# anthonyhu/tumblr-emotions

Measured on AMD Instinct MI355X. Metric: training samples/sec (224x224 img + 32-tok text, batch 256), higher is better.
Workload: dtype f32; 1 GPU; joint train step (fwd+bwd+all-reduce+Adam): Inception-v1 224x224x3 + 300-d embedding + LSTM-512, T=32, V=10000, 15 classes, batch 256 per GPU, reference freeze (<=Mixed_5b conv weights frozen, all BN betas trainable), dropout 0.8, BN train mode; global_batch=256, per_gpu_batch=256, parallelism=dp1, launch=eager

## Files before the change

include/ds_kernels.h:

```cpp
#ifndef DS_KERNELS_H
#define DS_KERNELS_H

#include <stddef.h>
#include <stdint.h>

#ifdef __cplusplus
extern "C" {
#endif

#define DS_OK 0
#define DS_ERR_ARG (-1)
#define DS_ERR_LAUNCH (-2)
#define DS_ERR_WORKSPACE (-3)

#define DS_DTYPE_F32 0
#define DS_DTYPE_BF16 1

#define DS_EPI_BIAS 1
#define DS_EPI_RELU 2
#define DS_EPI_ACCUM 4
#define DS_EPI_STATS 8
#define DS_EPI_MASK 16
#define DS_EPI_BNSUMS 32
#define DS_EPI_BN_RELU 64
// ... 312 lines not shown
                           int32_t N, int32_t H, int32_t W, int32_t C, int32_t k, int32_t stride, int32_t pad_t,
                           int32_t pad_l, int32_t OH, int32_t OW, int32_t y_dtype, float *amax, void *stream);
int ds_bn_pool_bwd_partials(int32_t N, int32_t OH, int32_t OW, int32_t C);
int ds_bn_pool_bwd_reduce(const float *z, const float *dpool, const uint8_t *argmax, int32_t N, int32_t H, int32_t W,
                          int32_t C, int32_t pad_t, int32_t pad_l, int32_t OH, int32_t OW, const float *mean,
                          const float *rstd, const float *shift, float *partials, void *stream);
int ds_bn_pool_bwd_apply(const float *z, const float *dpool, const uint8_t *argmax, int32_t N, int32_t H, int32_t W,
                         int32_t C, int32_t pad_t, int32_t pad_l, int32_t OH, int32_t OW, const float *mean,
                         const float *rstd, const float *shift, const float *coef, float *dz, void *stream);
int ds_bn_pool_bwd_apply_cols(const float *z, int32_t ldz, float *dz, int32_t lddz, const float *dpool, const uint8_t *argmax,
                              int32_t Cp, int32_t c0, int32_t N, int32_t H, int32_t W, int32_t pad_t, int32_t pad_l, int32_t OH,
                              int32_t OW, int32_t ncols, const float *mean, const float *rstd, const float *shift,
                              const float *coef_g, const float *coef_gx, int32_t k, void *stream);
int ds_bn_pool_infer_bwd_apply(const float *z, const float *dpool, const uint8_t *argmax, int32_t N, int32_t H, int32_t W,
                               int32_t C, int32_t pad_t, int32_t pad_l, int32_t OH, int32_t OW, const float *rstd,
                               const float *shift, float *dz, void *stream);
int ds_bn_pool_infer_bwd_apply_sums(const float *z, const float *dpool, const uint8_t *argmax, int32_t N, int32_t H, int32_t W,
                                    int32_t C, int32_t pad_t, int32_t pad_l, int32_t OH, int32_t OW, const float *rstd,
                                    const float *shift, float *dz, float *partials, void *stream);
int ds_maxpool_bwd(const float *dy, const uint8_t *argmax, float *dx, int32_t accumulate, int32_t N,
                   int32_t H, int32_t W, int32_t C, int32_t k, int32_t stride, int32_t pad_t, int32_t pad_l,
                   int32_t OH, int32_t OW, void *stream);

int ds_maxpool3_bwd_sums_partials(int32_t N, int32_t W, int32_t C);
int ds_maxpool3_bwd_sums(const float *dy, const uint8_t *argmax, float *dx, int32_t accumulate, const void *y,
                         int32_t y_dtype, int32_t N, int32_t H, int32_t W, int32_t C, float *partials, void *stream);

int ds_maxpool3_bwd_dy16(const void *dy16, const uint8_t *argmax, float *dx, int32_t accumulate, const void *y, int32_t y_dtype,
                         int32_t N, int32_t H, int32_t W, int32_t C, float *partials, void *stream);

int ds_avgpool_dropout_fwd(const float *x, int32_t N, int32_t HW, int32_t C, float keep, uint64_t seed,
                           const uint64_t *seed_dev, const float *mask_in, float *mask_out, float *out,
                           void *stream);
int ds_avgpool_dropout_bwd(const float *dout, const float *mask, int32_t N, int32_t HW, int32_t C,
                           float keep, float *dx, void *stream);

int ds_gather_rows(const float *table, const int64_t *ids, float *out, int32_t B, int32_t T, int32_t D,
                   int64_t table_rows, int32_t time_major, void *stream);

int ds_token_dot(const float *dx, const float *x, const int64_t *seq_len, float *out, int32_t B, int32_t T, int32_t D,
                 void *stream);

int ds_embedding_grad(const float *dx, const int64_t *ids, float *dtable, int32_t B, int32_t T, int32_t D,
                      int64_t table_rows, int32_t time_major, void *stream);

int ds_lstm_cell_fwd(float *gates, const float *rec_slabs, int32_t nslabs, int64_t slab_stride,
                     const float *c_prev, const float *h_prev, const int64_t *seq_len, int32_t t, int32_t B,
                     int32_t H, float forget_bias, float *c_out, float *h_out, void *stream);
int ds_lstm_cell_bwd(const float *acts, const float *c_t, const float *c_prev, const float *dh,
                     const float *dh_slabs, int32_t nslabs, int64_t slab_stride, const float *dc,
                     const int64_t *seq_len, int32_t t, int32_t B, int32_t H, float *dgates, float *dc_prev,
                     float *dh_carry, void *stream);

int ds_seq_sort_desc(const int64_t *seq_len, int32_t B, int32_t T, int32_t *perm, int64_t *len_sorted, void *stream);
int ds_permute_rows(const void *src, int64_t lds, void *dst, int64_t ldd, const int32_t *perm, int32_t rows, int32_t cols,
                    int32_t elem_bytes, int32_t gather, void *stream);
#define DS_LSTM_SKIP_MASKED 256
int ds_lstm_seq_supported(int32_t B, int32_t H);
size_t ds_lstm_seq_workspace(int32_t B, int32_t H);
int ds_lstm_seq_fwd(float *gates, const float *wh, int32_t ldw, float *h, float *c, const int64_t *seq_len, int32_t T,
                    int32_t B, int32_t H, float forget_bias, int32_t rows, void *ws, size_t ws_bytes, void *stream);
int ds_lstm_seq_bwd(const float *acts, const float *wh, int32_t ldw, const float *c, const float *dh_last,
                    int32_t ld_dh, const int64_t *seq_len, int32_t T, int32_t B, int32_t H, float *dgates, int32_t rows,
                    void *ws, size_t ws_bytes, void *stream);
int ds_lstm_seq_status(void *ws, int32_t B);
#ifdef DS_TUNING
int ds_debug_lstm_seq_set_profile(void *buf);
int ds_debug_lstm_seq_set_profile_bwd(void *buf);
#endif

int ds_softmax_ce(const float *logits, const int64_t *labels, int32_t B, int32_t C, float grad_scale,
                  const float *grad_scale_dev, float *loss, float *dlogits, void *stream);

int ds_adam_tf(float *theta, const float *g, float *m, float *v, int64_t n, int64_t n_wd, float wd,
               float grad_scale, float lr_t, const float *lr_t_dev, float beta1, float beta2, float eps,
               void *stream);

int ds_grad_accumulate(float *acc, float *g, int64_t n, int32_t mode, void *stream);

int ds_sumsq(const float *x, int64_t n, float *scratch, float *out, void *stream);
int ds_colsum(const float *x, int64_t M, int32_t C, int32_t ld, float *scratch, float *out, void *stream);
int ds_slab_epilogue(const float *slabs, int32_t splits, int64_t slab_stride, int32_t lds, int64_t M, int32_t N, float *out,
                     int32_t ldo, const float *bias, const float *mask, int32_t ldmask, int32_t flags, void *stream);
int ds_copy2d(const float *src, int32_t lds, float *dst, int32_t ldd, int64_t rows, int32_t cols,
              void *stream);
int ds_pad_channels(const float *src, int32_t cs, float *dst, int32_t cd, int64_t pixels, void *stream);
int ds_fill(float *dst, int64_t n, float value, void *stream);

typedef struct ds_preprocess_desc {
    int64_t offset;
    int32_t height, width;
    float scale_y, scale_x;
} ds_preprocess_desc;
int ds_preprocess_eval(const uint8_t *bytes, int64_t nbytes, const ds_preprocess_desc *desc, int32_t batch, const float *lut,
                       float *out, int32_t out_h, int32_t out_w, void *stream);

#define DS_PREPROCESS_FLIP 1u
#define DS_PREPROCESS_SATURATION_FIRST 2u
typedef struct ds_preprocess_train_desc {
    int64_t offset;
    int32_t height, width;
    float scale_y, scale_x;
    float delta;
    float factor;
    uint32_t flags;
    uint32_t reserved;
} ds_preprocess_train_desc;
int ds_preprocess_train(const uint8_t *bytes, int64_t nbytes, const ds_preprocess_train_desc *desc, int32_t batch,
                        const float *lut, float *out, int32_t out_h, int32_t out_w, void *stream);

#define DS_JPEG_UNSUPPORTED 1
#define DS_JPEG_MORE 2
#define DS_JPEG_444 0
#define DS_JPEG_422 1
#define DS_JPEG_420 2
#define DS_JPEG_GREY 3
typedef struct ds_jpeg_info {
    int32_t width, height;
    int32_t components;
    int32_t sampling;
    int32_t restart_interval;
    int32_t supported;
    int64_t coef_count;
    int64_t coef_bytes;
    uint8_t quant[3][64];
} ds_jpeg_info;
int ds_jpeg_probe(const uint8_t *bytes, int64_t n, ds_jpeg_info *info);
int ds_jpeg_entropy_decode(const uint8_t *bytes, int64_t n, const ds_jpeg_info *info, int16_t *coef, int64_t capacity);

typedef struct ds_jpeg_desc {
    int64_t coef_offset;
    int64_t out_offset;
    int32_t width, height;
    int32_t sampling;
    int32_t y0, x0, crop_h, crop_w;
    int32_t reserved;
    uint8_t quant[3][64];
} ds_jpeg_desc;
int ds_jpeg_reconstruct_host(const int16_t *coef, int64_t ncoef, const ds_jpeg_desc *desc, int32_t batch,
                             uint8_t *out_bytes, int64_t nbytes);
int ds_jpeg_reconstruct(const int16_t *coef, int64_t ncoef, const ds_jpeg_desc *desc, int32_t batch, uint8_t *out_bytes,
                        int64_t nbytes, void *scratch, int64_t scratch_bytes, void *stream);

typedef struct ds_example_fields {
    int64_t image_offset, image_length;
    int64_t seq_len, label, post_id, day;
    int32_t text_len;
    int32_t reserved;
} ds_example_fields;
int ds_example_parse(const uint8_t *rec, int64_t n, int64_t *text, int32_t text_capacity, ds_example_fields *fields);
int ds_jpeg_record_decode(const uint8_t *rec, int64_t n, int64_t *text, int32_t text_capacity, ds_example_fields *fields,
                          ds_jpeg_info *info, int16_t *coef, int64_t capacity, int32_t *jpeg_status);

typedef struct ds_jpeg_huff {
    uint8_t counts[16];
    uint8_t values[256];
} ds_jpeg_huff;
typedef struct ds_jpeg_scan_info {
    int64_t scan_begin;
    int64_t cut_count;
    ds_jpeg_huff dc[3], ac[3];
} ds_jpeg_scan_info;
int ds_jpeg_scan(const uint8_t *bytes, int64_t n, ds_jpeg_info *info, ds_jpeg_scan_info *scan, int64_t *cuts, int64_t capacity);
int ds_jpeg_record_scan(const uint8_t *rec, int64_t n, int64_t *text, int32_t text_capacity, ds_example_fields *fields,
                        ds_jpeg_info *info, ds_jpeg_scan_info *scan, int64_t *cuts, int64_t capacity, int32_t *jpeg_status);
int ds_jpeg_restart_transcode(const uint8_t *bytes, int64_t n, int32_t interval_mcus, uint8_t *out, int64_t capacity,
// ... 51 lines not shown
```

tumblr_emotions_amd/_lib.py:

```python
import ctypes as C
import os

_HERE = os.path.dirname(os.path.abspath(__file__))
LIB_PATH = os.environ.get("DS_LIB") or os.path.join(_HERE, "libds_kernels.so")

def tuning_env(name, default=None):
    return os.environ.get(name, default) if os.environ.get("DS_LIB") else default


DS_EPI_BIAS, DS_EPI_RELU, DS_EPI_ACCUM, DS_EPI_STATS, DS_EPI_MASK, DS_EPI_BNSUMS = 1, 2, 4, 8, 16, 32
DS_EPI_BN_RELU = 64
DS_DTYPE_F32, DS_DTYPE_BF16 = 0, 1
DS_FP8_E4M3, DS_FP8_E5M2 = 0, 1
DS_CONV_FWD, DS_CONV_DGRAD = 0, 1
DS_LSTM_SKIP_MASKED = 256
DS_ARITH_F32, DS_ARITH_BF16, DS_ARITH_FP8, DS_ARITH_F32X3 = 0, 1, 2, 3
DS_FAM_IGEMM, DS_FAM_WINO2, DS_FAM_WINO4, DS_FAM_STEM, DS_FAM_BF16D, DS_FAM_FP8D, DS_FAM_F32X3, DS_FAM_WINO4H, DS_FAM_STEM_POOL = range(9)
DS_FAM_STEM_DGRAD = 9
DS_PLAN_NO_WINO, DS_PLAN_NO_WINO4, DS_PLAN_NO_STEM_DIRECT, DS_PLAN_NO_BF16_DIRECT, DS_PLAN_ACT16, DS_PLAN_PACKED_RGB = 1, 2, 4, 8, 16, 32
DS_PLAN_FP8_EVERYWHERE, DS_PLAN_FP8_WIDE_RULE, DS_PLAN_NO_WINO4H, DS_PLAN_STEM_POOL = 64, 128, 256, 512
DS_PLAN_NO_SPLITK = 1024
DS_PREPROCESS_FLIP, DS_PREPROCESS_SATURATION_FIRST = 1, 2
DS_JPEG_UNSUPPORTED, DS_JPEG_MORE = 1, 2
DS_JPEG_444, DS_JPEG_422, DS_JPEG_420, DS_JPEG_GREY = 0, 1, 2, 3
DS_JPEG_E_CODE, DS_JPEG_E_RUN, DS_JPEG_E_RANGE, DS_JPEG_E_COLUMN, DS_JPEG_E_SEGMENT, DS_JPEG_E_TABLE = 1, 2, 4, 8, 16, 32


class ConvDesc(C.Structure):
    _fields_ = [
        ("N", C.c_int32), ("H", C.c_int32), ("W", C.c_int32), ("Cin", C.c_int32), ("ldx", C.c_int32),
        ("KH", C.c_int32), ("KW", C.c_int32), ("stride", C.c_int32), ("pad_t", C.c_int32), ("pad_l", C.c_int32),
        ("OH", C.c_int32), ("OW", C.c_int32), ("Cout", C.c_int32), ("ldz", C.c_int32),
        ("w_tap_stride", C.c_int64), ("w_n_stride", C.c_int32), ("w_k_stride", C.c_int32),
        ("flip", C.c_int32), ("fold_cin", C.c_int32), ("flags", C.c_int32), ("ldmask", C.c_int32),
        ("splits", C.c_int32), ("z_split_stride", C.c_int64),
        ("tile_nt", C.c_int32), ("grid_x", C.c_int32), ("dtype", C.c_int32), ("x_dtype", C.c_int32),
        ("partials", C.c_int32),
        ("norm_rstd", C.c_void_p), ("norm_shift", C.c_void_p), ("mask_rstd", C.c_void_p), ("mask_shift", C.c_void_p),
        ("bnb", C.c_void_p), ("mask_dtype", C.c_int32), ("z_dtype", C.c_int32), ("pool_argmax", C.c_void_p), ("fin", C.c_void_p),
    ]


class BnBwdOnLoad(C.Structure):
    _fields_ = [("mean", C.c_void_p), ("rstd", C.c_void_p), ("shift", C.c_void_p), ("coef", C.c_void_p),
                ("nseg", C.c_int32), ("c_end", C.c_int32 * 3), ("ld", C.c_int32 * 3), ("dy", C.c_void_p * 3)]


class BnFinalizeInLaunch(C.Structure):
    _fields_ = [("beta", C.c_void_p), ("mean", C.c_void_p), ("rstd", C.c_void_p), ("shift", C.c_void_p),
                ("moving_mean", C.c_void_p), ("moving_var", C.c_void_p), ("ticket", C.c_void_p), ("count", C.c_int64),
                ("eps", C.c_float), ("decay", C.c_float)]


class LayerPlanStruct(C.Structure):
    _fields_ = [("d", ConvDesc), ("family", C.c_int32), ("role", C.c_int32), ("arith", C.c_int32), ("partials", C.c_int32),
                ("w_cin", C.c_int32), ("w_cout", C.c_int32), ("k", C.c_int32), ("a_format", C.c_int32), ("x16_ok", C.c_int32),
                ("w_bytes", C.c_int64), ("wscale_floats", C.c_int64), ("alg_flops", C.c_double), ("splitk", C.c_int32),
                ("reserved0", C.c_int32), ("ws_bytes", C.c_int64)]


class ConvIO(C.Structure):
    _fields_ = [("bias", C.c_void_p), ("mask", C.c_void_p), ("stats", C.c_void_p), ("pivot", C.c_void_p),
                ("x_amax", C.c_void_p), ("wscale", C.c_void_p), ("fin", C.c_void_p), ("ws", C.c_void_p), ("ws_bytes", C.c_size_t),
                ("scale", C.c_void_p), ("shift", C.c_void_p)]


class Segments(C.Structure):
    _fields_ = [("nseg", C.c_int32), ("c_begin", C.c_int32 * 4), ("c_end", C.c_int32 * 4),
                ("ld", C.c_int32 * 4), ("ptr", C.c_void_p * 4), ("dtype", C.c_int32 * 4),
                ("amax", C.c_void_p * 4), ("ptr2", C.c_void_p * 4)]


class BnFinalizeJob(C.Structure):
    _fields_ = [("stats", C.c_void_p), ("P", C.c_int32), ("C", C.c_int32), ("count", C.c_int64), ("beta", C.c_void_p),
                ("pivot", C.c_void_p), ("mean", C.c_void_p), ("rstd", C.c_void_p), ("shift", C.c_void_p),
                ("moving_mean", C.c_void_p), ("moving_var", C.c_void_p)]


class BnInferJob(C.Structure):
    _fields_ = [("beta", C.c_void_p), ("moving_mean", C.c_void_p), ("moving_var", C.c_void_p), ("C", C.c_int32),
                ("rstd", C.c_void_p), ("shift", C.c_void_p)]


class BnSumJob(C.Structure):
    _fields_ = [("partials", C.c_void_p), ("P", C.c_int32), ("C", C.c_int32), ("dbeta", C.c_void_p)]


class SumSegments(C.Structure):
    _fields_ = [("nseg", C.c_int32), ("c_begin", C.c_int32 * 4), ("c_end", C.c_int32 * 4), ("P", C.c_int32 * 4),
                ("kind", C.c_int32 * 4), ("s", C.c_void_p * 4), ("q", C.c_void_p * 4), ("P2", C.c_int32 * 4),
                ("s2", C.c_void_p * 4), ("q2", C.c_void_p * 4)]


class PreprocessDesc(C.Structure):
    _fields_ = [("offset", C.c_int64), ("height", C.c_int32), ("width", C.c_int32), ("scale_y", C.c_float), ("scale_x", C.c_float)]


class PreprocessTrainDesc(C.Structure):
    _fields_ = [("offset", C.c_int64), ("height", C.c_int32), ("width", C.c_int32), ("scale_y", C.c_float), ("scale_x", C.c_float),
                ("delta", C.c_float), ("factor", C.c_float), ("flags", C.c_uint32), ("reserved", C.c_uint32)]


class JpegInfo(C.Structure):
    _fields_ = [("width", C.c_int32), ("height", C.c_int32), ("components", C.c_int32), ("sampling", C.c_int32),
                ("restart_interval", C.c_int32), ("supported", C.c_int32), ("coef_count", C.c_int64), ("coef_bytes", C.c_int64),
                ("quant", C.c_uint8 * 192)]


class JpegDesc(C.Structure):
    _fields_ = [("coef_offset", C.c_int64), ("out_offset", C.c_int64), ("width", C.c_int32), ("height", C.c_int32),
                ("sampling", C.c_int32), ("y0", C.c_int32), ("x0", C.c_int32), ("crop_h", C.c_int32), ("crop_w", C.c_int32),
                ("reserved", C.c_int32), ("quant", C.c_uint8 * 192)]


class JpegHuff(C.Structure):
    _fields_ = [("counts", C.c_uint8 * 16), ("values", C.c_uint8 * 256)]


class JpegScanInfo(C.Structure):
    _fields_ = [("scan_begin", C.c_int64), ("cut_count", C.c_int64), ("dc", JpegHuff * 3), ("ac", JpegHuff * 3)]


class GatherDesc(C.Structure):
    _fields_ = [("src_offset", C.c_int64), ("out_offset", C.c_int64), ("src", C.c_int32), ("pitch", C.c_int32),
                ("y0", C.c_int32), ("x0", C.c_int32), ("height", C.c_int32), ("width", C.c_int32)]


class ExampleFields(C.Structure):
    _fields_ = [("image_offset", C.c_int64), ("image_length", C.c_int64), ("seq_len", C.c_int64), ("label", C.c_int64),
                ("post_id", C.c_int64), ("day", C.c_int64), ("text_len", C.c_int32), ("reserved", C.c_int32)]


_P = C.c_void_p
_i32, _i64, _f32, _u64 = C.c_int32, C.c_int64, C.c_float, C.c_uint64
_CD = C.POINTER(ConvDesc)
_SG = C.POINTER(Segments)
_SS = C.POINTER(SumSegments)
_LP = C.POINTER(LayerPlanStruct)
_IO = C.POINTER(ConvIO)

SIGNATURES = {
    "ds_version": (C.c_int, []),
    "ds_last_error": (C.c_char_p, []),
    "ds_conv_igemm_partials": (C.c_int, [_CD]),
    "ds_conv_igemm_bnsums_supported": (C.c_int, [_CD]),
    "ds_conv_igemm_norm_supported": (C.c_int, [_CD]),
    "ds_conv_igemm_bnb_supported": (C.c_int, [_CD]),
    "ds_conv_igemm_pool3_supported": (C.c_int, [_CD]),
    "ds_conv_igemm_finalize_tickets": (C.c_int, [_CD]),
    "ds_conv_igemm": (C.c_int, [_CD, _P, _P, _P, _P, _P, _P, _P, _P]),
    "ds_weights_bf16_bytes": (C.c_size_t, [_i32, _i32, _i32, _i32]),
    "ds_weights_to_bf16": (C.c_int, [_P, _P, _i32, _i32, _i32, _i32, _P]),
    "ds_conv_bf16_supported": (C.c_int, [_CD]),
    "ds_conv_bf16_partials": (C.c_int, [_CD]),
    "ds_conv_bf16": (C.c_int, [_CD, _P, _P, _P, _P, _P, _P, _P]),
    "ds_weights_f32x3_bytes": (C.c_size_t, [_i32, _i32, _i32, _i32]),
    "ds_weights_to_f32x3": (C.c_int, [_P, _P, _i32, _i32, _i32, _i32, _P]),
    "ds_conv_f32x3_supported": (C.c_int, [_CD]),
    "ds_conv_f32x3_partials": (C.c_int, [_CD]),
    "ds_conv_f32x3": (C.c_int, [_CD, _P, _P, _P, _P, _P, _P, _P]),
    "ds_absmax": (C.c_int, [_P, _i64, _i32, _P, _P]),
    "ds_weights_fp8_bytes": (C.c_size_t, [_i32, _i32, _i32, _i32]),
    "ds_weights_to_fp8": (C.c_int, [_P, _P, _P, _i32, _i32, _i32, _i32, _P]),
    "ds_conv_fp8_supported": (C.c_int, [_CD]),
    "ds_conv_fp8_partials": (C.c_int, [_CD]),
    "ds_conv_fp8": (C.c_int, [_CD, _P, _P, _i32, _P, _P, _P, _P, _P, _P, _P]),
    "ds_conv_stem_partials": (C.c_int, [_i32, _i32, _i32]),
    "ds_conv_stem_bf16_partials": (C.c_int, [_i32, _i32, _i32]),
    "ds_conv_stem": (C.c_int, [_P, _P, _P, _P, _P, _i32, _i32, _i32, _i32, _i32, _i32, _P]),
    "ds_conv_stem_bf16": (C.c_int, [_P, _P, _P, _P, _P, _i32, _i32, _i32, _i32, _i32, _i32, _P]),
    "ds_conv_stem_pool_supported": (C.c_int, [_i32, _i32]),
    "ds_conv_stem_pool_partials": (C.c_int, [_i32, _i32, _i32]),
    "ds_conv_stem_pool": (C.c_int, [_P, _P, _P, _P, _P, _i32, _i32, _i32, _i32, _i32, _i32, _P]),
    "ds_conv_stem_pool_bf16": (C.c_int, [_P, _P, _P, _P, _P, _i32, _i32, _i32, _i32, _i32, _i32, _P]),
    "ds_conv_stem_dgrad_supported": (C.c_int, [_i32, _i32]),
    "ds_conv_stem_dgrad": (C.c_int, [_P, _P, _P, _i32, _i32, _i32, _i32, _i32, _P]),
    "ds_wino_transform_weights": (C.c_int, [_P, _P, _i32, _i32, _i32, _P]),
    "ds_conv_wino_partials": (C.c_int, [_i32, _i32, _i32]),
    "ds_conv_wino": (C.c_int, [_P, _P, _P, _P, _P, _P, _i32, _i32, _i32, _i32, _i32, _i32, _i32, _i32, _P]),
    "ds_conv_wino4_supported": (C.c_int, [_i32, _i32, _i32, _i32]),
    "ds_conv_wino4_prefer": (C.c_int, [_i32, _i32, _i32, _i32, _i32]),
    "ds_wino4_transform_weights": (C.c_int, [_P, _P, _i32, _i32, _i32, _P]),
    "ds_conv_wino4_partials": (C.c_int, [_i32, _i32, _i32]),
    "ds_conv_wino4_splitk_choose": (C.c_int, [_i32, _i32, _i32, _i32, _i32]),
    "ds_conv_wino4_splitk_partials": (C.c_int, [_i32, _i32, _i32]),
    "ds_conv_wino4_splitk_workspace": (C.c_size_t, [_i32, _i32, _i32, _i32, _i32]),
    "ds_conv_wino4_splitk": (C.c_int, [_P, _P, _P, _P, _P, _P, _i32, _i32, _i32, _i32, _i32, _i32, _i32, _i32, _i32, _i32, _P, C.c_size_t, _P]),
    "ds_conv_wino4": (C.c_int, [_P, _P, _P, _P, _P, _P, _i32, _i32, _i32, _i32, _i32, _i32, _i32, _i32, _P]),
    "ds_conv_wino4_bf16x2": (C.c_int, [_P, _P, _P, _P, _P, _P, _i32, _i32, _i32, _i32, _i32, _i32, _i32, _i32, _i32, _P]),
    "ds_conv_wino4_bf16x2_x16": (C.c_int, [_P, _P, _P, _P, _P, _P, _i32, _i32, _i32, _i32, _i32, _i32, _i32, _i32, _i32, _P]),
    "ds_wino4_transform_weights_bf16x2": (C.c_int, [_P, _P, _i32, _i32, _i32, _P]),
    "ds_conv_plan": (C.c_int, [_LP, _i32, _i32, C.c_uint32] + [_i32] * 10),
    "ds_conv_plan_set_flags": (C.c_int, [_LP, _i32]),
    "ds_conv_plan_enable_bnsums": (C.c_int, [_LP, _i32]),
    "ds_conv_plan_norm_supported": (C.c_int, [_LP]),
    "ds_conv_plan_bnb_supported": (C.c_int, [_LP]),
    "ds_conv_plan_enable_pool3": (C.c_int, [_LP, C.c_void_p]),
    "ds_conv_plan_enable_bn_relu": (C.c_int, [_LP]),
    "ds_conv_plan_finalize_tickets": (C.c_int, [_LP]),
    "ds_conv_prepare_weights": (C.c_int, [_LP, _P, _P, _P, _P]),
    "ds_conv_run": (C.c_int, [_LP, _P, _P, _P, _IO, _P]),
    "ds_conv_wgrad_workspace": (C.c_size_t, [_CD]),
    "ds_conv_wgrad": (C.c_int, [_CD, _P, _P, _i32, _P, _P, C.c_size_t, _P]),
    "ds_bn_finalize": (C.c_int, [_P, _i32, _i64, _i32, _P, _P, _f32, _f32, _P, _P, _P, _P, _P, _P]),
    "ds_bn_finalize_centered": (C.c_int, [_P, _i32, _i64, _i32, _P, _P, _f32, _f32, _P, _P, _P, _P, _P, _P, _P, _P]),
    "ds_bn_apply_relu": (C.c_int, [_P, _i64, _i32, _P, _P, _SG, _P]),
    "ds_bn_apply_relu_z16": (C.c_int, [_P, _i64, _i32, _P, _P, _SG, _P]),
    "ds_bn_bwd_apply_z16": (C.c_int, [_P, _i32, _SG, _i64, _i32, _P, _P, _P, _P, _P, _i32, _P, _P]),
    "ds_bn_infer_prepare": (C.c_int, [_P, _P, _P, _f32, _i32, _P, _P, _P]),
    "ds_bn_infer_prepare_multi": (C.c_int, [_P, _i32, _f32, _P]),
    "ds_bn_bwd_partials": (C.c_int, [_i64, _i32]),
    "ds_bn_bwd_reduce": (C.c_int, [_P, _i32, _i32, _SG, _i64, _i32, _P, _P, _P, _P, _P]),
    "ds_bn_bwd_finalize_segs": (C.c_int, [_SS, _i64, _i32, _P, _P, _P, _P]),
    "ds_bn_bwd_finalize": (C.c_int, [_P, _i32, _i64, _i32, _P, _P, _P]),
    "ds_bn_bwd_finalize_multi": (C.c_int, [_SS, _i64, _i32, _P, _P, _P, _P]),
    "ds_bn_finalize_multi": (C.c_int, [_P, _i32, _f32, _f32, _P]),
    "ds_bn_finalize_apply_relu": (C.c_int, [_P, _i32, _i64, _i32, _P, _P, _f32, _f32, _P, _P, _P, _P, _P, _P, _i64, _SG, _P, _P]),
    "ds_bn_bwd_finalize_apply": (C.c_int, [_SS, _P, _P, _P, _P, _P, _P, _i32, _SG, _i64, _i32, _P, _P, _P, _P, _i32, _i32, _P, _P, _P]),
    "ds_bn_bwd_apply": (C.c_int, [_P, _i32, _SG, _i64, _i32, _P, _P, _P, _P, _P, _P, _P]),
    "ds_bn_bwd_apply_cols": (C.c_int, [_P, _i32, _SG, _i64, _i32, _P, _P, _P, _P, _P, _P, _P]),
    "ds_bn_infer_bwd_apply": (C.c_int, [_P, _i32, _SG, _i64, _i32, _P, _P, _P, _P]),
    "ds_bn_infer_bwd_partials": (C.c_int, [_i64, _i32]),
    "ds_bn_infer_bwd_apply_sums": (C.c_int, [_P, _i32, _SG, _i64, _i32, _P, _P, _P, _P, _P]),
    "ds_bn_dbeta_reduce_multi": (C.c_int, [_P, _i32, _P]),
    "ds_bn_bwd_apply_bf16": (C.c_int, [_P, _i32, _SG, _i64, _i32, _P, _P, _P, _P, _P, _i32, _P, _P]),
    "ds_maxpool_fwd": (C.c_int, [_P, _P, _P] + [_i32] * 11 + [_P]),
    "ds_maxpool_bn_relu_fwd": (C.c_int, [_P, _P, _P, _P, _P] + [_i32] * 11 + [_P, _P]),
    "ds_bn_pool_bwd_partials": (C.c_int, [_i32, _i32, _i32, _i32]),
    "ds_bn_pool_bwd_reduce": (C.c_int, [_P, _P, _P] + [_i32] * 8 + [_P, _P, _P, _P, _P]),
    "ds_bn_pool_bwd_apply": (C.c_int, [_P, _P, _P] + [_i32] * 8 + [_P, _P, _P, _P, _P, _P]),
    "ds_bn_pool_bwd_apply_cols": (C.c_int, [_P, _i32, _P, _i32, _P, _P] + [_i32] * 10 + [_P, _P, _P, _P, _P, _i32, _P]),
    "ds_bn_pool_infer_bwd_apply": (C.c_int, [_P, _P, _P] + [_i32] * 8 + [_P, _P, _P, _P]),
    "ds_bn_pool_infer_bwd_apply_sums": (C.c_int, [_P, _P, _P] + [_i32] * 8 + [_P, _P, _P, _P, _P]),
    "ds_maxpool_bwd": (C.c_int, [_P, _P, _P] + [_i32] * 11 + [_P]),
    "ds_maxpool3_bwd_sums_partials": (C.c_int, [_i32, _i32, _i32]),
    "ds_maxpool3_bwd_sums": (C.c_int, [_P, _P, _P, _i32, _P, _i32, _i32, _i32, _i32, _i32, _P, _P]),
    "ds_maxpool3_bwd_dy16": (C.c_int, [_P, _P, _P, _i32, _P, _i32, _i32, _i32, _i32, _i32, _P, _P]),
    "ds_avgpool_dropout_fwd": (C.c_int, [_P, _i32, _i32, _i32, _f32, _u64, _P, _P, _P, _P, _P]),
    "ds_avgpool_dropout_bwd": (C.c_int, [_P, _P, _i32, _i32, _i32, _f32, _P, _P]),
    "ds_gather_rows": (C.c_int, [_P, _P, _P, _i32, _i32, _i32, _i64, _i32, _P]),
    "ds_token_dot": (C.c_int, [_P, _P, _P, _P, _i32, _i32, _i32, _P]),
    "ds_embedding_grad": (C.c_int, [_P, _P, _P, _i32, _i32, _i32, _i64, _i32, _P]),
    "ds_lstm_cell_fwd": (C.c_int, [_P, _P, _i32, _i64, _P, _P, _P, _i32, _i32, _i32, _f32, _P, _P, _P]),
    "ds_lstm_cell_bwd": (C.c_int, [_P, _P, _P, _P, _P, _i32, _i64, _P, _P, _i32, _i32, _i32, _P, _P, _P, _P]),
    "ds_seq_sort_desc": (C.c_int, [_P, _i32, _i32, _P, _P, _P]),
    "ds_permute_rows": (C.c_int, [_P, _i64, _P, _i64, _P, _i32, _i32, _i32, _i32, _P]),
    "ds_lstm_seq_supported": (C.c_int, [_i32, _i32]),
    "ds_lstm_seq_workspace": (C.c_size_t, [_i32, _i32]),
    "ds_lstm_seq_fwd": (C.c_int, [_P, _P, _i32, _P, _P, _P, _i32, _i32, _i32, _f32, _i32, _P, C.c_size_t, _P]),
    "ds_lstm_seq_bwd": (C.c_int, [_P, _P, _i32, _P, _P, _i32, _P, _i32, _i32, _i32, _P, _i32, _P, C.c_size_t, _P]),
    "ds_lstm_seq_status": (C.c_int, [_P, _i32]),
    "ds_softmax_ce": (C.c_int, [_P, _P, _i32, _i32, _f32, _P, _P, _P, _P]),
    "ds_adam_tf": (C.c_int, [_P, _P, _P, _P, _i64, _i64, _f32, _f32, _f32, _P, _f32, _f32, _f32, _P]),
    "ds_grad_accumulate": (C.c_int, [_P, _P, _i64, _i32, _P]),
    "ds_sumsq": (C.c_int, [_P, _i64, _P, _P, _P]),
    "ds_colsum": (C.c_int, [_P, _i64, _i32, _i32, _P, _P, _P]),
    "ds_slab_epilogue": (C.c_int, [_P, _i32, _i64, _i32, _i64, _i32, _P, _i32, _P, _P, _i32, _i32, _P]),
    "ds_copy2d": (C.c_int, [_P, _i32, _P, _i32, _i64, _i32, _P]),
    "ds_pad_channels": (C.c_int, [_P, _i32, _P, _i32, _i64, _P]),
    "ds_fill": (C.c_int, [_P, _i64, _f32, _P]),
    "ds_preprocess_eval": (C.c_int, [_P, _i64, _P, _i32, _P, _P, _i32, _i32, _P]),
    "ds_preprocess_train": (C.c_int, [_P, _i64, _P, _i32, _P, _P, _i32, _i32, _P]),
    "ds_jpeg_probe": (C.c_int, [_P, _i64, C.POINTER(JpegInfo)]),
    "ds_jpeg_entropy_decode": (C.c_int, [_P, _i64, C.POINTER(JpegInfo), _P, _i64]),
    "ds_jpeg_reconstruct_host": (C.c_int, [_P, _i64, _P, _i32, _P, _i64]),
    "ds_jpeg_reconstruct": (C.c_int, [_P, _i64, _P, _i32, _P, _i64, _P, _i64, _P]),
    "ds_example_parse": (C.c_int, [_P, _i64, _P, _i32, C.POINTER(ExampleFields)]),
    "ds_jpeg_record_decode": (C.c_int, [_P, _i64, _P, _i32, C.POINTER(ExampleFields), C.POINTER(JpegInfo), _P, _i64,
                                        C.POINTER(_i32)]),
    "ds_jpeg_scan": (C.c_int, [_P, _i64, C.POINTER(JpegInfo), C.POINTER(JpegScanInfo), _P, _i64]),
    "ds_jpeg_record_scan": (C.c_int, [_P, _i64, _P, _i32, C.POINTER(ExampleFields), C.POINTER(JpegInfo), C.POINTER(JpegScanInfo),
                                      _P, _i64, C.POINTER(_i32)]),
    "ds_jpeg_restart_transcode": (C.c_int, [_P, _i64, _i32, _P, _i64, C.POINTER(_i64)]),
    "ds_jpeg_entropy_decode_segments_host": (C.c_int, [_P, _i64, _P, _i32, _P, _i64, _P, _i64, _P]),
    "ds_jpeg_entropy_decode_device": (C.c_int, [_P, _i64, _P, _i32, _P, _i64, _P, _i64, _P, _P]),
    "ds_ragged_gather": (C.c_int, [_P, _i64, _P, _i64, _P, _i32, _P, _i64, _P]),
    "ds_ragged_gather_host": (C.c_int, [_P, _i64, _P, _i64, _P, _i32, _P, _i64]),
    "ds_eval_metrics_workspace": (C.c_int, [_i32, _i32]),
    "ds_eval_metrics_update": (C.c_int, [_P, _i32, _P, _i32, _i32, _P, _P, _P, _P]),
}

_lib = None


DEBUG_SIGNATURES = {
    "ds_debug_conv_set_tile": (C.c_int, [C.c_int, C.c_int]),
    "ds_debug_conv_set_path": (C.c_int, [C.c_int]),
    "ds_debug_conv_set_wide": (C.c_int, [C.c_int]),
    "ds_debug_conv_wino_allow_ablation": (C.c_int, [C.c_int]),
    "ds_debug_conv_wino4_set_nb": (C.c_int, [C.c_int]),
    "ds_debug_conv_bf16_set_max_nb": (C.c_int, [C.c_int]),
    "ds_debug_lstm_seq_set_profile": (C.c_int, [_P]),
    "ds_debug_lstm_seq_set_profile_bwd": (C.c_int, [_P]),
}
TUNING_LIB_PATH = os.path.join(_HERE, "libds_kernels_tuning.so")
_tuning = None


def _bind(lib, table):
    for name, (res, args) in table.items():
        fn = getattr(lib, name)
        fn.restype = res
        fn.argtypes = args


def load_tuning():
    global _tuning
    if _tuning is None:
        if not os.path.exists(TUNING_LIB_PATH):
            raise RuntimeError("tumblr_emotions_amd: %s not found -- `make -C tumblr_emotions_amd/csrc` builds it" % TUNING_LIB_PATH)
        lib = C.CDLL(TUNING_LIB_PATH)
        _bind(lib, SIGNATURES)
        _bind(lib, DEBUG_SIGNATURES)
        _tuning = lib
    return _tuning


class tuning_library:

    def __enter__(self):
        global _lib
        self._saved = load()
        _lib = load_tuning()
        return _lib

    def __exit__(self, *exc):
        global _lib
        _lib = self._saved
        return False


def load():
    global _lib
    if _lib is not None:
        return _lib
    if not os.path.exists(LIB_PATH):
        raise RuntimeError(
            "tumblr_emotions_amd: %s not found -- build it with `python -c 'import __graft_entry__ as g; "
            "g.build()'` or `make -C tumblr_emotions_amd/csrc`.  There is no CPU fallback." % LIB_PATH)
    if os.environ.get("DS_LIB"):
# ... 14 lines not shown
```

tumblr_emotions_amd/csrc/conv_igemm.hip:

```cpp
#include <stdlib.h>
#include <type_traits>
#include "ds_common.h"

typedef float f32x16 __attribute__((ext_vector_type(16)));
typedef float f32x4 __attribute__((ext_vector_type(4)));
typedef float f32x2 __attribute__((ext_vector_type(2)));
typedef unsigned int u32x4 __attribute__((ext_vector_type(4)));
typedef __attribute__((address_space(3))) void *lds_ptr;

namespace {

constexpr int BK = 16;
constexpr int LDK = 20;
constexpr unsigned kOOB = 0x80000000u;

struct ConvParams {
    ds_conv_desc d;
    const float *x;
    const float *w;
    float *z;
    const float *bias;
    const float *mask;
    float *stats;
    const float *pivot;
    int M;
    int taps;
    int row_tiles;
    unsigned x_bytes, w_bytes;
    int prio_mode;
    int col_tiles;
    int col_total;
    ds_bn_bwd_on_load bnb;
    int pool_rpb, pool_bpi;
    ds_bn_finalize_in_launch fin;
    double fin_inv_count;
    const float *scale, *shift;
};

__device__ __forceinline__ __amdgpu_buffer_rsrc_t make_srd(const void *p, unsigned bytes) {
    return __builtin_amdgcn_make_buffer_rsrc(const_cast<void *>(p), 0, (int)bytes, 0x00020000);
}

struct TileId {
    int row, col, stride;
};
__device__ __forceinline__ TileId tile_id(const ConvParams &p) {
    TileId t;
    if (p.col_tiles > 0) {
        const int id = blockIdx.x;
        const int lin = (id & 7) * (int)(gridDim.x >> 3) + (id >> 3);
        t.row = lin / p.col_tiles;
        t.col = lin - t.row * p.col_tiles;
        t.stride = p.row_tiles;
    } else {
        t.row = blockIdx.x;
        t.col = blockIdx.y;
        t.stride = gridDim.x;
    }
    return t;
}

template <bool VEC>
__device__ __forceinline__ f32x4 load4(__amdgpu_buffer_rsrc_t r, unsigned off, bool ok, int valid) {
    if (VEC) {
        return __builtin_bit_cast(f32x4, __builtin_amdgcn_raw_buffer_load_b128(r, ok ? off : kOOB, 0, 0));
    } else {
        f32x4 v;
#pragma unroll
        for (int j = 0; j < 4; ++j)
            v[j] = __builtin_bit_cast(float, __builtin_amdgcn_raw_buffer_load_b32(r, (ok && j < valid) ? off + 4 * j : kOOB, 0, 0));
        return v;
    }
}

template <int MT, int NT, bool BNMAJOR, bool FOLD, bool VEC, bool BNR = false>
__global__ __launch_bounds__(256, (MT == 1 && NT == 1) ? 4 : (MT == 1 && NT == 2) ? 3 : 1) void conv_igemm_kernel(
    const ConvParams p) {
    constexpr int WM = 4;
    constexpr int BM = WM * MT * 32, BN = NT * 32;
    constexpr int AR = BM / 64;
    constexpr int BR = (BN * 4 + 255) / 256;
    constexpr int LDB = BNMAJOR ? (BN + 4) : LDK;
    constexpr int BSZ = BNMAJOR ? BK * LDB : BN * LDK;
    __shared__ __attribute__((aligned(16))) float smem[2 * BM * LDK + 2 * BSZ];
    float *As = smem;
    float *Bs = smem + 2 * BM * LDK;

    const ds_conv_desc &d = p.d;
    const int tid = threadIdx.x, lane = tid & 63;
    const int wm = __builtin_amdgcn_readfirstlane(tid >> 6);
    const int li = lane & 31, lk = lane >> 5;
    const TileId tid0 = tile_id(p);
    const int n0 = tid0.col * BN;
    const int ohw = d.OH * d.OW;
    const int chunks = (d.Cin + BK - 1) / BK;
    const int KT_all = p.taps * chunks;
    const int kts = (KT_all + (int)gridDim.z - 1) / (int)gridDim.z;
    const int kt0 = (int)blockIdx.z * kts;
    const int KT = (kt0 + kts < KT_all ? kt0 + kts : KT_all) - kt0;
    float *const zout = p.z + (int64_t)blockIdx.z * p.d.z_split_stride;
    const int flags = d.flags;
    const __amdgpu_buffer_rsrc_t srd_x = make_srd(p.x, p.x_bytes);
    const __amdgpu_buffer_rsrc_t srd_w = make_srd(p.w, p.w_bytes);

    switch (p.prio_mode ? ((blockIdx.x + blockIdx.y * gridDim.x + blockIdx.z * gridDim.x * gridDim.y) >> 8) & 3 : 0) {
        case 1: __builtin_amdgcn_s_setprio(1); break;
        case 2: __builtin_amdgcn_s_setprio(2); break;
        case 3: __builtin_amdgcn_s_setprio(3); break;
        default: break;
    }

    float csum[NT], csq[NT];
#pragma unroll
    for (int j = 0; j < NT; ++j) csum[j] = csq[j] = 0.f;

    const int arow = tid >> 2, ak4 = (tid & 3) * 4;

    int b_n[BR], b_k[BR];
    unsigned b_off[BR];
    bool b_ok[BR];
#pragma unroll
    for (int i = 0; i < BR; ++i) {
        const int idx = tid + 256 * i;
        if (BNMAJOR) {
            b_n[i] = n0 + (idx % (BN / 4)) * 4;
            b_k[i] = idx / (BN / 4);
            b_off[i] = (unsigned)b_k[i] * (unsigned)d.w_k_stride + (unsigned)b_n[i];
        } else {
            b_n[i] = n0 + (idx >> 2);
            b_k[i] = (idx & 3) * 4;
            b_off[i] = (unsigned)b_n[i] * (unsigned)d.w_n_stride + (unsigned)b_k[i];
        }
        b_ok[i] = idx < BN * 4 && b_n[i] < d.Cout;
    }

    int ih0[AR], iw0[AR];
    unsigned xb[AR];
    int tap, c0, dh, dw;
    f32x4 ra[AR], rb[BR];
    f32x16 acc[MT][NT];

    auto setup_tile = [&](int tile) {
        const int m0 = tile * BM;
#pragma unroll
        for (int i = 0; i < AR; ++i) {
            const int m = m0 + arow + 64 * i;
            const bool rv = m < p.M;
            const int mm = rv ? m : 0;
            const int n = mm / ohw;
            const int r = mm - n * ohw;
            const int oh = r / d.OW;
            const int ow = r - oh * d.OW;
            ih0[i] = rv ? oh * d.stride - d.pad_t : -(1 << 20);
            iw0[i] = ow * d.stride - d.pad_l;
            xb[i] = (unsigned)n * (unsigned)(d.H * d.W) * (unsigned)d.ldx;
        }
        const int chunk = kt0 / p.taps;
        tap = kt0 - chunk * p.taps;
        c0 = chunk * BK;
        dh = tap / d.KW;
        dw = tap - dh * d.KW;
    };

    {

        auto load_tile = [&]() {
            const int k = c0 + ak4;
#pragma unroll
            for (int i = 0; i < AR; ++i) {
                const int ih = ih0[i] + dh;
                const int iw = iw0[i] + dw;
                const int iwc = FOLD ? iw + k / d.fold_cin : iw;
                const bool ok = (unsigned)ih < (unsigned)d.H && (unsigned)iwc < (unsigned)d.W && k < d.Cin;
                const unsigned off = xb[i] + (unsigned)(ih * d.W + iw) * (unsigned)d.ldx + (unsigned)k;
                ra[i] = load4<VEC>(srd_x, off * 4u, ok, d.Cin - k);
            }
            const int tap_eff = d.flip ? p.taps - 1 - tap : tap;
            const unsigned wt = (unsigned)tap_eff * (unsigned)d.w_tap_stride +
                                (unsigned)c0 * (BNMAJOR ? (unsigned)d.w_k_stride : 1u);
#pragma unroll
            for (int i = 0; i < BR; ++i) {
                const bool ok = b_ok[i] && c0 + b_k[i] < d.Cin;
                rb[i] = load4<VEC>(srd_w, (wt + b_off[i]) * 4u, ok, BNMAJOR ? d.Cout - b_n[i] : d.Cin - c0 - b_k[i]);
            }
            ++tap;
            if (++dw == d.KW) {
                dw = 0;
                if (++dh == d.KH) { dh = 0; tap = 0; c0 += BK; }
// ... 67 lines not shown
        for (int a = 0; a < MT; ++a)
#pragma unroll
            for (int b = 0; b < NT; ++b)
#pragma unroll
                for (int r = 0; r < 16; ++r) acc[a][b][r] = 0.f;
        for (int kt = 0; kt < KT; ++kt) {
            const bool last = kt + 1 == KT;
            if (last && has_next) setup_tile(tile + tid0.stride);
            const bool fetch = !last || has_next;
            if (fetch) load_tile();
            compute(par);
            if (fetch) store_tile(par ^ 1);
            __syncthreads();
            par ^= 1;
        }

#pragma unroll
        for (int b = 0; b < NT; ++b) {
            const int col = n0 + b * 32 + li;
            const bool colok = col < d.Cout;
            const float bv = ((flags & DS_EPI_BIAS) && colok) ? p.bias[col] : 0.f;
            const float pv = (p.pivot && colok) ? p.pivot[col] : 0.f;
            float s = 0.f, q = 0.f;
            if constexpr (BNR) {
                const float sc = colok ? p.scale[col] : 0.f, sh = colok ? p.shift[col] : 0.f;
#pragma unroll
                for (int a = 0; a < MT; ++a) {
#pragma unroll
                    for (int r = 0; r < 16; ++r) {
                        const int row = m0 + wm * MT * 32 + a * 32 + (r & 3) + 8 * (r >> 2) + 4 * lk;
                        if (row < p.M && colok) zout[(int64_t)row * d.ldz + col] = fmaxf(fmaf(acc[a][b][r], sc, sh), 0.f);
                    }
                }
                continue;
            }
#pragma unroll
            for (int a = 0; a < MT; ++a) {
#pragma unroll
                for (int r = 0; r < 16; ++r) {
                    const int row = m0 + wm * MT * 32 + a * 32 + (r & 3) + 8 * (r >> 2) + 4 * lk;
                    if (row < p.M && colok) {
                        float v = acc[a][b][r] + bv;
                        const int64_t off = (int64_t)row * d.ldz + col;
                        if (flags & DS_EPI_ACCUM) v += zout[off];
                        if (flags & DS_EPI_MASK) v = p.mask[(int64_t)row * d.ldmask + col] > 0.f ? v : 0.f;
                        if (flags & DS_EPI_RELU) v = fmaxf(v, 0.f);
                        zout[off] = v;
                        const float u = v - pv;
                        s += u;
                        q += u * u;
                    }
                }
            }
            csum[b] += s;
            csq[b] += q;
        }
    }
    }

    if (flags & DS_EPI_STATS) {
        float *red = smem;
        __syncthreads();
#pragma unroll
        for (int b = 0; b < NT; ++b) {
            const float s = csum[b] + __shfl_xor(csum[b], 32);
            const float q = csq[b] + __shfl_xor(csq[b], 32);
            if (lk == 0) {
                const int c = b * 32 + li;
                red[(wm * BN + c) * 2 + 0] = s;
                red[(wm * BN + c) * 2 + 1] = q;
            }
        }
        __syncthreads();
        if (tid < BN && n0 + tid < d.Cout && tid0.row < p.row_tiles) {
            float s = 0.f, q = 0.f;
#pragma unroll
            for (int w = 0; w < WM; ++w) {
                s += red[(w * BN + tid) * 2 + 0];
                q += red[(w * BN + tid) * 2 + 1];
            }
            p.stats[(int64_t)(n0 + tid) * tid0.stride + tid0.row] = s;
            p.stats[((int64_t)d.Cout + n0 + tid) * tid0.stride + tid0.row] = q;
        }
    }
}

template <int MT, int NT, bool BNMAJOR>
struct Frag {
    f32x4 alo[MT], ahi[MT];
    f32x4 blo[BNMAJOR ? 1 : NT], bhi[BNMAJOR ? 1 : NT];
    float bs[BNMAJOR ? NT : 1][8];
};

template <int MT, int NT, bool BNMAJOR, bool FOLD>
__global__ __launch_bounds__(256) void conv_direct_kernel(const ConvParams p) {
    const ds_conv_desc &d = p.d;
    const int tid = threadIdx.x, lane = tid & 63;
    const int wave = __builtin_amdgcn_readfirstlane(tid >> 6);
    const int li = lane & 31, lk = lane >> 5;
    constexpr int BM = 32 * MT, BN = 32 * NT;
    const int n0 = blockIdx.y * BN;
    const int ohw = d.OH * d.OW;
    const int chunks = (d.Cin + BK - 1) / BK;
    const int KT_all = p.taps * chunks;
    const int kts = (KT_all + (int)gridDim.z - 1) / (int)gridDim.z;
    const int kt0 = (int)blockIdx.z * kts;
    const int KT = (kt0 + kts < KT_all ? kt0 + kts : KT_all) - kt0;
    float *const zout = p.z + (int64_t)blockIdx.z * p.d.z_split_stride;
    const int flags = d.flags;
    const __amdgpu_buffer_rsrc_t srd_x = make_srd(p.x, p.x_bytes);
    const __amdgpu_buffer_rsrc_t srd_w = make_srd(p.w, p.w_bytes);
    const int wave_id = blockIdx.x * 4 + wave, waves = gridDim.x * 4;

    unsigned b_off[NT];
    bool b_ok[NT];
#pragma unroll
    for (int b = 0; b < NT; ++b) {
        const int n = n0 + b * 32 + li;
        b_ok[b] = n < d.Cout;
        b_off[b] = BNMAJOR ? (unsigned)n + (unsigned)(lk * 8) * (unsigned)d.w_k_stride
                           : (unsigned)n * (unsigned)d.w_n_stride + (unsigned)(lk * 8);
    }

    int ih0[MT], iw0[MT];
    unsigned xb[MT];
    int tap, c0, dh, dw;
    auto setup_tile = [&](int tile) {
#pragma unroll
        for (int a = 0; a < MT; ++a) {
            const int m = tile * BM + a * 32 + li;
            const bool rv = m < p.M;
            const int mm = rv ? m : 0;
            const int n = mm / ohw;
            const int r = mm - n * ohw;
            const int oh = r / d.OW;
            const int ow = r - oh * d.OW;
            ih0[a] = rv ? oh * d.stride - d.pad_t : -(1 << 20);
            iw0[a] = ow * d.stride - d.pad_l;
            xb[a] = (unsigned)n * (unsigned)(d.H * d.W) * (unsigned)d.ldx;
        }
        const int chunk = kt0 / p.taps;
        tap = kt0 - chunk * p.taps;
        c0 = chunk * BK;
        dh = tap / d.KW;
        dw = tap - dh * d.KW;
    };

    typedef Frag<MT, NT, BNMAJOR> F;
    auto load = [&](F &f) {
        const int k = c0 + lk * 8;
#pragma unroll
        for (int a = 0; a < MT; ++a) {
            const int ih = ih0[a] + dh, iw = iw0[a] + dw;
            const bool pix = (unsigned)ih < (unsigned)d.H;
            const bool ok0 = pix && (unsigned)(FOLD ? iw + k / d.fold_cin : iw) < (unsigned)d.W && k < d.Cin;
            const bool ok1 = pix && (unsigned)(FOLD ? iw + (k + 4) / d.fold_cin : iw) < (unsigned)d.W && k + 4 < d.Cin;
            const unsigned off = (xb[a] + (unsigned)(ih * d.W + iw) * (unsigned)d.ldx + (unsigned)k) * 4u;
            f.alo[a] = __builtin_bit_cast(f32x4, __builtin_amdgcn_raw_buffer_load_b128(srd_x, ok0 ? off : kOOB, 0, 0));
            f.ahi[a] = __builtin_bit_cast(f32x4, __builtin_amdgcn_raw_buffer_load_b128(srd_x, ok1 ? off + 16u : kOOB, 0, 0));
        }
        const int tap_eff = d.flip ? p.taps - 1 - tap : tap;
        const unsigned wt = (unsigned)tap_eff * (unsigned)d.w_tap_stride + (unsigned)c0 * (BNMAJOR ? (unsigned)d.w_k_stride : 1u);
        if (BNMAJOR) {
#pragma unroll
            for (int b = 0; b < NT; ++b)
#pragma unroll
// ... 1714 lines not shown
extern "C" int ds_debug_conv_set_path(int path) {
    DS_REQUIRE(path >= 0 && path <= 3, "ds_debug_conv_set_path: 0 = automatic, 1 = register-staged LDS kernel, 2 = register-direct kernel, 3 = LDS-DMA kernel");
    force_path = path;
    return DS_OK;
}
#endif

extern "C" int ds_conv_igemm_partials(const ds_conv_desc *d) {
    Variant v;
    v.bnmajor = d->w_n_stride == 1 && d->w_k_stride != 1;
    v.fold = d->fold_cin > 0;
    v.vec = dims_vec(d);
    const TileCfg c = pick_cfg(d, v.vec);
    int gx, gy, rt;
    grid_for(d, c, v, &gx, &gy, &rt);
    return c.direct ? gx * 4 : gx;
}

extern "C" int ds_conv_igemm_bnsums_supported(const ds_conv_desc *d) {
    if (!d) return 0;
    ds_conv_desc t = *d;
    t.flags = (t.flags & DS_EPI_ACCUM) | DS_EPI_BNSUMS;
    return wide_nb(&t, dims_vec(&t)) > 0 ? 1 : 0;
}

extern "C" int ds_conv_igemm_norm_supported(const ds_conv_desc *d) {
    if (!d || d->Cin > 1024) return 0;
    return wide_nb(d, dims_vec(d)) > 0 ? 1 : 0;
}

extern "C" int ds_conv_igemm_pool3_supported(const ds_conv_desc *d) {
    if (!d) return 0;
    return pool3_nb(d, dims_vec(d)) > 0 ? 1 : 0;
}

extern "C" int ds_conv_igemm_finalize_tickets(const ds_conv_desc *d) {
    if (!d || !(d->flags & DS_EPI_STATS)) return 0;
    ds_conv_desc t = *d;
    t.partials = 0;
    t.fin = nullptr;
    const Variant v = {t.w_n_stride == 1 && t.w_k_stride != 1, t.fold_cin > 0, dims_vec(&t)};
    const TileCfg c = pick_cfg(&t, v.vec);
    if (!c.wide) return 0;
    int gx, gy, rt;
    grid_for(&t, c, v, &gx, &gy, &rt);
    return rt <= 256 ? gy : 0;
}

namespace ds {
int conv_igemm_bn_relu_supported(const ds_conv_desc *d) {
    if (!d || (d->flags & ~DS_EPI_BN_RELU)) return 0;
    ds_conv_desc t = *d;
    t.flags = DS_EPI_BN_RELU;
    const Variant v = {t.w_n_stride == 1 && t.w_k_stride != 1, t.fold_cin > 0, dims_vec(&t)};
    return bnr_supported(&t, pick_cfg(&t, v.vec), v) ? 1 : 0;
}
}

extern "C" int ds_conv_igemm_bnb_supported(const ds_conv_desc *d) {
    if (!d || d->Cin > 1024 || (d->w_n_stride == 1 && d->w_k_stride != 1) || d->norm_rstd) return 0;
    return wide_nb(d, dims_vec(d), true) > 0 ? 1 : 0;
}

namespace {
int igemm_launch(const ds_conv_desc *d, const float *x, const float *w, float *z, const float *bias, const float *mask,
                 float *stats, const float *pivot, const float *scale, const float *shift, void *stream);
}

extern "C" int ds_conv_igemm(const ds_conv_desc *d, const float *x, const float *w, float *z, const float *bias,
                             const float *mask, float *stats, const float *pivot, void *stream) {
    DS_REQUIRE(!d || !(d->flags & DS_EPI_BN_RELU), "ds_conv_igemm: DS_EPI_BN_RELU takes its scale / shift through ds_conv_run (ds_conv_io)");
    return igemm_launch(d, x, w, z, bias, mask, stats, pivot, nullptr, nullptr, stream);
}

namespace ds {
int conv_igemm_bn_relu(const ds_conv_desc *d, const float *x, const float *w, float *z, const float *scale, const float *shift,
                       void *stream) {
    DS_REQUIRE(d && (d->flags & DS_EPI_BN_RELU) && scale && shift, "ds_conv_run: DS_EPI_BN_RELU without scale / shift");
    return igemm_launch(d, x, w, z, nullptr, nullptr, nullptr, nullptr, scale, shift, stream);
}
}

namespace {
int igemm_launch(const ds_conv_desc *d, const float *x, const float *w, float *z, const float *bias, const float *mask,
                 float *stats, const float *pivot, const float *scale, const float *shift, void *stream) {
    DS_REQUIRE(d && x && w && z, "ds_conv_igemm: null argument");
    DS_REQUIRE(d->Cin > 0 && d->Cout > 0 && d->N > 0 && d->OH > 0 && d->OW > 0, "ds_conv_igemm: bad dims");
    DS_REQUIRE(d->w_n_stride == 1 || d->w_k_stride == 1, "ds_conv_igemm: one weight stride must be 1");
    DS_REQUIRE(!(d->flags & DS_EPI_BIAS) || bias, "ds_conv_igemm: DS_EPI_BIAS without bias");
    DS_REQUIRE(!(d->flags & DS_EPI_MASK) || mask, "ds_conv_igemm: DS_EPI_MASK without mask");
    DS_REQUIRE(!(d->flags & DS_EPI_STATS) || stats, "ds_conv_igemm: DS_EPI_STATS without stats buffer");
    DS_REQUIRE(!(d->flags & DS_EPI_BNSUMS) || (stats && mask && !(d->flags & (DS_EPI_STATS | DS_EPI_MASK)) && d->ldmask >= d->Cout),
               "ds_conv_igemm: DS_EPI_BNSUMS needs the partials buffer (stats), y (mask, ldmask) and excludes STATS / MASK");
    DS_REQUIRE(conv_M(d) < (1ll << 31), "ds_conv_igemm: M too large");
    DS_REQUIRE(d->dtype == DS_DTYPE_F32 || d->dtype == DS_DTYPE_BF16, "ds_conv_igemm: dtype must be DS_DTYPE_F32 or DS_DTYPE_BF16");
    const Variant v = variant_of(d, x, w);
    DS_REQUIRE(!(d->flags & DS_EPI_STATS) || v.vec == dims_vec(d),
               "ds_conv_igemm: DS_EPI_STATS needs 16-byte aligned operand pointers");

    ConvParams p;
    p.d = *d;
    p.x = x; p.w = w; p.z = z; p.bias = bias; p.mask = mask; p.stats = stats;
    p.pivot = (d->flags & DS_EPI_STATS) ? pivot : nullptr;
    p.M = (int)conv_M(d);
    p.taps = d->KH * d->KW;
    static int prio_mode = -1;
    if (prio_mode < 0) {
        const char *e = ds::tune_env("DS_CONV_PRIO");
        prio_mode = e ? atoi(e) : 0;
    }
    p.prio_mode = prio_mode;
    const int64_t x_elems = ((int64_t)d->N * d->H * d->W - 1) * d->ldx + (v.fold ? d->fold_cin : d->Cin);
    const int64_t w_elems = (int64_t)(p.taps - 1) * d->w_tap_stride + (int64_t)(d->Cout - 1) * d->w_n_stride +
                            (int64_t)(d->Cin - 1) * d->w_k_stride + 1;
    DS_REQUIRE(x_elems * 4 < (1ll << 31) && w_elems * 4 < (1ll << 31),
               "ds_conv_igemm: operand larger than 2 GiB (split the batch)");
    p.x_bytes = (unsigned)(x_elems * 4);
    p.w_bytes = (unsigned)(w_elems * 4);
    DS_REQUIRE(!v.fold || (v.bnmajor && v.vec && d->KW == 1 && d->fold_cin % 4 == 0 && d->ldx == d->fold_cin),
               "ds_conv_igemm: fold_cin needs KW=1, n-contiguous 16-byte-aligned weights, ldx==fold_cin");

    DS_REQUIRE(d->dtype != DS_DTYPE_BF16 || (v.vec && d->splits <= 1),
               "ds_conv_igemm: DS_DTYPE_BF16 needs 16-byte aligned operands with channel counts / strides divisible by 4, no split-K");
    const int splits = d->splits > 1 ? d->splits : 1;
    DS_REQUIRE(splits == 1 || (d->flags == 0 && d->z_split_stride >= (int64_t)(conv_M(d) - 1) * d->ldz + d->Cout),
               "ds_conv_igemm: split-K needs flags == 0 and non-overlapping output slabs");
    if (splits == 1) p.d.z_split_stride = 0;
    const TileCfg c = pick_cfg(d, v.vec);
    const bool bnr = (d->flags & DS_EPI_BN_RELU) != 0;
    DS_REQUIRE(!bnr || (d->flags == DS_EPI_BN_RELU && scale && shift && bnr_supported(d, c, v)),
               "ds_conv_igemm: DS_EPI_BN_RELU excludes every other epilogue flag, needs scale / shift and a forward fp32 launch "
               "with 16-byte aligned operands (ds_conv_plan_enable_bn_relu)");
    p.scale = scale; p.shift = shift;
    int gx, gy, rt;
    bool one;
    grid_for(d, c, v, &gx, &gy, &rt, &one);
    DS_REQUIRE((!d->norm_rstd && !d->norm_shift) || (c.wide && d->norm_rstd && d->norm_shift && d->Cin <= 1024),
               "ds_conv_igemm: norm_rstd / norm_shift are implemented by the wide 1x1 kernel only (ds_conv_igemm_norm_supported)");
    DS_REQUIRE((!d->mask_rstd && !d->mask_shift) || ((d->flags & DS_EPI_BNSUMS) && d->mask_rstd && d->mask_shift),
               "ds_conv_igemm: mask_rstd / mask_shift go with DS_EPI_BNSUMS");
    DS_REQUIRE(!(d->flags & DS_EPI_BNSUMS) || c.wide,
               "ds_conv_igemm: DS_EPI_BNSUMS is implemented by the wide 1x1 kernel only (ds_conv_igemm_bnsums_supported)");
    DS_REQUIRE(!(d->flags & (DS_EPI_STATS | DS_EPI_BNSUMS)) || d->partials <= 0 || d->partials == (c.direct ? gx * 4 : gx),
               "ds_conv_igemm: the launch would write %d statistics partials but the plan was made for %d "
               "(a ds_debug_conv_set_* switch changed after planning?)", c.direct ? gx * 4 : gx, d->partials);
    p.row_tiles = rt;
    static int xcd_remap = -1;
    if (xcd_remap < 0) {
        const char *e = ds::tune_env("DS_CONV_XCD_REMAP");
        xcd_remap = e ? atoi(e) : 1;
    }
    dim3 grid(gx, gy, splits);
    p.col_tiles = 0;
    if (one && (c.wide || (xcd_remap && gy > 1)) && !c.direct) {
        p.col_tiles = gy;
        grid = dim3((rt * gy + 7) / 8 * 8, 1, splits);
    }
    if (d->bnb) {
        const ds_bn_bwd_on_load &b = *d->bnb;
        DS_REQUIRE(c.wide && !v.bnmajor && d->Cin <= 1024 && !d->norm_rstd,
                   "ds_conv_igemm: ds_conv_desc.bnb is implemented by the wide 1x1 kernel for k-contiguous weights only "
                   "(ds_conv_igemm_bnb_supported)");
        DS_REQUIRE(b.mean && b.rstd && b.shift && b.coef && b.nseg >= 1 && b.nseg <= 3 && b.c_end[b.nseg - 1] == d->Cin,
                   "ds_conv_igemm: bnb needs mean / rstd / shift / coef and 1..3 channel ranges that end at Cin");
        for (int i = 0; i < b.nseg; ++i) {
            const int cb = i ? b.c_end[i - 1] : 0;
            DS_REQUIRE(b.dy[i] && (((uintptr_t)b.dy[i]) & 15) == 0 && b.ld[i] % 4 == 0 && b.c_end[i] > cb && cb % 16 == 0 &&
                           b.ld[i] >= b.c_end[i] - cb && ((int64_t)(p.M - 1) * b.ld[i] + (b.c_end[i] - cb)) * 4 < (1ll << 31),
                       "ds_conv_igemm: bnb channel range %d (16-byte aligned dy, ld %% 4 == 0, boundaries %% 16 == 0)", i);
        }
        p.bnb = b;
    }
    p.fin = ds_bn_finalize_in_launch{};
    p.fin_inv_count = 0.0;
    if (d->fin) {
        DS_REQUIRE(c.wide && (d->flags & DS_EPI_STATS) && rt <= 256 && d->fin->ticket && d->fin->beta && d->fin->mean &&
                       d->fin->rstd && d->fin->shift && d->fin->count > 0,
                   "ds_conv_igemm: ds_conv_desc.fin needs a DS_EPI_STATS launch of the wide 1x1 kernel with at most 256 partials "
                   "(ds_conv_igemm_finalize_tickets) and beta / mean / rstd / shift / ticket / count");
        p.fin = *d->fin;
        p.fin_inv_count = 1.0 / (double)d->fin->count;
    }
    p.pool_rpb = p.pool_bpi = 0;
    if (d->pool_argmax) {
        DS_REQUIRE(c.wide && v.bnmajor && pool3_nb(d, v.vec) == c.wide && !d->bnb,
                   "ds_conv_igemm: ds_conv_desc.pool_argmax is implemented by the wide 1x1 kernel's forward instantiation only "
                   "(ds_conv_igemm_pool3_supported)");
        pool3_blocks(d, &p.pool_rpb, &p.pool_bpi);
    }
    if (c.wide) launch_wide(c.wide, v.bnmajor, d->bnb != nullptr, grid, (hipStream_t)stream, p);
    else hipLaunchKernelGGL(bnr ? bnr_kernel(c) : kernel_for(c, v), grid, dim3(256), 0, (hipStream_t)stream, p);
    return ds::check_launch("ds_conv_igemm");
}
}

namespace {
int g_bf16d_max_nb = 8;
int bf16d_nb(int Cout, bool x16_1x1) {
    const int top = x16_1x1 && g_bf16d_max_nb > 4 ? 4 : g_bf16d_max_nb;
    int best = top, best_cost = 1 << 30;
    for (int nb = top; nb >= 1; --nb) {
        const int tiles = (Cout + 32 * nb - 1) / (32 * nb);
        const int cost = tiles * (4 + nb);
        if (cost < best_cost) { best_cost = cost; best = nb; }
    }
    return best;
}
bool bf16d_ok(const ds_conv_desc *d) {
    return (d->KH == d->KW) && (d->KH == 1 || d->KH == 3) && d->fold_cin == 0 && d->Cin % 8 == 0 && d->ldx % 4 == 0 &&
           !(d->flags & ~(DS_EPI_STATS | DS_EPI_ACCUM | DS_EPI_BNSUMS)) &&
           !((d->flags & DS_EPI_BNSUMS) && (d->flags & DS_EPI_STATS)) && d->splits <= 1 &&
           ((conv_M(d) - 1) * d->ldz + d->Cout) * 4 < (1ll << 31) &&
           (!(d->flags & DS_EPI_BNSUMS) || ((conv_M(d) - 1) * d->ldmask + d->Cout) * 4 < (1ll << 31));
}
}

extern "C" size_t ds_weights_bf16_bytes(int32_t Cin, int32_t Cout, int32_t taps, int32_t dgrad) {
    const int K = dgrad ? Cout : Cin, Ncol = dgrad ? Cin : Cout;
    return (size_t)((K + 15) / 16) * taps * ((Ncol + 31) / 32 * 32) * 16 * 2;
}

extern "C" int ds_weights_to_bf16(const float *w, void *wb, int32_t Cin, int32_t Cout, int32_t taps, int32_t dgrad,
                                  void *stream) {
    DS_REQUIRE(w && wb && Cin > 0 && Cout > 0 && taps > 0, "ds_weights_to_bf16: bad argument");
    const int64_t total = (int64_t)ds_weights_bf16_bytes(Cin, Cout, taps, dgrad) / 2;
    hipLaunchKernelGGL(weights_to_bf16_kernel, dim3(ds::stream_grid(total, 256)), dim3(256), 0, (hipStream_t)stream, w,
                       (__bf16 *)wb, Cin, Cout, taps, dgrad);
    return ds::check_launch("ds_weights_to_bf16");
}

extern "C" int ds_conv_bf16_supported(const ds_conv_desc *d) { return d && bf16d_ok(d) ? 1 : 0; }

#ifdef DS_TUNING
extern "C" int ds_debug_conv_bf16_set_max_nb(int nb) {
    DS_REQUIRE(nb >= 1 && nb <= 8, "ds_debug_conv_bf16_set_max_nb: 1 .. 8 column blocks per wave");
    g_bf16d_max_nb = nb;
    return 0;
}
#endif

extern "C" int ds_conv_bf16_partials(const ds_conv_desc *d) { return (int)((conv_M(d) + 127) / 128); }

extern "C" int ds_conv_bf16(const ds_conv_desc *d, const void *x, const void *wb, float *z, const void *mask, float *stats,
                            const float *pivot, void *stream) {
    DS_REQUIRE(d && x && wb && z, "ds_conv_bf16: null argument");
    DS_REQUIRE(!(d->flags & DS_EPI_BNSUMS) || (mask && stats && d->ldmask >= d->Cout &&
                                               (d->mask_dtype == DS_DTYPE_F32 || d->mask_dtype == DS_DTYPE_BF16)),
               "ds_conv_bf16: DS_EPI_BNSUMS needs mask (row stride ldmask, mask_dtype) and a partials buffer");
    DS_REQUIRE(!d->mask_rstd && !d->norm_rstd && !d->bnb, "ds_conv_bf16: the on-load transforms belong to the fp32 kernels");
    DS_REQUIRE(d->x_dtype == DS_DTYPE_F32 || (d->x_dtype == DS_DTYPE_BF16 && d->ldx % 8 == 0),
               "ds_conv_bf16: x_dtype must be DS_DTYPE_F32 or DS_DTYPE_BF16 (then ldx %% 8 == 0)");
    const bool xb = d->x_dtype == DS_DTYPE_BF16;
    DS_REQUIRE(bf16d_ok(d), "ds_conv_bf16: needs a 1x1 or 3x3 conv, Cin %% 8 == 0, ldx %% 4 == 0, flags within DS_EPI_STATS, or "
                            "DS_EPI_ACCUM | DS_EPI_BNSUMS for a dgrad");
    DS_REQUIRE(((((uintptr_t)x | (uintptr_t)wb) & 15) == 0) && conv_M(d) < (1ll << 31), "ds_conv_bf16: operands must be 16-byte aligned");
    DS_REQUIRE(!(d->flags & DS_EPI_STATS) || stats, "ds_conv_bf16: DS_EPI_STATS without stats buffer");
    DS_REQUIRE(d->z_dtype == DS_DTYPE_F32 || (d->z_dtype == DS_DTYPE_BF16 && !(d->flags & (DS_EPI_ACCUM | DS_EPI_BNSUMS))),
               "ds_conv_bf16: the output in bf16 storage excludes the accumulate / BatchNorm-sums epilogues");
    ConvParams p = {};
    p.d = *d;
    p.x = (const float *)x; p.w = (const float *)wb; p.z = z; p.stats = stats; p.mask = (const float *)mask;
    p.pivot = (d->flags & DS_EPI_STATS) ? pivot : nullptr;
    p.M = (int)conv_M(d);
    p.taps = d->KH * d->KW;
    const int64_t x_elems = ((int64_t)d->N * d->H * d->W - 1) * d->ldx + d->Cin;
    const int64_t wb_bytes = (int64_t)((d->Cin + 15) / 16) * p.taps * ((d->Cout + 31) / 32 * 32) * 32;
    DS_REQUIRE(x_elems * 4 < (1ll << 31) && wb_bytes < (1ll << 31), "ds_conv_bf16: operand larger than 2 GiB");
    p.x_bytes = (unsigned)(x_elems * (xb ? 2 : 4));
    p.w_bytes = (unsigned)wb_bytes;
    p.col_total = (d->Cout + 31) / 32 * 32;
    const int nb = bf16d_nb(d->Cout, xb && d->KH == 1);
    p.row_tiles = (int)((conv_M(d) + 127) / 128);
    p.col_tiles = (d->Cout + 32 * nb - 1) / (32 * nb);
    const dim3 grid((unsigned)(((int64_t)p.row_tiles * p.col_tiles + 7) / 8 * 8));
    hipStream_t st = (hipStream_t)stream;
#define DS_B16(NBV)                                                                                        \
// ... 87 lines not shown
```

tumblr_emotions_amd/csrc/text_misc.hip:

```cpp
#include <stdlib.h>
#include "ds_common.h"

namespace {

template <int VEC, bool NT = true, bool OUTORDER = false>
__global__ __launch_bounds__(256) void gather_rows_kernel(const float *table, const int64_t *ids, float *out, int B,
                                                          int T, int D, int64_t rows, int time_major, int rpw) {
    typedef float vec_t __attribute__((ext_vector_type(VEC)));
    const int lane = threadIdx.x & 63;
    const int64_t wave = ((int64_t)blockIdx.x * 256 + threadIdx.x) >> 6;
    const int64_t total = (int64_t)B * T;
    int64_t r = wave * rpw;
    const int64_t r1 = r + rpw < total ? r + rpw : total;
    if (r >= r1) return;
    const int DV = D / VEC;
    int b, t;
    if (OUTORDER) { t = (int)(r / B); b = (int)(r - (int64_t)t * B); }
    else { b = (int)(r / T); t = (int)(r - (int64_t)b * T); }
    constexpr int U = 4;
    if (VEC == 4 && DV <= 128) {
        const float *srcA[U], *srcB[U];
        float *dstA[U], *dstB[U];
        bool okA[U], okB[U];
        vec_t a0[U], a1[U], b0[U], b1[U];
// ... 93 lines not shown
            const int b = p / T, t = p - b * T;
            const float *src = dx + (time_major ? (int64_t)t * B + b : (int64_t)p) * D;
#pragma unroll
            for (int q = 0; q < NQ; ++q) {
                const int c = lane + 64 * q;
                if (c < D) acc[q] += src[c];
            }
        }
    }
#pragma unroll
    for (int q = 0; q < NQ; ++q) {
        const int c = lane + 64 * q;
        if (c < D) dtable[v * D + c] = acc[q];
    }
}

__device__ __forceinline__ float sigmoidf_(float x) { return 1.f / (1.f + __expf(-x)); }

__global__ __launch_bounds__(256) void lstm_cell_fwd_kernel(float *gates, const float *rec, int nslabs,
                                                            int64_t slab_stride, const float *c_prev,
                                                            const float *h_prev, const int64_t *seq_len, int t, int B,
                                                            int H, float forget_bias, float *c_out, float *h_out) {
    const int64_t total = (int64_t)B * H;
    for (int64_t i = (int64_t)blockIdx.x * 256 + threadIdx.x; i < total; i += (int64_t)gridDim.x * 256) {
        const int b = (int)(i / H), h = (int)(i - (int64_t)b * H);
        float *g = gates + (int64_t)b * 4 * H + h;
        float pi = g[0], pj = g[H], pf = g[2 * H], po = g[3 * H];
        for (int s = 0; s < nslabs; ++s) {
            const float *r = rec + s * slab_stride + (int64_t)b * 4 * H + h;
            pi += r[0]; pj += r[H]; pf += r[2 * H]; po += r[3 * H];
        }
        const float si = sigmoidf_(pi);
        const float tj = tanhf(pj);
        const float sf = sigmoidf_(pf + forget_bias);
        const float so = sigmoidf_(po);
        const float cp = c_prev[i], hp = h_prev[i];
        const float cn = cp * sf + si * tj;
        const float hn = tanhf(cn) * so;
        const bool live = (int64_t)t < seq_len[b];
        g[0] = si;
        g[H] = tj;
        g[2 * H] = sf;
        g[3 * H] = so;
        c_out[i] = live ? cn : cp;
        h_out[i] = live ? hn : hp;
    }
}

__global__ __launch_bounds__(256) void lstm_cell_bwd_kernel(const float *acts, const float *c_t, const float *c_prev,
                                                            const float *dh, const float *dh_slabs, int nslabs,
                                                            int64_t slab_stride, const float *dc,
                                                            const int64_t *seq_len, int t, int B, int H,
                                                            float *dgates, float *dc_prev, float *dh_carry) {
    const int64_t total = (int64_t)B * H;
    for (int64_t i = (int64_t)blockIdx.x * 256 + threadIdx.x; i < total; i += (int64_t)gridDim.x * 256) {
        const int b = (int)(i / H), h = (int)(i - (int64_t)b * H);
        const float *a = acts + (int64_t)b * 4 * H + h;
        float *dg = dgates + (int64_t)b * 4 * H + h;
        const bool live = (int64_t)t < seq_len[b];
        float dhv = dh[i];
        for (int s = 0; s < nslabs; ++s) dhv += dh_slabs[s * slab_stride + i];
        const float dcv = dc[i];
        if (live) {
            const float si = a[0], tj = a[H], sf = a[2 * H], so = a[3 * H];
            const float tc = tanhf(c_t[i]);
            const float dct = dcv + dhv * so * (1.f - tc * tc);
            dg[0] = dct * tj * si * (1.f - si);
            dg[H] = dct * si * (1.f - tj * tj);
            dg[2 * H] = dct * c_prev[i] * sf * (1.f - sf);
            dg[3 * H] = dhv * tc * so * (1.f - so);
            dc_prev[i] = dct * sf;
            dh_carry[i] = 0.f;
        } else {
            dg[0] = 0.f;
            dg[H] = 0.f;
            dg[2 * H] = 0.f;
            dg[3 * H] = 0.f;
            dc_prev[i] = dcv;
            dh_carry[i] = dhv;
        }
    }
}

__global__ __launch_bounds__(256) void softmax_ce_kernel(const float *logits, const int64_t *labels, int B, int C,
                                                         float grad_scale, const float *grad_scale_dev,
                                                         float *loss, float *dlogits) {
    __shared__ float red[256];
    if (grad_scale_dev) grad_scale *= grad_scale_dev[0];
    float acc = 0.f;
    for (int b = threadIdx.x; b < B; b += 256) {
        const float *z = logits + (int64_t)b * C;
        float m = -INFINITY;
        for (int c = 0; c < C; ++c) m = fmaxf(m, z[c]);
        float s = 0.f;
        for (int c = 0; c < C; ++c) s += expf(z[c] - m);
        const int64_t yl = labels[b];
        const bool yok = yl >= 0 && yl < C;
        const int y = yok ? (int)yl : -1;
        acc += yok ? (m + logf(s)) - z[y] : NAN;
        if (dlogits) {
            const float k = grad_scale / (float)B, inv = 1.f / s;
            for (int c = 0; c < C; ++c)
                dlogits[(int64_t)b * C + c] = (expf(z[c] - m) * inv - (c == y ? 1.f : 0.f)) * k;
        }
    }
    red[threadIdx.x] = acc;
    __syncthreads();
    for (int o = 128; o > 0; o >>= 1) {
        if (threadIdx.x < o) red[threadIdx.x] += red[threadIdx.x + o];
        __syncthreads();
    }
    if (threadIdx.x == 0 && loss) loss[0] = red[0] / (float)B;
}

__global__ __launch_bounds__(256) void adam_tf_kernel(float *theta, const float *g, float *m, float *v, int64_t n,
                                                      int64_t n_wd, float wd, float grad_scale, float lr_t,
                                                      const float *lr_t_dev, float b1, float b2, float eps) {
    if (lr_t_dev) lr_t = lr_t_dev[0];
    for (int64_t i = (int64_t)blockIdx.x * 256 + threadIdx.x; i < n; i += (int64_t)gridDim.x * 256) {
        const float w = theta[i];
        float gi = g[i] * grad_scale;
        if (i < n_wd) gi += wd * w;
        const float mi = b1 * m[i] + (1.f - b1) * gi;
        const float vi = b2 * v[i] + (1.f - b2) * gi * gi;
        m[i] = mi;
        v[i] = vi;
        theta[i] = w - lr_t * mi / (sqrtf(vi) + eps);
    }
}

constexpr int kAccumVecPerBlock = 256 * 4;

template <int MODE>
__global__ __launch_bounds__(256) void grad_accumulate_kernel(float4 *acc, float4 *g, int64_t n4) {
    for (int64_t i = (int64_t)blockIdx.x * 256 + threadIdx.x; i < n4; i += (int64_t)gridDim.x * 256) {
        const float4 b = g[i];
        if (MODE == 0) {
            acc[i] = b;
        } else {
            const float4 a = acc[i];
            const float4 s = make_float4(a.x + b.x, a.y + b.y, a.z + b.z, a.w + b.w);
            if (MODE == 1) acc[i] = s;
            else g[i] = s;
        }
    }
}

constexpr int kSumsqBlocks = 256;

__global__ __launch_bounds__(256) void sumsq_stage1(const float *x, int64_t n, float *partials) {
    __shared__ float red[256];
    float acc = 0.f;
    for (int64_t i = (int64_t)blockIdx.x * 256 + threadIdx.x; i < n; i += (int64_t)gridDim.x * 256) acc += x[i] * x[i];
    red[threadIdx.x] = acc;
    __syncthreads();
    for (int o = 128; o > 0; o >>= 1) {
        if (threadIdx.x < o) red[threadIdx.x] += red[threadIdx.x + o];
        __syncthreads();
    }
    if (threadIdx.x == 0) partials[blockIdx.x] = red[0];
}

__global__ __launch_bounds__(256) void sum_stage2(const float *partials, int n, float *out) {
    __shared__ double red[256];
    double acc = 0.0;
    for (int i = threadIdx.x; i < n; i += 256) acc += (double)partials[i];
    red[threadIdx.x] = acc;
    __syncthreads();
    for (int o = 128; o > 0; o >>= 1) {
        if (threadIdx.x < o) red[threadIdx.x] += red[threadIdx.x + o];
        __syncthreads();
    }
    if (threadIdx.x == 0) out[0] = (float)red[0];
}

__global__ __launch_bounds__(256) void colsum_stage1(const float *x, int64_t M, int C, int ld, int rows_per_split,
                                                     float *partials) {
    __shared__ float red[4][64];
    const int cl = threadIdx.x & 63, rl = threadIdx.x >> 6;
    const int c = blockIdx.x * 64 + cl;
    const int64_t r0 = (int64_t)blockIdx.y * rows_per_split;
    int64_t r1 = r0 + rows_per_split;
    if (r1 > M) r1 = M;
    float acc = 0.f;
    if (c < C)
        for (int64_t r = r0 + rl; r < r1; r += 4) acc += x[r * ld + c];
    red[rl][cl] = acc;
    __syncthreads();
    if (rl == 0 && c < C) partials[(int64_t)blockIdx.y * C + c] = red[0][cl] + red[1][cl] + red[2][cl] + red[3][cl];
}

__global__ __launch_bounds__(256) void colsum_small_kernel(const float *x, int64_t M, int C, int ld, int rows_per_split,
                                                           int RS, float *out) {
    __shared__ float red[4][64];
    const int cl = threadIdx.x & 63, rl = threadIdx.x >> 6;
// ... 217 lines not shown
        perm[rank] = i;
        len_sorted[rank] = li;
    }
}

template <typename E>
__global__ __launch_bounds__(256) void permute_rows_kernel(const E *src, int64_t lds, E *dst, int64_t ldd, const int *perm,
                                                           int rows, int cols, int gather) {
    const int64_t total = (int64_t)rows * cols;
    for (int64_t i = (int64_t)blockIdx.x * 256 + threadIdx.x; i < total; i += (int64_t)gridDim.x * 256) {
        const int r = (int)(i / cols), c = (int)(i - (int64_t)r * cols);
        const int pr = perm[r];
        if (gather) dst[(int64_t)r * ldd + c] = src[(int64_t)pr * lds + c];
        else dst[(int64_t)pr * ldd + c] = src[(int64_t)r * lds + c];
    }
}

extern "C" int ds_seq_sort_desc(const int64_t *seq_len, int32_t B, int32_t T, int32_t *perm, int64_t *len_sorted, void *stream) {
    DS_REQUIRE(seq_len && perm && len_sorted && B > 0 && B <= 4096 && T > 0, "ds_seq_sort_desc: bad argument (1 <= B <= 4096)");
    hipLaunchKernelGGL(seq_sort_desc_kernel, dim3(1), dim3(256), (size_t)B * sizeof(int), (hipStream_t)stream, seq_len, B, T, perm,
                       len_sorted);
    return ds::check_launch("ds_seq_sort_desc");
}

extern "C" int ds_permute_rows(const void *src, int64_t lds, void *dst, int64_t ldd, const int32_t *perm, int32_t rows, int32_t cols,
                               int32_t elem_bytes, int32_t gather, void *stream) {
    DS_REQUIRE(src && dst && perm && rows > 0 && cols > 0 && lds >= cols && ldd >= cols && (elem_bytes == 4 || elem_bytes == 8),
               "ds_permute_rows: bad argument (elem_bytes 4 or 8)");
    const int grid = ds::stream_grid((int64_t)rows * cols, 256);
    if (elem_bytes == 4)
        hipLaunchKernelGGL(permute_rows_kernel<float>, dim3(grid), dim3(256), 0, (hipStream_t)stream, (const float *)src, lds,
                           (float *)dst, ldd, perm, rows, cols, gather);
    else
        hipLaunchKernelGGL(permute_rows_kernel<int64_t>, dim3(grid), dim3(256), 0, (hipStream_t)stream, (const int64_t *)src, lds,
                           (int64_t *)dst, ldd, perm, rows, cols, gather);
    return ds::check_launch("ds_permute_rows");
}

extern "C" int ds_colsum(const float *x, int64_t M, int32_t C, int32_t ld, float *scratch, float *out, void *stream) {
    DS_REQUIRE(x && scratch && out && M > 0 && C > 0 && ld >= C, "ds_colsum: bad argument");
    int RS = (int)((M + 63) / 64);
    if (RS > 64) RS = 64;
    const int rps = (int)((M + RS - 1) / RS);
    if (RS <= 8) {
        hipLaunchKernelGGL(colsum_small_kernel, dim3((C + 63) / 64), dim3(256), 0, (hipStream_t)stream, x, M, C, ld, rps, RS, out);
        return ds::check_launch("ds_colsum");
    }
    hipLaunchKernelGGL(colsum_stage1, dim3((C + 63) / 64, RS), dim3(256), 0, (hipStream_t)stream, x, M, C, ld, rps,
                       scratch);
    hipLaunchKernelGGL(colsum_stage2, dim3((C + 255) / 256), dim3(256), 0, (hipStream_t)stream, scratch, RS, C, out);
    return ds::check_launch("ds_colsum");
}

__global__ __launch_bounds__(256) void slab_epilogue_kernel(const float *slabs, int splits, int64_t slab_stride, int lds,
                                                            int64_t M, int N, float *out, int ldo, const float *bias,
                                                            const float *mask, int ldmask, int flags) {
    const int64_t total = M * N;
    for (int64_t i = (int64_t)blockIdx.x * 256 + threadIdx.x; i < total; i += (int64_t)gridDim.x * 256) {
        const int64_t m = i / N;
        const int n = (int)(i - m * N);
        float v = 0.f;
        for (int k = 0; k < splits; ++k) v += slabs[(int64_t)k * slab_stride + m * lds + n];
        if (flags & DS_EPI_BIAS) v += bias[n];
        const int64_t o = m * ldo + n;
        if (flags & DS_EPI_ACCUM) v += out[o];
        if (flags & DS_EPI_MASK) v = mask[m * ldmask + n] > 0.f ? v : 0.f;
        if (flags & DS_EPI_RELU) v = fmaxf(v, 0.f);
        out[o] = v;
    }
}

extern "C" int ds_slab_epilogue(const float *slabs, int32_t splits, int64_t slab_stride, int32_t lds, int64_t M, int32_t N,
                                float *out, int32_t ldo, const float *bias, const float *mask, int32_t ldmask, int32_t flags,
                                void *stream) {
    DS_REQUIRE(slabs && out && splits >= 1 && M > 0 && N > 0 && lds >= N && ldo >= N, "ds_slab_epilogue: bad argument");
    DS_REQUIRE((flags & ~(DS_EPI_BIAS | DS_EPI_ACCUM | DS_EPI_MASK | DS_EPI_RELU)) == 0 && (!(flags & DS_EPI_BIAS) || bias) &&
                   (!(flags & DS_EPI_MASK) || (mask && ldmask >= N)),
               "ds_slab_epilogue: flags are BIAS / ACCUM / MASK / RELU (with their operands)");
    hipLaunchKernelGGL(slab_epilogue_kernel, dim3(ds::stream_grid(M * N, 256)), dim3(256), 0, (hipStream_t)stream, slabs, splits,
                       slab_stride, lds, M, N, out, ldo, bias, mask, ldmask, flags);
    return ds::check_launch("ds_slab_epilogue");
}

extern "C" int ds_copy2d(const float *src, int32_t lds, float *dst, int32_t ldd, int64_t rows, int32_t cols,
                         void *stream) {
    DS_REQUIRE(src && dst && rows > 0 && cols > 0, "ds_copy2d: bad argument");
    hipLaunchKernelGGL(copy2d_kernel, dim3(ds::stream_grid(rows * cols, 256)), dim3(256), 0, (hipStream_t)stream, src,
                       lds, dst, ldd, rows, cols);
    return ds::check_launch("ds_copy2d");
}

extern "C" int ds_pad_channels(const float *src, int32_t cs, float *dst, int32_t cd, int64_t pixels, void *stream) {
    DS_REQUIRE(src && dst && cs > 0 && cd >= cs && pixels > 0, "ds_pad_channels: bad argument");
    hipLaunchKernelGGL(pad_channels_kernel, dim3(ds::stream_grid(pixels * cd, 256)), dim3(256), 0, (hipStream_t)stream,
                       src, cs, dst, cd, pixels);
    return ds::check_launch("ds_pad_channels");
}

extern "C" int ds_fill(float *dst, int64_t n, float value, void *stream) {
    DS_REQUIRE(dst && n > 0, "ds_fill: bad argument");
    hipLaunchKernelGGL(fill_kernel, dim3(ds::stream_grid(n, 256)), dim3(256), 0, (hipStream_t)stream, dst, n, value);
    return ds::check_launch("ds_fill");
}
```

tumblr_emotions_amd/engine_image.py:

```python
import contextlib
import ctypes as C
import os
from collections import namedtuple

import torch

from . import _lib, ops
from .ops import WgradPlan, gemm_plan, make_segments, same_pad, DS_EPI_BIAS, DS_EPI_STATS

BN_EPS = 0.001
BN_DECAY = 0.9997
WEIGHT_DECAY = 0.00004

TOPOLOGY = [
    ("conv", "Conv2d_1a_7x7", 7, 2, 64),
    ("maxpool", "MaxPool_2a_3x3", 3, 2),
    ("conv", "Conv2d_2b_1x1", 1, 1, 64),
    ("conv", "Conv2d_2c_3x3", 3, 1, 192),
    ("maxpool", "MaxPool_3a_3x3", 3, 2),
    ("mixed", "Mixed_3b", 64, (96, 128), (16, 32), 32),
    ("mixed", "Mixed_3c", 128, (128, 192), (32, 96), 64),
    ("maxpool", "MaxPool_4a_3x3", 3, 2),
    ("mixed", "Mixed_4b", 192, (96, 208), (16, 48), 64),
    ("mixed", "Mixed_4c", 160, (112, 224), (24, 64), 64),
# ... 1001 lines not shown
        from_pool = self.pooled_bwd and batched and not eng.fuse_fin_apply
        if self.pooled_bwd and not from_pool:
            nx = self.next
            ops.maxpool_bwd(nx.dout, nx.argmax, self.dout, False, self.B, self.H, self.W, self.C, nx.k, nx.stride, "SAME")
        if batched:
            self._bn_backward_closing(from_pool)
        if infer and self.zcat:
            M, Ct = self.B * self.H * self.W, self.C
            if self._infer_close is None:
                self._infer_close = (make_segments([(0, Ct - b0, self.dout.data_ptr() + 4 * b0, Ct)]), self.out.view(M, Ct)[:, b0:])
            dy, z = self._infer_close
            if self.c1.gbeta is not None:
                if self._fz_close is None:
                    P = ops.bn_infer_bwd_partials(M, Ct - b0)
                    self._fz_close = torch.empty((Ct - b0) * P, device=eng.device)
                    off = 0
                    for l in (self.c1, self.c2, self.c3):
                        l.fz_job = (self._fz_close.data_ptr() + 4 * off * P, P)
                        off += l.cout
                ops.bn_infer_bwd_apply_sums(z, dy, M, Ct - b0, self.rs_cat[0, b0:], self.rs_cat[1, b0:], z, self._fz_close, ldz=Ct)
            else:
                ops.bn_infer_bwd_apply(z, dy, M, Ct - b0, self.rs_cat[0, b0:], self.rs_cat[1, b0:], z, ldz=Ct)

        def closing(layer, x_ptr, ldx, dx_ptr, ndx):
            if infer:
                layer.backward_pointwise(x_ptr, ldx, dx_ptr, ndx, apply=not self.zcat)
            elif batched:
                layer._run_dgrad(dx_ptr)
            else:
                layer.backward(x_ptr, ldx, dx_ptr, ndx)

        def branch3():
            closing(self.c3, None if self.fuse_b3 else ops._p(self.pooled), p.C, ops._p(self.dpooled), need_dx)
            if pool_first:
                ops.maxpool_bwd(self.dpooled, self.argmax, p.dout, False, self.B, p.H, p.W, p.C, 3, 1, "SAME")
            elif need_dx and self.split_dout and infer:
                ops.maxpool_bwd(self.dpooled, self.argmax, p.dout2, False, self.B, p.H, p.W, p.C, 3, 1, "SAME")
            elif need_dx and self.split_dout:
                ops.maxpool3_bwd_sums(self.dpooled, self.argmax, p.dout2, False, p.out, self.B, p.H, p.W, p.C, self.pool_sums)

        self._fork_join(None, lambda: closing(self.c1, ops._p(self.r1), b1a, ops._p(self.dr1), True),
                        lambda: closing(self.c2, ops._p(self.r2), b2a, ops._p(self.dr2), True), branch3)
        if infer:
            self.fused.backward_pointwise(x, p.C, ops._p(p.dout) if need_dx else None, need_dx)
            if need_dx and not pool_first and not self.split_dout:
                ops.maxpool_bwd(self.dpooled, self.argmax, p.dout, True, self.B, p.H, p.W, p.C, 3, 1, "SAME")
            return
        self.fused.backward(x, p.C, ops._p(p.dout) if need_dx else None, need_dx, pool=self.next if from_pool else None)
        if need_dx and self.split_dout:
            ops.bn_bwd_reduce(p.out, self._dgrad_sum_segs, self.B * p.H * p.W, p.C, eng.zeros, eng.ones, eng.zeros, self.dgrad_sums,
                              ldz=p.C)
        if need_dx and not pool_first and not self.split_dout:
            if self.pool_sums is not None:
                ops.maxpool3_bwd_sums(self.dpooled, self.argmax, p.dout, True, p.out, self.B, p.H, p.W, p.C, self.pool_sums)
            else:
                ops.maxpool_bwd(self.dpooled, self.argmax, p.dout, True, self.B, p.H, p.W, p.C, 3, 1, "SAME")


class InceptionV1Engine:

    def __init__(self, store, num_classes, image_size=224, dropout_keep_prob=0.8, trainable_bn_beta=True,
                 device="cuda", train_all=False, dtype="f32"):
        self.store, self.num_classes, self.keep = store, num_classes, dropout_keep_prob
        assert dtype in ("f32", "bf16", "fp8")
        self.dtype = dtype
        self.conv_dtype = ops.DS_DTYPE_F32 if dtype == "f32" else ops.DS_DTYPE_BF16
        self.trainable_bn_beta = trainable_bn_beta
        self.train_all = train_all
        self.device = torch.device(device)
        self.update_moving = True
        self.training = True
        self.reducer = None
        self.sync_bn = False
        self.sync_world = 1
        self.sync_group = None
        self.seed_dev = None
        self.side_mode = None
        self.one_side_stream = 1
        self.pool_first = True
        self.act16 = dtype in ("bf16", "fp8") and not train_all
        self.wgrad_side = True
        self.side_w = None
        self.wgrad_stream = None
        self.bwd_sums = True
        self.stem_direct = True
        self.stem_pool = _lib.tuning_env("DS_STEM_POOL", "1") != "0"
        self.branch_streams = True
        self.side = None
        self.fp8_everywhere = _lib.tuning_env("DS_FP8_EVERYWHERE", "0") == "1"
        self.fp8_wide_rule = _lib.tuning_env("DS_FP8_RULE", "0") == "1"
        self.bf16_direct = True
        self.wino16 = _lib.tuning_env("DS_WINO16", "1") != "0"
        self.winograd = True
        self.mul3 = _lib.tuning_env("DS_MUL3", "0") == "1"
        self.bnb_on_load = int(_lib.tuning_env("DS_BNB", "1"))
        self.zcat = _lib.tuning_env("DS_ZCAT", "1") != "0"
        self.pool_apply = _lib.tuning_env("DS_POOL_APPLY", "1") != "0"
        self.fuse_finalize = _lib.tuning_env("DS_FUSE_FIN", "0") == "1"
        self.fuse_fin_apply = _lib.tuning_env("DS_FIN_APPLY", "0") == "1"
        e = _lib.tuning_env("DS_BATCH_BN")
        self.batch_bn = int(e) if e else None
        self.pool_sums = _lib.tuning_env("DS_POOL_SUMS", "1") != "0"
        self.split_dout = _lib.tuning_env("DS_SPLIT_DOUT", "0") == "1"
        self.z16 = _lib.tuning_env("DS_Z16", "1") != "0"
        self.dpooled16 = _lib.tuning_env("DS_DPOOLED16", "0") == "1"
        self.stem_sums_from_dgrad = _lib.tuning_env("DS_STEM_SUMS", "1") != "0"
        self.dz16 = int(_lib.tuning_env("DS_DZ16", "2"))
        self.fuse_branch3 = _lib.tuning_env("DS_FUSE_B3", "1") != "0"
        self.winograd4 = _lib.tuning_env("DS_WINO4", "1") != "0"
        self.splitk = _lib.tuning_env("DS_SPLITK", "1") != "0"
        e = _lib.tuning_env("DS_TEXT_GATE")
        self.text_gate = int(e) if e else None
        self.text_gate_event = None
        self.weights_version = 0
        self.fused_infer = False
        self.fused_request = False
        self._fused_key = None
        self._fused_targets = {}
        self._fused_jobs = None
        self.input_grad = False
        self.infer_bwd = False
        self.frozen_step = False
        self._frozen_prep = None
        self._frozen_jobs = {}
        self._input_grad_training = True
        self._pivots = None
        self._restore_pivots = None
        self._stats_n = self._bwdp_n = self._ws_bytes = 0
        self.B = None
        self.alloc_gen = 0
        self.input = InputStage(self, image_size)
        self.stages = []
        prev = self.input
        for item in TOPOLOGY:
            kind, name = item[0], item[1]
            tr = train_all or name in TRAINABLE_ENDPOINTS
            bucket = 1 if tr else 2
            if kind == "conv":
                st = ConvStage(self, name, prev, item[2], item[3], item[4], tr, bucket)
            elif kind == "maxpool":
                st = PoolStage(self, name, prev, item[2], item[3])
            else:
                st = MixedStage(self, name, prev, item[2], item[3], item[4], item[5], tr, bucket)
            self.stages.append(st)
            prev = st
        self.last = prev
        for a, b in zip(self.stages[:-1], self.stages[1:]):
            a.next = b
        self.fuse_bn_pool = True
        assert self.last.H == 7 and self.last.W == 7, "AvgPool_0a_7x7 + SpatialSqueeze need a 7x7 map (224x224 input)"
        self.feat = self.last.C
        lg = "InceptionV1/Logits/Conv2d_0c_1x1"
        store.declare(lg + "/weights", (1, 1, self.feat, num_classes), True, l2=True, bucket=1)
        store.declare(lg + "/biases", (num_classes,), True, bucket=1)
        self.lg = lg
        self.layers = [l for s in self.stages for l in s.layers]

    @property
    def batch_stats(self):
        return bool(self.training and not self.frozen_step)

    @property
    def arith(self):
        if self.dtype == "f32":
            return ops.DS_ARITH_F32X3 if self.mul3 else ops.DS_ARITH_F32
        return ops.DS_ARITH_BF16 if self.dtype == "bf16" else ops.DS_ARITH_FP8
# ... 166 lines not shown

    def _frozen_prepare(self):
        if self._frozen_prep is None or self._frozen_prep[0] != self.alloc_gen:
            jobs = [(l.beta, l.mm, l.mv, l.cout, l.rstd, l.shift) for l in self.layers]
            self._frozen_prep = (self.alloc_gen, ops.BnInferJobs(jobs))
        self._frozen_prep[1].run(BN_EPS)

    def _frozen_dbeta(self, top):
        if not self.trainable_bn_beta:
            return
        key = (self.alloc_gen, top)
        jobs = self._frozen_jobs.get(key)
        if jobs is None:
            layers = [l for s in self.stages if (s.name in TRAINABLE_ENDPOINTS) == top for l in s.layers]
            assert all(l.fz_job is not None for l in layers)
            jobs = self._frozen_jobs[key] = ops.BnSumJobs([(l.fz_job[0], l.fz_job[1], l.cout, l.gbeta) for l in layers])
        jobs.run()

    def fused_report(self):
        return [(l.key, self._fused_targets[id(l)]) for l in self.layers
                if isinstance(self._fused_targets.get(id(l)), str)]

    def forward(self, images, dropout_mask=None, seed=0, input_grad=False, fused=None):
        B = images.shape[0]
        if fused is None:
            fused = self.fused_request
        if fused and (self.training or input_grad or self.dtype != "f32" or self.mul3):
            raise ValueError("the fused forward is the fp32 moving-statistics pass (is_training=False)")
        self.fused_infer = bool(fused)
        self._set_input_grad(input_grad)
        self.alloc(B)
        if self._restore_pivots is not None:
            pB, pivots = self._restore_pivots
            self._restore_pivots = None
            if pB == B:
                for l, m in zip(self.layers, pivots):
                    l.mean.copy_(m)
        if input_grad:
            self._input_grad_training = bool(self.training)
        if input_grad and self.training:
            saved = self._pivots if self._pivots is not None and self._pivots[0] == B else None
            for i, l in enumerate(self.layers):
                l.mean.copy_(saved[1][i] if saved is not None else l.mm)
        for a, b in zip(self.stages[:-1], self.stages[1:]):
            if isinstance(a, ConvStage):
                a.fused_into_pool = self.fuse_bn_pool and isinstance(b, PoolStage) and b.k == 3
                a.pool = b if a.fused_into_pool else None
        if images.dtype != torch.float32 or images.dim() != 4 or images.shape[-1] != 3:
            raise ValueError("images must be float32 NHWC [B, H, W, 3], got %s %s" % (images.dtype, tuple(images.shape)))
        if not images.is_contiguous():
            images = images.contiguous()
        self.images = images
        if self.amax_pool is not None:
            ops.fill(self.amax_pool, self._amax_next, 0.0)
        stem = self.stages[0].layer
        if not stem.stem_direct or (stem.trainable and self.training):
            ops.pad_channels(images, 3, self.input.out, 4, B * self.input.H * self.input.W)
        if self.frozen_step:
            if not self.training or input_grad or fused:
                raise ValueError("a frozen-BatchNorm step is a plain training pass")
            if self.dtype != "f32" or self.train_all or self.sync_bn:
                raise NotImplementedError("frozen-BatchNorm training is the fp32 configuration without train_all / sync_bn")
            self._frozen_prepare()
        if self.fused_infer:
            self._fused_prepare()
        else:
            self._fused_key = None
        gate = self.text_gate
        for i, s in enumerate(self.stages):
            s.forward()
            if gate is not None and i == gate:
                self.text_gate_event = torch.cuda.Event()
                self.text_gate_event.record(torch.cuda.current_stream())
        last = self.last
        ops.avgpool_dropout_fwd(last.out, B, last.H * last.W, self.feat, self.keep if self.training else 1.0, seed,
                                dropout_mask, self.mask, self.pooled, seed_dev=self.seed_dev)
        self.fc.run(ops._p(self.pooled), self.w_fc, ops._p(self.logits), bias=self.b_fc)
        return self.logits

    def backward(self, dlogits):
        B, nc, F = self.B, self.num_classes, self.feat
        last = self.last
        dl = ops._p(dlogits)
        self.fc_wgrad.run(ops._p(self.pooled), dl, self.gw_fc, ops._p(self.ws), self.ws_bytes)
        ops.colsum(dlogits, B, nc, nc, self.colsum_scratch, self.gb_fc)
        self.fc_dgrad.run(dl, self.w_fc, ops._p(self.dpooled))
        ops.avgpool_dropout_bwd(self.dpooled, self.mask, B, last.H * last.W, F, self.keep, last.dout)
        n = len(self.stages)
        stop = 0
        if not self.trainable_bn_beta:
            stop = min(i for i, s in enumerate(self.stages) if any(l.trainable for l in s.layers))
        self.wgrad_stream = self.side_w if (self.wgrad_side and self.side_w is not None) else None
        self.wgrad_pending = False
        if self.frozen_step:
            self._backward_frozen(n, stop)
            return
        self._backward_walk(n, stop)

    def _backward_frozen(self, n, stop):
        with self._pointwise_backward():
            self._backward_walk(n, stop)

    @contextlib.contextmanager
    def _pointwise_backward(self, on=True):
        plans = [l.dgrad for l in self.layers if l.dgrad is not None] if on else []
        saved_plans = [(pl.d.flags, pl.d.bnb, pl.d.mask_rstd, pl.d.mask_shift) for pl in plans]
        try:
            for pl in plans:
                pl.d.flags &= ~ops.DS_EPI_BNSUMS
                pl.d.bnb = pl.d.mask_rstd = pl.d.mask_shift = None
            self.infer_bwd = bool(on)
            yield
        finally:
            self.infer_bwd = False
            for pl, (fl, bnb, mr, ms) in zip(plans, saved_plans):
                pl.d.flags, pl.d.bnb, pl.d.mask_rstd, pl.d.mask_shift = fl, bnb, mr, ms

    def _backward_walk(self, n, stop):
        frozen = self.frozen_step
        for i in range(n - 1, stop - 1, -1):
            self.stages[i].backward(need_dx=(i > stop))
            top = self.stages[i].name in TRAINABLE_ENDPOINTS
            if frozen and top:
                self._frozen_dbeta(True)
                if self.wgrad_pending:
                    self.wgrad_stream.wait_stream(torch.cuda.current_stream())
            if self.reducer is not None and not self.train_all and top:
                if self.wgrad_pending:
                    with torch.cuda.stream(self.wgrad_stream):
                        self.reducer.stage_done(self.stages[i].name)
                else:
                    self.reducer.stage_done(self.stages[i].name)
        if frozen and stop == 0:
            self._frozen_dbeta(False)
        if self.wgrad_pending:
            torch.cuda.current_stream().wait_stream(self.wgrad_stream)
        if self.reducer is not None and self.train_all:
            self.reducer.stage_done(TRAINABLE_ENDPOINTS[0])

    def input_backward(self, dlogits, dimages, eval_mode=False):
        if not self.input_grad:
            raise RuntimeError("input_backward needs a forward pass with input_grad=True")
        if bool(eval_mode) == self._input_grad_training:
            raise RuntimeError("input_backward(eval_mode=%s) after a forward pass with training=%s" % (bool(eval_mode), self._input_grad_training))
        if eval_mode and self.dtype != "f32":
            raise NotImplementedError("the moving-statistics backward is implemented for the fp32 configuration only")
        B, F = self.B, self.feat
        if tuple(dimages.shape) != (B, self.input.H, self.input.W, 3) or dimages.dtype != torch.float32 or not dimages.is_contiguous():
            raise ValueError("dimages must be a contiguous float32 [%d, %d, %d, 3] tensor" % (B, self.input.H, self.input.W))
        last = self.last
        self.fc_dgrad.run(ops._p(dlogits), self.w_fc, ops._p(self.dpooled))
        ops.avgpool_dropout_bwd(self.dpooled, self.mask, B, last.H * last.W, F, 1.0 if eval_mode else self.keep, last.dout)
        stem = self.stages[0].layer
        if stem.dgrad is None:
            stem.make_dgrad(3)
        saved = [(l.trainable, l.gbeta) for l in self.layers]
        self.input.dout = dimages
        try:
            for l in self.layers:
                l.trainable, l.gbeta = False, None
            with self._pointwise_backward(bool(eval_mode)):
                self.wgrad_stream, self.wgrad_pending = None, False
                for s in reversed(self.stages):
                    s.backward(need_dx=True)
        finally:
            for l, (tr, gb) in zip(self.layers, saved):
                l.trainable, l.gbeta = tr, gb
            self.input.dout = None
        return dimages
```

tumblr_emotions_amd/engine_text.py:

```python
import ctypes as C

import torch

from . import _lib, ops
from .ops import WgradPlan, gemm_plan, head_gemm_plan, DS_EPI_ACCUM, DS_EPI_BIAS, DS_EPI_MASK, DS_EPI_RELU

FORGET_BIAS = 1.0


def _vp(addr):
    return C.c_void_p(addr)


def _gemm_wgrad(M, K, N, lda, lddz):
    return WgradPlan(M, 1, 1, K, lda, 1, 1, 1, N, lddz, pad_t=0, pad_l=0, OH=1, OW=1)


class TextTowerEngine:
    KERNEL = "Text/rnn/basic_lstm_cell/kernel"
    BIAS = "Text/rnn/basic_lstm_cell/bias"
    EMB = "Text/W_embedding"

    def __init__(self, store, vocab_rows, embed_dim, rnn_size, post_size, device="cuda", trainable_embedding=False):
        self.store, self.V, self.D, self.H, self.T = store, vocab_rows, embed_dim, rnn_size, post_size
        self.device = torch.device(device)
        self.trainable_embedding = trainable_embedding
        store.declare(self.EMB, (vocab_rows, embed_dim), trainable_embedding, bucket=1)
        store.declare(self.KERNEL, (embed_dim + rnn_size, 4 * rnn_size), True, bucket=1)
        store.declare(self.BIAS, (4 * rnn_size,), True, bucket=1)
        self.B = None
        self.reducer = None
        self.persistent = True
        self.seq_rows = 1
        self.sort_by_length = _lib.tuning_env("DS_LSTM_SORT", "1") != "0" 

    def alloc(self, B):
        if self.B == B:
            return
        dev, T, D, H = self.device, self.T, self.D, self.H
        self.B = B
        self.alloc_gen = getattr(self, "alloc_gen", 0) + 1
        self.use_seq = self.persistent and ops.lstm_seq_supported(B, H)
        self.sorted = bool(self.use_seq and self.sort_by_length)
        if self.sorted:
            self.perm = torch.empty(B, dtype=torch.int32, device=dev)
            self.len_sorted = torch.empty(B, dtype=torch.int64, device=dev)
            self.texts_sorted = torch.empty(B, T, dtype=torch.int64, device=dev)
            self.h_last = torch.empty(B, H, device=dev)
            self.dh_sorted = torch.empty(B, H, device=dev)
        self.seq_ws = torch.zeros(max(ops.lstm_seq_workspace(B, H) // 4, 4), dtype=torch.int32, device=dev)
        self.x = torch.empty(T * B, D, device=dev)
        self.gates = torch.empty(T, B, 4 * H, device=dev)
        self.dgates = torch.empty(T, B, 4 * H, device=dev)
        self.h = torch.zeros(T + 1, B, H, device=dev)
        self.c = torch.zeros(T + 1, B, H, device=dev)
        self.dh = [torch.empty(B, H, device=dev), torch.empty(B, H, device=dev)]
        self.dc = torch.empty(B, H, device=dev)
        st = self.store
        self.table = st.view(self.EMB)
        kptr = st.ptr(self.KERNEL)
        self.wx, self.wh = _vp(kptr), _vp(kptr + 4 * D * 4 * H)
        self.bias = _vp(st.ptr(self.BIAS))
        gk = st.grad_ptr(self.KERNEL)
        self.gwx, self.gwh = _vp(gk), _vp(gk + 4 * D * 4 * H)
        self.gbias = st.grad_view(self.BIAS)
        self.xproj = gemm_plan(T * B, D, 4 * H, D, 4 * H, 4 * H, flags=DS_EPI_BIAS)
        def nsplit(m, n, k):
            blocks = -(-m // 128) * -(-n // 32)
            return int(max(1, min(512 // max(blocks, 1), (k // 16) // 4)))
        self.sf, self.sb = nsplit(B, 4 * H, H), nsplit(B, H, 4 * H)
        self.rec_slabs = torch.empty(self.sf, B, 4 * H, device=dev)
        self.dh_slabs = torch.empty(self.sb, B, H, device=dev)
        self.rec = gemm_plan(B, H, 4 * H, H, 4 * H, 4 * H, splits=self.sf, z_split_stride=B * 4 * H)
        self.rec_dgrad = gemm_plan(B, 4 * H, H, 4 * H, H, 4 * H, transposed_w=True, splits=self.sb,
                                   z_split_stride=B * H)
        self.wgrad_x = _gemm_wgrad(T * B, D, 4 * H, D, 4 * H)
        self.wgrad_h = _gemm_wgrad(T * B, H, 4 * H, H, 4 * H)
        self.ws_bytes = max(self.wgrad_x.ws_bytes, self.wgrad_h.ws_bytes)
        self.ws = torch.empty(max(self.ws_bytes // 4, 4), device=dev)
        self.colsum_scratch = torch.empty(64 * 4 * H, device=dev)
        self.dx = None
        if self.trainable_embedding:
# ... 32 lines not shown
            if self.sorted:
                ops.permute_rows(self.h[T], self.h_last, self.perm, B, H, gather=False)
                return self.h_last
            return self.h[T]
        slab = B * 4 * H
        for t in range(T):
            ns = 0
            if t > 0:
                self.rec.run(ops._p(self.h[t]), self.wh, ops._p(self.rec_slabs))
                ns = self.sf
            ops.lstm_cell_fwd(self.gates[t], self.c[t], self.h[t], seq_lens, t, B, H, FORGET_BIAS, self.c[t + 1],
                              self.h[t + 1], self.rec_slabs, ns, slab)
        return self.h[T]

    def check_status(self):
        if self.B is not None and self.use_seq:
            ops.lstm_seq_status(self.seq_ws, self.B)

    def backward(self, dh_last):
        self._bptt(dh_last)
        self._weight_grads()

    def input_backward(self, dh_last):
        B, T, D, H = self.B, self.T, self.D, self.H
        self._bptt(dh_last)
        self._ensure_dx()
        self.x_dgrad.run(ops._p(self.dgates), self.wx, ops._p(self.dx))
        ops.token_dot(self.dx, self.x, self.seq_lens, self.tok, B, T, D)
        live = torch.arange(T, device=self.device).view(1, T) < self.seq_lens.view(B, 1)
        dwords = torch.where(live.unsqueeze(-1), self.dx.view(T, B, D).permute(1, 0, 2), self.dx.new_zeros(()))
        scores = self.tok
        if self.sorted:
            order = torch.empty_like(self.perm, dtype=torch.int64)
            order[self.perm.long()] = torch.arange(B, device=self.device)
            dwords, scores = dwords[order], scores[order]
        return dwords.contiguous(), scores.clone()

    def _bptt(self, dh_last):
        B, T, H = self.B, self.T, self.H
        if self.use_seq:
            rows = self.seq_rows
            if self.sorted:
                ops.permute_rows(dh_last, self.dh_sorted, self.perm, B, H, gather=True)
                dh_last, rows = self.dh_sorted, rows | _lib.DS_LSTM_SKIP_MASKED
            ops.lstm_seq_bwd(self.gates, self.wh, 4 * H, self.c, dh_last, dh_last.stride(0), self.seq_lens, T, B, H,
                             self.dgates, self.seq_ws, rows=rows)
            return
        dh, dh2 = self.dh
        ops.copy2d(dh_last, dh_last.stride(0), dh, H, B, H)
        ops.fill(self.dc, B * H, 0.0)
        ns = 0
        for t in range(T - 1, -1, -1):
            ops.lstm_cell_bwd(self.gates[t], self.c[t + 1], self.c[t], dh, self.dc, self.seq_lens, t, B, H,
                              self.dgates[t], self.dc, dh2, self.dh_slabs, ns, B * H)
            if t > 0:
                self.rec_dgrad.run(ops._p(self.dgates[t]), self.wh, ops._p(self.dh_slabs))
                ns = self.sb
            dh, dh2 = dh2, dh

    def _weight_grads(self):
        B, T, H = self.B, self.T, self.H
        dg = ops._p(self.dgates)
        self.wgrad_x.run(ops._p(self.x), dg, self.gwx, ops._p(self.ws), self.ws_bytes)
        self.wgrad_h.run(ops._p(self.h), dg, self.gwh, ops._p(self.ws), self.ws_bytes)
        ops.colsum(self.dgates, T * B, 4 * H, 4 * H, self.colsum_scratch, self.gbias)
        if self.trainable_embedding:
            self.x_dgrad.run(dg, self.wx, ops._p(self.dx))
            ops.embedding_grad(self.dx, self.texts, self.gtable, B, T, self.D, time_major=True)
        if self.reducer is not None:
            self.reducer.stage_done("text")


class JointHeadEngine:

    def __init__(self, store, im_size, tx_size, fc_size, nb_emotions, device="cuda"):
        self.store, self.im, self.tx, self.fc, self.nc = store, im_size, tx_size, fc_size, nb_emotions
        self.device = torch.device(device)
        store.declare("W_fc", (im_size + tx_size, fc_size), True, bucket=1)
        store.declare("b_fc", (fc_size,), True, bucket=1)
        store.declare("W_softmax", (fc_size, nb_emotions), True, bucket=1)
        store.declare("b_softmax", (nb_emotions,), True, bucket=1)
        self.B = None
        self.reducer = None

    def alloc(self, B):
        if self.B == B:
            return
        dev, im, tx, fc, nc = self.device, self.im, self.tx, self.fc, self.nc
        self.B = B
        self.alloc_gen = getattr(self, "alloc_gen", 0) + 1
        self.dense = torch.empty(B, fc, device=dev)
        self.ddense = torch.empty(B, fc, device=dev)
        self.logits = torch.empty(B, nc, device=dev)
        self.d_im = torch.empty(B, im, device=dev)
        self.d_tx = torch.empty(B, tx, device=dev)
        st = self.store
        w = st.ptr("W_fc")
        self.w_im, self.w_tx = _vp(w), _vp(w + 4 * im * fc)
        gw = st.grad_ptr("W_fc")
        self.gw_im, self.gw_tx = _vp(gw), _vp(gw + 4 * im * fc)
        self.b_fc, self.gb_fc = _vp(st.ptr("b_fc")), st.grad_view("b_fc")
        self.w_sm, self.gw_sm = _vp(st.ptr("W_softmax")), _vp(st.grad_ptr("W_softmax"))
        self.b_sm, self.gb_sm = _vp(st.ptr("b_softmax")), st.grad_view("b_softmax")
        self.fc_im = None
        self.ws_bytes = 0
        self.colsum_scratch = torch.empty(64 * max(fc, nc), device=dev)

    def _plans(self, ld_im, ld_tx):
        B, im, tx, fc, nc = self.B, self.im, self.tx, self.fc, self.nc
        self.fc_im = head_gemm_plan(B, im, fc, ld_im, fc, fc, device=self.device)
        self.fc_tx = head_gemm_plan(B, tx, fc, ld_tx, fc, fc, flags=DS_EPI_ACCUM | DS_EPI_BIAS | DS_EPI_RELU, device=self.device)
        self.sm = head_gemm_plan(B, fc, nc, fc, nc, nc, flags=DS_EPI_BIAS, device=self.device)
        self.sm_dgrad = head_gemm_plan(B, nc, fc, nc, fc, nc, transposed_w=True, flags=DS_EPI_MASK, ldmask=fc, device=self.device)
        self.sm_wgrad = _gemm_wgrad(B, fc, nc, fc, nc)
        self.im_dgrad = head_gemm_plan(B, fc, im, fc, im, fc, transposed_w=True, device=self.device)
        self.tx_dgrad = head_gemm_plan(B, fc, tx, fc, tx, fc, transposed_w=True, device=self.device)
        self.im_wgrad = _gemm_wgrad(B, im, fc, ld_im, fc)
        self.tx_wgrad = _gemm_wgrad(B, tx, fc, ld_tx, fc)
        self.ws_bytes = max(p.ws_bytes for p in (self.sm_wgrad, self.im_wgrad, self.tx_wgrad))
        self.ws = torch.empty(max(self.ws_bytes // 4, 4), device=self.device)
        self._lds = (ld_im, ld_tx)

    def forward(self, im_feat, tx_feat):
        B = im_feat.shape[0]
        self.alloc(B)
        lds = (im_feat.stride(0), tx_feat.stride(0))
        if self.fc_im is None or self._lds != lds:
            self._plans(*lds)
        self.im_feat, self.tx_feat = im_feat, tx_feat
        self.fc_im.run(ops._p(im_feat), self.w_im, ops._p(self.dense))
        self.fc_tx.run(ops._p(tx_feat), self.w_tx, ops._p(self.dense), bias=self.b_fc)
        self.sm.run(ops._p(self.dense), self.w_sm, ops._p(self.logits), bias=self.b_sm)
        return self.logits

    def backward(self, dlogits):
        B, fc, nc = self.B, self.fc, self.nc
        dl, ws = ops._p(dlogits), ops._p(self.ws)
        self.sm_wgrad.run(ops._p(self.dense), dl, self.gw_sm, ws, self.ws_bytes)
        ops.colsum(dlogits, B, nc, nc, self.colsum_scratch, self.gb_sm)
        self.sm_dgrad.run(dl, self.w_sm, ops._p(self.ddense), mask=ops._p(self.dense))
        dd = ops._p(self.ddense)
        self.im_wgrad.run(ops._p(self.im_feat), dd, self.gw_im, ws, self.ws_bytes)
        self.tx_wgrad.run(ops._p(self.tx_feat), dd, self.gw_tx, ws, self.ws_bytes)
        ops.colsum(self.ddense, B, fc, fc, self.colsum_scratch, self.gb_fc)
        self.im_dgrad.run(dd, self.w_im, ops._p(self.d_im))
        self.tx_dgrad.run(dd, self.w_tx, ops._p(self.d_tx))
        if self.reducer is not None:
            self.reducer.stage_done("head")
        return self.d_im, self.d_tx

    def input_backward(self, dlogits, with_text=False):
        self.sm_dgrad.run(ops._p(dlogits), self.w_sm, ops._p(self.ddense), mask=ops._p(self.dense))
        self.im_dgrad.run(ops._p(self.ddense), self.w_im, ops._p(self.d_im))
        if with_text:
            self.tx_dgrad.run(ops._p(self.ddense), self.w_tx, ops._p(self.d_tx))
            return self.d_im, self.d_tx
        return self.d_im


class TextHeadEngine:

    def __init__(self, store, rnn_size, nb_emotions, device="cuda"):
        self.store, self.H, self.nc = store, rnn_size, nb_emotions
        self.device = torch.device(device)
        store.declare("W_softmax", (rnn_size, nb_emotions), True, bucket=1)
        store.declare("b_softmax", (nb_emotions,), True, bucket=1)
        self.B = None
        self.reducer = None

    def alloc(self, B):
        if self.B == B:
            return
        dev, H, nc = self.device, self.H, self.nc
        self.B = B
        self.alloc_gen = getattr(self, "alloc_gen", 0) + 1
        self.logits = torch.empty(B, nc, device=dev)
        self.d_tx = torch.empty(B, H, device=dev)
        st = self.store
        self.w_sm, self.gw_sm = _vp(st.ptr("W_softmax")), _vp(st.grad_ptr("W_softmax"))
        self.b_sm, self.gb_sm = _vp(st.ptr("b_softmax")), st.grad_view("b_softmax")
        self.sm = head_gemm_plan(B, H, nc, H, nc, nc, flags=DS_EPI_BIAS, device=self.device)
        self.sm_dgrad = head_gemm_plan(B, nc, H, nc, H, nc, transposed_w=True, device=self.device)
        self.sm_wgrad = _gemm_wgrad(B, H, nc, H, nc)
        self.ws_bytes = self.sm_wgrad.ws_bytes
        self.ws = torch.empty(max(self.ws_bytes // 4, 4), device=dev)
        self.colsum_scratch = torch.empty(64 * max(nc, 4), device=dev)

    def forward(self, tx_feat):
        self.alloc(tx_feat.shape[0])
        assert tx_feat.stride(0) == self.H
        self.tx_feat = tx_feat
        self.sm.run(ops._p(tx_feat), self.w_sm, ops._p(self.logits), bias=self.b_sm)
        return self.logits

    def backward(self, dlogits):
        dl = ops._p(dlogits)
        self.sm_wgrad.run(ops._p(self.tx_feat), dl, self.gw_sm, ops._p(self.ws), self.ws_bytes)
        ops.colsum(dlogits, self.B, self.nc, self.nc, self.colsum_scratch, self.gb_sm)
        self.sm_dgrad.run(dl, self.w_sm, ops._p(self.d_tx))
        if self.reducer is not None:
            self.reducer.stage_done("head")
        return self.d_tx

    def input_backward(self, dlogits):
        self.sm_dgrad.run(ops._p(dlogits), self.w_sm, ops._p(self.d_tx))
        return self.d_tx
```

tumblr_emotions_amd/net.py:

```python
import math

import numpy as np
import torch

from . import ops
from .engine_image import InceptionV1Engine, WEIGHT_DECAY
from .engine_text import JointHeadEngine, TextHeadEngine, TextTowerEngine
from .functions import (InceptionV1Function, JointHeadFunction, SoftmaxCrossEntropyFunction, TextHeadFunction,
                        TextTowerFunction)
from .dp import GradientReducer
from .params import ParamStore

ADAM_B1, ADAM_B2, ADAM_EPS = 0.9, 0.999, 1e-8


class SentimentNet:
    def __init__(self, mode="joint", nb_emotions=15, im_features_size=256, rnn_size=512, fc_size=512,
                 vocab_size=10000, embedding_dim=300, post_size=32, image_size=224, dropout_keep_prob=0.8,
                 trainable_bn_beta=True, device="cuda", process_group=None, overlap_comm=True,
                 concurrent_towers=True, train_all=False, trainable_embedding=False, dtype="f32",
                 force_dp_buckets=False, sync_bn=False, frozen_bn=False):
        assert mode in ("joint", "image", "text")
        self.dtype = dtype
        self.frozen_bn = bool(frozen_bn)
        if self.frozen_bn:
            if mode == "text":
                raise ValueError("frozen_bn: mode 'text' has no BatchNorm")
            if sync_bn:
                raise ValueError("frozen_bn with sync_bn: fixed statistics leave nothing to synchronise")
            if dtype != "f32":
                raise NotImplementedError("frozen_bn is implemented for the fp32 configuration, not %r" % dtype)
            if train_all:
                raise NotImplementedError("frozen_bn with train_all is not implemented")
        if not torch.cuda.is_available():
            raise RuntimeError("tumblr_emotions_amd needs an MI355X (HIP) device: the training path has no CPU fallback")
        self.mode, self.nb_emotions, self.device = mode, nb_emotions, torch.device(device)
        self.store = ParamStore(device)
        self.image = self.text = self.head = None
        if mode in ("joint", "image"):
            nc = im_features_size if mode == "joint" else nb_emotions
            self.image = InceptionV1Engine(self.store, nc, image_size, dropout_keep_prob, trainable_bn_beta, device,
                                           train_all=train_all, dtype=dtype)
        if mode in ("joint", "text"):
            self.text = TextTowerEngine(self.store, vocab_size + 1, embedding_dim, rnn_size, post_size, device,
                                        trainable_embedding=trainable_embedding)
        if mode == "joint":
            self.head = JointHeadEngine(self.store, im_features_size, rnn_size, fc_size, nb_emotions, device)
        elif mode == "text":
            self.head = TextHeadEngine(self.store, rnn_size, nb_emotions, device)
        self.store.finalize()
        st = self.store
        self.leaves = {e.name: st.view(e.name).detach().requires_grad_() for e in st.entries.values() if e.trainable}
        if self.image is not None:
            self.image_param_names = [n for n in self.leaves if n.startswith("InceptionV1/")]
            self.image.param_names = self.image_param_names
            self.image_params = [self.leaves[n] for n in self.image_param_names]
        self.step = 0
        self.frozen_l2_sumsq = 0.0
        self.loss_buf = torch.zeros(1, device=self.device)
        self.l2_buf = torch.zeros(1, device=self.device)
        self.l2_scratch = torch.zeros(256, device=self.device)
        self.lr_t_dev = torch.zeros(1, device=self.device)
        self.seed_dev = torch.zeros(1, dtype=torch.int64, device=self.device)
        self.dlogits = None
        self.pg = process_group
        from . import streams
        streams.reserve(self.device)
        self.text_stream = streams.get("text", self.device) if (mode == "joint" and concurrent_towers) else None
        if self.text_stream is not None:
            self.text.seq_rows = 8
        self.reducer = GradientReducer(st.grad, st.n_bucket1, process_group, overlap_comm,
                                       force_buckets=force_dp_buckets)
        self.world = self.reducer.world
        self.reducer.expect(*[n for n, e in (("Mixed_5c", self.image), ("text", self.text), ("head", self.head))
                              if e is not None])
        for e in (self.image, self.text, self.head):
            if e is not None:
                e.reducer = self.reducer
        self.sync_bn = bool(sync_bn and self.world > 1 and self.image is not None)
        self.sync_bn_requested = bool(sync_bn)
        if self.sync_bn:
            if dtype != "f32":
                raise ValueError("sync_bn is implemented for the fp32 configuration")
            self.image.sync_bn, self.image.sync_world, self.image.sync_group = True, self.world, process_group
        self.logits = None
        self._graph = None
        self._graph_key = None

    def initialize(self, seed=1):
        rng = np.random.RandomState(seed)
        sd = {}

        def trunc(shape, std):
            a = rng.standard_normal(size=shape)
            bad = np.abs(a) > 2
            while bad.any():
                a[bad] = rng.standard_normal(size=int(bad.sum()))
                bad = np.abs(a) > 2
            return (a * std).astype(np.float32)

        def glorot(shape):
            fi, fo = (shape[0], shape[0]) if len(shape) == 1 else (int(np.prod(shape[:-1])), shape[-1])
            lim = math.sqrt(6.0 / (fi + fo))
            return rng.uniform(-lim, lim, size=shape).astype(np.float32)

        for e in self.store.entries.values():
            n, shp = e.name, e.shape
            if n.endswith("/weights") and "/Logits/" in n:
                v = trunc(shp, math.sqrt(1.3 * 2.0 / (shp[0] * shp[1] * shp[2])))
            elif n.endswith("/weights"):
                v = trunc(shp, 0.01)
                if shp[2] == 4 and shp[0] == 7:
                    v[:, :, 3, :] = 0
            elif n.endswith("moving_variance"):
                v = np.ones(shp, np.float32)
            elif n.endswith("beta") or n.endswith("moving_mean") or n.endswith("/biases") or n.endswith("cell/bias"):
                v = np.zeros(shp, np.float32)
            elif n == "Text/W_embedding":
                v = rng.normal(0, 0.4, size=shp).astype(np.float32)
                v[-1] = 0
            else:
                v = glorot(shp)
            self.store.view(n).copy_(torch.from_numpy(v))
        self.after_load()

    def load_state_dict(self, sd, strict=True):
        sd = dict(sd)
        k = "InceptionV1/Conv2d_1a_7x7/weights"
        if k in sd and np.asarray(sd[k]).shape[2] == 3:
            w = np.zeros((7, 7, 4, 64), np.float32)
# ... 187 lines not shown
        for b in range(B):
            sub = {}
            if has_im:
                x, x0 = x_all[b:b + 1], x0_all[b:b + 1]
                sub["images"] = (x0 + alpha.view(steps, 1, 1, 1) * (x - x0)).contiguous()
            if has_tx:
                sub["texts"] = batch["texts"][b:b + 1].expand(steps, -1).contiguous()
                sub["seq_lens"] = batch["seq_lens"][b:b + 1].expand(steps).contiguous()
            _, dimg, dwords, _ = self.eval_gradients(sub, target[b:b + 1].expand(steps, -1).contiguous(),
                                                    text_scale=alpha if has_tx else None)
            if has_im:
                im_attr[b] = (x_all[b] - x0_all[b]) * dimg.mean(0)
            if has_tx:
                words = self.text.table[batch["texts"][b]]
                tok_attr[b] = (words * dwords.mean(0)).sum(-1)
        idx = torch.arange(2 * B, device=self.device)
        f = torch.empty(2 * B, device=self.device)
        for i in range(0, 2 * B, steps):
            take = idx[i:i + steps]
            pad = torch.cat([take, take[-1:].expand(steps - take.shape[0])])
            post, at_x = pad % B, pad >= B
            ends = {}
            if has_im:
                ends["images"] = torch.where(at_x.view(-1, 1, 1, 1), x_all[post], x0_all[post]).contiguous()
            if has_tx:
                ends["texts"], ends["seq_lens"] = batch["texts"][post].contiguous(), batch["seq_lens"][post].contiguous()
            lg, _, _, _ = self.eval_gradients(ends, target[post].contiguous(), text_scale=at_x.float() if has_tx else None)
            f[take] = (lg * target[post]).sum(1)[:take.shape[0]]
        delta = f[B:] - f[:B]
        return im_attr, tok_attr, delta

    def cross_entropy(self, logits, labels):
        if self.dlogits is None or self.dlogits.shape != logits.shape:
            self.dlogits = torch.empty(logits.shape, device=self.device)
        return SoftmaxCrossEntropyFunction.apply(logits, labels, self.loss_buf, self.dlogits)

    def total_loss_value(self):
        reg = 0.0
        if self.store.n_l2 > 0 or self.frozen_l2_sumsq:
            reg = 0.5 * WEIGHT_DECAY * (self.frozen_l2_sumsq + float(self.l2_buf.item()))
        if getattr(self, "_clone_count", 1) > 1:
            ce = 0.0
            for x in self.clone_loss.cpu().tolist():
                ce += x
            ce /= self._clone_count
        else:
            ce = float(self.loss_buf.item())
        loss = ce + reg
        self.check_status()
        return loss

    def check_status(self):
        if self.text is not None:
            torch.cuda.synchronize(self.device)
            self.text.check_status()

    def _rank_seed(self, seed):
        return int(seed) * 4096 + self.reducer.rank

    def train_step(self, batch, lr, dropout_mask=None, seed=None, num_clones=1, after_clone=None):
        if type(num_clones) is not int or num_clones != 1:
            return self._train_step_clones(batch, lr, dropout_mask, seed, num_clones, after_clone)
        self._clone_count = 1
        st = self.store
        self.step += 1
        t = self.step
        if self.image is not None:
            self.image.invalidate_fused()
        lr_t = lr * math.sqrt(1.0 - ADAM_B2 ** t) / (1.0 - ADAM_B1 ** t)
        seed = self._rank_seed(self.step) if seed is None else seed
        if self._graph is not None:
            if self._graph_key == self._batch_key(batch, dropout_mask):
                self.seed_dev.fill_(seed)
                self.lr_t_dev.fill_(lr_t)
                self._graph.replay()
                return self.loss_buf.view(())
            if self._graph_key[-2:] != self._batch_key(batch, dropout_mask)[-2:]:
                self.release_graph()
        for p in self.leaves.values():
            p.grad = None
        if self.frozen_bn:
            self.image.frozen_step = True
        try:
            logits = self.forward(batch, dropout_mask, seed)
            ce = self.cross_entropy(logits, batch["labels"])
            if st.n_l2 > 0:
                ops.sumsq(st.theta, st.n_l2, self.l2_scratch, self.l2_buf)
            self.reducer.begin_step()
            ce.backward()
        finally:
            if self.frozen_bn:
                self.image.frozen_step = False
        grad_scale = self.reducer.finish()
        ops.adam_tf(st.theta, st.grad, st.m, st.v, st.n_trainable_padded, st.n_l2, WEIGHT_DECAY, grad_scale, lr_t,
                    ADAM_B1, ADAM_B2, ADAM_EPS)
        return ce

    def check_clones(self, num_clones, batch_rows=None, seed=None):
        K = num_clones
        if isinstance(K, bool) or not isinstance(K, (int, np.integer)) or K < 1:
            raise ValueError("num_clones must be a positive int, not %r" % (K,))
        K = int(K)
        if K == 1:
            return K
        if self.sync_bn_requested:
            raise ValueError("num_clones = %d with sync_bn: clones have their own BatchNorm statistics by definition" % K)
        if self.dtype != "f32":
            raise NotImplementedError("num_clones = %d with dtype %r: clones are implemented for the fp32 configuration"
                                      % (K, self.dtype))
        if self._graph is not None:
            raise NotImplementedError("num_clones = %d with a captured step: release_graph() first, a step of several "
                                      "clones is not captured" % K)
        if seed is not None:
            raise ValueError("num_clones = %d with an explicit seed: every clone draws its own dropout stream" % K)
        if K * self.world > 4096:
            raise ValueError("num_clones * world = %d exceeds the 4096 dropout streams of a step" % (K * self.world))
        if batch_rows is not None and batch_rows % K != 0:
            raise ValueError("num_clones = %d does not divide the batch of %d rows" % (K, batch_rows))
        return K

    @staticmethod
    def _clone_rows(t, lo, hi):
        v = t[lo:hi]
        return v if v.data_ptr() % 16 == 0 and v.is_contiguous() else v.clone(memory_format=torch.contiguous_format)

    def _train_step_clones(self, batch, lr, dropout_mask, seed, num_clones, after_clone):
        B = int(batch["labels"].shape[0])
        K = self.check_clones(num_clones, B, seed)
        if K == 1:
            return self.train_step(batch, lr, dropout_mask=dropout_mask, seed=seed)
        st = self.store
        b = B // K
        nc = self.nb_emotions
        if getattr(self, "grad_acc", None) is None:
            self.grad_acc = torch.zeros_like(st.grad)
        if getattr(self, "clone_loss", None) is None or self.clone_loss.shape[0] != K:
            self.clone_loss = torch.zeros(K, device=self.device)
        if getattr(self, "clone_logits", None) is None or tuple(self.clone_logits.shape) != (B, nc):
            self.clone_logits = torch.empty(B, nc, device=self.device)
        self.step += 1
        t = self.step
        if self.image is not None:
            self.image.invalidate_fused()
        lr_t = lr * math.sqrt(1.0 - ADAM_B2 ** t) / (1.0 - ADAM_B1 ** t)
        if self.frozen_bn:
            self.image.frozen_step = True
        try:
            self.reducer.begin_step(defer=True)
            for c in range(K):
                lo, hi = c * b, (c + 1) * b
                sub = {k: self._clone_rows(v, lo, hi) for k, v in batch.items()}
                mask = None if dropout_mask is None else self._clone_rows(dropout_mask, lo, hi)
                clone_seed = int(self.step) * 4096 + self.reducer.rank * K + c
                for p in self.leaves.values():
                    p.grad = None
                if self.image is not None:
                    self.image.update_moving = c == 0
                logits = self.forward(sub, mask, clone_seed)
                if self.dlogits is None or self.dlogits.shape != logits.shape:
                    self.dlogits = torch.empty(logits.shape, device=self.device)
                ce = SoftmaxCrossEntropyFunction.apply(logits, sub["labels"], self.clone_loss[c:c + 1], self.dlogits)
                if c == 0 and st.n_l2 > 0:
                    ops.sumsq(st.theta, st.n_l2, self.l2_scratch, self.l2_buf)
                ce.backward()
                self.clone_logits[lo:hi].copy_(logits.detach())
                ops.grad_accumulate(self.grad_acc, st.grad, st.n_trainable_padded, 0 if c == 0 else (2 if c == K - 1 else 1))
                if after_clone is not None:
                    after_clone(c)
        finally:
            if self.image is not None:
                self.image.update_moving = True
            if self.frozen_bn:
                self.image.frozen_step = False
        self.reducer.finish()
        self.logits = self.clone_logits
        self._clone_count = K
        ops.adam_tf(st.theta, st.grad, st.m, st.v, st.n_trainable_padded, st.n_l2, WEIGHT_DECAY, 1.0 / (self.world * K), lr_t,
                    ADAM_B1, ADAM_B2, ADAM_EPS)
        return self.clone_loss

    def _batch_key(self, batch, dropout_mask):
        gen = tuple(getattr(e, "alloc_gen", 0) for e in (self.image, self.text, self.head) if e is not None)
        wv = self.image.weights_version if self.image is not None else 0
        return tuple(sorted((k, v.data_ptr(), tuple(v.shape)) for k, v in batch.items())) + (
            None if dropout_mask is None else dropout_mask.data_ptr(), gen, wv)

    def _step_kernels(self, batch, dropout_mask):
        st = self.store
        main = torch.cuda.current_stream()
        side = self.text_stream if (self.image is not None and self.text is not None) else None
        im = tx = None
        if side is not None:
            ready = torch.cuda.Event()
            ready.record(main)
        if self.image is not None:
            im = self.image.forward(batch["images"], dropout_mask, 0)
        if self.text is not None:
            if side is not None:
                side.wait_event(ready)
                with torch.cuda.stream(side):
                    tx = self.text.forward(batch["texts"], batch["seq_lens"])
                main.wait_stream(side)
            else:
                tx = self.text.forward(batch["texts"], batch["seq_lens"])
        if self.mode == "image":
            logits = im
        elif self.mode == "text":
            logits = self.head.forward(tx)
        else:
            logits = self.head.forward(im, tx)
        self.logits = logits
        if self.dlogits is None or self.dlogits.shape != logits.shape:
            raise RuntimeError("capture_step: run one eager train_step with this batch size first")
        B, C_ = logits.shape
        ops.softmax_ce(logits, batch["labels"], B, C_, 1.0, None, self.loss_buf, self.dlogits)
        if st.n_l2 > 0:
            ops.sumsq(st.theta, st.n_l2, self.l2_scratch, self.l2_buf)
        if self.mode == "image":
            self.image.backward(self.dlogits)
        elif self.mode == "text":
            self.text.backward(self.head.backward(self.dlogits))
        else:
            d_im, d_tx = self.head.backward(self.dlogits)
            if side is not None:
                side.wait_stream(main)
                with torch.cuda.stream(side):
                    self.text.backward(d_tx)
                self.image.backward(d_im)
                main.wait_stream(side)
            else:
                self.text.backward(d_tx)
                self.image.backward(d_im)

    def capture_step(self, batch, dropout_mask=None, num_clones=1):
        if type(num_clones) is not int or num_clones != 1:
            if self.check_clones(num_clones) > 1:
                raise NotImplementedError("capture_step with num_clones = %d: a step of several clones is not captured"
                                          % num_clones)
        if self.frozen_bn:
            raise NotImplementedError("capture_step is not implemented for a frozen_bn net")
        if self.reducer.active:
            return False
        st = self.store
        keep = [b.clone() for b in (st.theta, st.m, st.v, st.frozen)]
        if self.image is not None and self.image.B != batch["images"].shape[0]:
            self.image.alloc(batch["images"].shape[0])
        if self.image is not None:
            im = self.image
            im.one_side_stream = im.side_arrangement(im.side_mode, im.B, im.dtype, capturing=True)
        pivots = [] if self.image is None else [l.mean for l in self.image.layers]
        keep_pivots = [m.clone() for m in pivots]
        self.train_step(batch, 0.0, dropout_mask)
        self.step -= 1
        for b, k in zip((st.theta, st.m, st.v, st.frozen), keep):
            b.copy_(k)
        for m, k in zip(pivots, keep_pivots):
            m.copy_(k)
        if self.image is not None:
            self.image.seed_dev = self.seed_dev
        torch.cuda.synchronize()
        g = torch.cuda.CUDAGraph()
        with torch.cuda.graph(g):
            self._step_kernels(batch, dropout_mask)
            ops.adam_tf(st.theta, st.grad, st.m, st.v, st.n_trainable_padded, st.n_l2, WEIGHT_DECAY, 1.0, 0.0,
                        ADAM_B1, ADAM_B2, ADAM_EPS, lr_t_dev=self.lr_t_dev)
        self._graph, self._graph_key = g, self._batch_key(batch, dropout_mask)
        return True

    def release_graph(self):
        self._graph = self._graph_key = None
        if self.image is not None:
            self.image.seed_dev = None
            im = self.image
            if im.B is not None:
                im.one_side_stream = im.side_arrangement(im.side_mode, im.B, im.dtype)
```

tumblr_emotions_amd/ops.py:

```python
import ctypes as C
import os

import torch

from . import _lib
from ._lib import (ConvDesc, Segments, SumSegments, DS_EPI_ACCUM, DS_EPI_BIAS, DS_EPI_BNSUMS, DS_EPI_MASK, DS_EPI_RELU,
                   DS_EPI_STATS, DS_EPI_BN_RELU,
                   DS_DTYPE_BF16, DS_DTYPE_F32, DS_FP8_E4M3, DS_FP8_E5M2, DS_CONV_FWD, DS_CONV_DGRAD, DS_ARITH_F32, DS_ARITH_BF16,
                   DS_ARITH_FP8, DS_ARITH_F32X3, DS_FAM_IGEMM, DS_FAM_WINO2, DS_FAM_WINO4, DS_FAM_STEM, DS_FAM_BF16D, DS_FAM_FP8D,
                   DS_FAM_F32X3, DS_FAM_WINO4H, DS_FAM_STEM_POOL, DS_FAM_STEM_DGRAD, DS_PLAN_STEM_POOL, DS_PLAN_NO_SPLITK, DS_PLAN_NO_WINO4H, DS_PLAN_NO_WINO, DS_PLAN_NO_WINO4, DS_PLAN_NO_STEM_DIRECT, DS_PLAN_NO_BF16_DIRECT, DS_PLAN_ACT16,
                   DS_PLAN_PACKED_RGB, DS_PLAN_FP8_EVERYWHERE, DS_PLAN_FP8_WIDE_RULE)


_raw_stream = getattr(torch._C, "_cuda_getCurrentRawStream", None)


def _stream():
    if _raw_stream is not None:
        return C.c_void_p(_raw_stream(torch.cuda.current_device()))
    return C.c_void_p(torch.cuda.current_stream().cuda_stream)


def _p(t):
    if t is None:
# ... 53 lines not shown

    def enable_bnsums(self, ldy):
        if not _lib.load().ds_conv_igemm_bnsums_supported(C.byref(self.d)):
            return 0
        self.d.partials = 0
        self.d.flags |= DS_EPI_BNSUMS
        self.d.ldmask = ldy
        self.partials = _lib.load().ds_conv_igemm_partials(C.byref(self.d))
        self.d.partials = self.partials
        return self.partials

    def run(self, x, w, z, bias=None, mask=None, stats=None, pivot=None):
        t = CONV_TIMER
        if t is not None:
            t.begin()
        _lib.check(_lib.load().ds_conv_igemm(C.byref(self.d), x, w, z, bias, mask, stats, pivot, _stream()),
                   "ds_conv_igemm")
        if t is not None:
            t.end(self)


class ConvTimer:

    def __init__(self):
        self.records = []
        self._start = None

    def begin(self):
        self._start = torch.cuda.Event(enable_timing=True)
        self._start.record(torch.cuda.current_stream())

    def end(self, plan):
        e = torch.cuda.Event(enable_timing=True)
        e.record(torch.cuda.current_stream())
        d = getattr(plan, "d", None)
        pooled = getattr(plan, "family", None) == DS_FAM_STEM_POOL or bool(getattr(d, "pool_argmax", None))
        self.records.append((self._start, e, plan.alg_flops, pooled))

    def summary(self, pooled=None):
        recs = [r for r in self.records if pooled is None or r[3] == pooled]
        ms = sum(s.elapsed_time(e) for (s, e, _, _) in recs)
        return len(recs), ms, sum(f for (_, _, f, _) in recs)


CONV_TIMER = None


def head_gemm_plan(M, K, N, lda, ldc, w_ld, transposed_w=False, flags=0, ldmask=0, *, device):
    if M <= 512 and K >= 256 and _lib.tuning_env("DS_SPLIT_GEMM", "1") != "0":
        return SplitGemm(M, K, N, lda, ldc, w_ld, transposed_w, flags, ldmask, 8 if K >= 512 else 4, device)
    return gemm_plan(M, K, N, lda, ldc, w_ld, transposed_w=transposed_w, flags=flags, ldmask=ldmask)


def gemm_plan(M, K, N, lda, ldc, w_ld, transposed_w=False, flags=0, ldmask=0, splits=1, z_split_stride=0,
              dtype=DS_DTYPE_F32):
    if transposed_w:
        return ConvPlan(M, 1, 1, K, lda, 1, 1, 1, N, ldc, 0, w_ld, 1, flags=flags, ldmask=ldmask,
                        pad_t=0, pad_l=0, OH=1, OW=1, splits=splits, z_split_stride=z_split_stride, dtype=dtype)
    return ConvPlan(M, 1, 1, K, lda, 1, 1, 1, N, ldc, 0, 1, w_ld, flags=flags, ldmask=ldmask,
                    pad_t=0, pad_l=0, OH=1, OW=1, splits=splits, z_split_stride=z_split_stride, dtype=dtype)


class SplitGemm:

    def __init__(self, M, K, N, lda, ldc, w_ld, transposed_w, flags, ldmask, splits, device):
        self.M, self.N, self.ldc, self.flags, self.ldmask, self.splits = M, N, ldc, flags, ldmask, splits
        self.slabs = torch.empty(splits, M, N, device=device)
        self.plan = gemm_plan(M, K, N, lda, N, w_ld, transposed_w=transposed_w, splits=splits, z_split_stride=M * N)
        self.d, self.alg_flops, self.partials = self.plan.d, self.plan.alg_flops, 0

    def run(self, x, w, z, bias=None, mask=None, stats=None, pivot=None):
        if stats is not None or pivot is not None:
            raise ValueError("SplitGemm has no BatchNorm-statistics epilogue (the heads' GEMMs are not followed by BatchNorm)")
        t = CONV_TIMER
        if t is not None:
            t.begin()
        lib = _lib.load()
        _lib.check(lib.ds_conv_igemm(C.byref(self.plan.d), x, w, _p(self.slabs), None, None, None, None, _stream()),
                   "ds_conv_igemm")
        _lib.check(lib.ds_slab_epilogue(_p(self.slabs), self.splits, self.M * self.N, self.N, self.M, self.N, z, self.ldc,
                                        bias, mask, self.ldmask, self.flags, _stream()), "ds_slab_epilogue")
        if t is not None:
            t.end(self)


class WinoPlan:

    def __init__(self, N, H, W, Cin, ldx, Cout, ldz, flags=0, f4=False):
        self.args = (N, H, W, Cin, ldx, Cout, ldz)
        self.flags = flags
        self.f4 = bool(f4)
        lib = _lib.load()
        self._run, self._name = (lib.ds_conv_wino4, "ds_conv_wino4") if f4 else (lib.ds_conv_wino, "ds_conv_wino")
        self._partials = lib.ds_conv_wino4_partials if f4 else lib.ds_conv_wino_partials
        self.u_elems = (36 if f4 else 16) * Cin * Cout
        self.M = N * H * W
        self.partials = self._partials(N, H, W) if flags & (DS_EPI_STATS | DS_EPI_BNSUMS) else 0
        self.alg_flops = 2.0 * self.M * Cout * 9 * Cin

    def enable_bnsums(self):
        N, H, W = self.args[:3]
        self.flags = (self.flags & ~DS_EPI_STATS) | DS_EPI_BNSUMS
        self.partials = self._partials(N, H, W)
        return self.partials

    def set_ldx(self, ldx):
        self.args = self.args[:4] + (ldx,) + self.args[5:]

    def set_ldz(self, ldz):
        self.args = self.args[:6] + (ldz,)

    def run(self, x, u, z, stats=None, pivot=None, ymask=None):
        t = CONV_TIMER
        if t is not None:
            t.begin()
        N, H, W, Cin, ldx, Cout, ldz = self.args
        _lib.check(self._run(x, u, z, stats, pivot, ymask, N, H, W, Cin, ldx, Cout, ldz, self.flags, _stream()), self._name)
        if t is not None:
            t.end(self)


class LayerPlan:

    def __init__(self, role, arith, options, N, H, W, w_cin, w_cout, k, stride, ldx, ldz, flags=0):
        self.p = _lib.LayerPlanStruct()
        _lib.check(_lib.load().ds_conv_plan(C.byref(self.p), role, arith, options, N, H, W, w_cin, w_cout, k, stride, ldx,
                                            ldz, flags), "ds_conv_plan")
        self.d = self.p.d
        self.family = self.p.family
        self.M = N * self.d.OH * self.d.OW
        self.alg_flops = self.p.alg_flops
        self.u = None
        self.wscale = None
        self.io = _lib.ConvIO()
        self.ws_bytes = int(self.p.ws_bytes)
        self.splitk = int(self.p.splitk)
        self._ws = None
        self._run = _lib.load().ds_conv_run
        self._ref = C.byref(self.p)
        self._io_ref = C.byref(self.io)

    @property
    def partials(self):
        return self.p.partials

    @property
    def x16_ok(self):
        return bool(self.p.x16_ok)

    def alloc_weights(self, device):
        if self.p.w_bytes:
            self.u = torch.empty(self.p.w_bytes, dtype=torch.uint8, device=device)
        if self.p.wscale_floats:
            self.wscale = torch.zeros(self.p.wscale_floats, device=device)
            self.io.wscale = self.wscale.data_ptr()

    def set_workspace(self, t):
        assert t.numel() * t.element_size() >= self.ws_bytes
        self._ws = t
        self.io.ws, self.io.ws_bytes = t.data_ptr(), t.numel() * t.element_size()

    def prepare(self, w_hwio):
        if self.u is not None:
            _lib.check(_lib.load().ds_conv_prepare_weights(self._ref, w_hwio, _p(self.u), _p(self.wscale), _stream()),
                       "ds_conv_prepare_weights")

# ... 1142 lines not shown
```

Baseline: 19780 samples/s.

## Group head split-K GEMMs into single launches and fuse epilogue with softmax-CE

Adds a grouped GEMM kernel that runs up to four small plain split-K GEMMs of the joint head in one launch, plus a grouped slab-combine epilogue and a slab-epilogue fused with softmax cross-entropy. Head weight gradients and the L2 sum-of-squares term are moved onto a side stream and joined before the optimizer. The aim is to cut kernel launch count and serialization in the small head layers, at the cost of extra stream synchronization and more complex bookkeeping.

```diff
diff --git a/include/ds_kernels.h b/include/ds_kernels.h
--- a/include/ds_kernels.h
+++ b/include/ds_kernels.h
@@ -418,6 +418,29 @@
 int ds_colsum(const float *x, int64_t M, int32_t C, int32_t ld, float *scratch, float *out, void *stream);
 int ds_slab_epilogue(const float *slabs, int32_t splits, int64_t slab_stride, int32_t lds, int64_t M, int32_t N, float *out,
                      int32_t ldo, const float *bias, const float *mask, int32_t ldmask, int32_t flags, void *stream);
+
+int ds_gemm_group(const ds_conv_desc *const *descs, const float *const *x, const float *const *w, float *const *z,
+                  int32_t count, void *stream);
+typedef struct ds_slab_combine {
+    const float *slabs;
+    const float *pre_slabs;
+    int64_t slab_stride, pre_slab_stride;
+    int64_t M;
+    int32_t N;
+    int32_t splits, pre_splits;
+    int32_t lds, pre_lds;
+    int32_t flags;
+    float *out;
+    float *out2;
+    int32_t ldo, ldo2, n_split;
+    int32_t ldmask;
+    const float *bias;
+    const float *mask;
+} ds_slab_combine;
+int ds_slab_epilogue_group(const ds_slab_combine *ops, int32_t count, void *stream);
+int ds_slab_epilogue_ce(const float *slabs, int32_t splits, int64_t slab_stride, int32_t lds, int32_t M, int32_t N,
+                        float *logits, const float *bias, const int64_t *labels, float grad_scale,
+                        const float *grad_scale_dev, float *loss, float *dlogits, void *stream);
 int ds_copy2d(const float *src, int32_t lds, float *dst, int32_t ldd, int64_t rows, int32_t cols,
               void *stream);
 int ds_pad_channels(const float *src, int32_t cs, float *dst, int32_t cd, int64_t pixels, void *stream);
diff --git a/tumblr_emotions_amd/_lib.py b/tumblr_emotions_amd/_lib.py
--- a/tumblr_emotions_amd/_lib.py
+++ b/tumblr_emotions_amd/_lib.py
@@ -90,6 +90,13 @@
     _fields_ = [("nseg", C.c_int32), ("c_begin", C.c_int32 * 4), ("c_end", C.c_int32 * 4), ("P", C.c_int32 * 4),
                 ("kind", C.c_int32 * 4), ("s", C.c_void_p * 4), ("q", C.c_void_p * 4), ("P2", C.c_int32 * 4),
                 ("s2", C.c_void_p * 4), ("q2", C.c_void_p * 4)]
+
+
+class SlabCombine(C.Structure):
+    _fields_ = [("slabs", C.c_void_p), ("pre_slabs", C.c_void_p), ("slab_stride", C.c_int64), ("pre_slab_stride", C.c_int64),
+                ("M", C.c_int64), ("N", C.c_int32), ("splits", C.c_int32), ("pre_splits", C.c_int32), ("lds", C.c_int32),
+                ("pre_lds", C.c_int32), ("flags", C.c_int32), ("out", C.c_void_p), ("out2", C.c_void_p), ("ldo", C.c_int32),
+                ("ldo2", C.c_int32), ("n_split", C.c_int32), ("ldmask", C.c_int32), ("bias", C.c_void_p), ("mask", C.c_void_p)]
 
 
 class PreprocessDesc(C.Structure):
@@ -256,6 +263,9 @@
     "ds_sumsq": (C.c_int, [_P, _i64, _P, _P, _P]),
     "ds_colsum": (C.c_int, [_P, _i64, _i32, _i32, _P, _P, _P]),
     "ds_slab_epilogue": (C.c_int, [_P, _i32, _i64, _i32, _i64, _i32, _P, _i32, _P, _P, _i32, _i32, _P]),
+    "ds_gemm_group": (C.c_int, [C.POINTER(_CD), C.POINTER(_P), C.POINTER(_P), C.POINTER(_P), _i32, _P]),
+    "ds_slab_epilogue_group": (C.c_int, [C.POINTER(SlabCombine), _i32, _P]),
+    "ds_slab_epilogue_ce": (C.c_int, [_P, _i32, _i64, _i32, _i32, _i32, _P, _P, _P, _f32, _P, _P, _P, _P]),
     "ds_copy2d": (C.c_int, [_P, _i32, _P, _i32, _i64, _i32, _P]),
     "ds_pad_channels": (C.c_int, [_P, _i32, _P, _i32, _i64, _P]),
     "ds_fill": (C.c_int, [_P, _i64, _f32, _P]),
diff --git a/tumblr_emotions_amd/csrc/conv_igemm.hip b/tumblr_emotions_amd/csrc/conv_igemm.hip
--- a/tumblr_emotions_amd/csrc/conv_igemm.hip
+++ b/tumblr_emotions_amd/csrc/conv_igemm.hip
@@ -44,21 +44,22 @@
 struct TileId {
     int row, col, stride;
 };
-__device__ __forceinline__ TileId tile_id(const ConvParams &p) {
+__device__ __forceinline__ TileId tile_id(const ConvParams &p, int bx, int by, int gx) {
     TileId t;
     if (p.col_tiles > 0) {
-        const int id = blockIdx.x;
-        const int lin = (id & 7) * (int)(gridDim.x >> 3) + (id >> 3);
+        const int id = bx;
+        const int lin = (id & 7) * (gx >> 3) + (id >> 3);
         t.row = lin / p.col_tiles;
         t.col = lin - t.row * p.col_tiles;
         t.stride = p.row_tiles;
     } else {
-        t.row = blockIdx.x;
-        t.col = blockIdx.y;
-        t.stride = gridDim.x;
+        t.row = bx;
+        t.col = by;
+        t.stride = gx;
     }
     return t;
 }
+__device__ __forceinline__ TileId tile_id(const ConvParams &p) { return tile_id(p, (int)blockIdx.x, (int)blockIdx.y, (int)gridDim.x); }
 
 template <bool VEC>
 __device__ __forceinline__ f32x4 load4(__amdgpu_buffer_rsrc_t r, unsigned off, bool ok, int valid) {
@@ -73,16 +74,21 @@
     }
 }
 
+template <int MT, int NT, bool BNMAJOR>
+constexpr int igemm_smem_floats() {
+    return 2 * (4 * MT * 32) * LDK + 2 * (BNMAJOR ? BK * (NT * 32 + 4) : NT * 32 * LDK);
+}
+
 template <int MT, int NT, bool BNMAJOR, bool FOLD, bool VEC, bool BNR = false>
-__global__ __launch_bounds__(256, (MT == 1 && NT == 1) ? 4 : (MT == 1 && NT == 2) ? 3 : 1) void conv_igemm_kernel(
-    const ConvParams p) {
+__device__ __forceinline__ void igemm_workgroup(const ConvParams &p, float *smem, const TileId tid0, const int split,
+                                                const int nsplits, const int wg_seq) {
     constexpr int WM = 4;
     constexpr int BM = WM * MT * 32, BN = NT * 32;
     constexpr int AR = BM / 64;
     constexpr int BR = (BN * 4 + 255) / 256;
     constexpr int LDB = BNMAJOR ? (BN + 4) : LDK;
     constexpr int BSZ = BNMAJOR ? BK * LDB : BN * LDK;
-    __shared__ __attribute__((aligned(16))) float smem[2 * BM * LDK + 2 * BSZ];
+    static_assert(igemm_smem_floats<MT, NT, BNMAJOR>() == 2 * BM * LDK + 2 * BSZ, "LDS size");
     float *As = smem;
     float *Bs = smem + 2 * BM * LDK;
 
@@ -90,20 +96,19 @@
     const int tid = threadIdx.x, lane = tid & 63;
     const int wm = __builtin_amdgcn_readfirstlane(tid >> 6);
     const int li = lane & 31, lk = lane >> 5;
-    const TileId tid0 = tile_id(p);
     const int n0 = tid0.col * BN;
     const int ohw = d.OH * d.OW;
     const int chunks = (d.Cin + BK - 1) / BK;
     const int KT_all = p.taps * chunks;
-    const int kts = (KT_all + (int)gridDim.z - 1) / (int)gridDim.z;
-    const int kt0 = (int)blockIdx.z * kts;
+    const int kts = (KT_all + nsplits - 1) / nsplits;
+    const int kt0 = split * kts;
     const int KT = (kt0 + kts < KT_all ? kt0 + kts : KT_all) - kt0;
-    float *const zout = p.z + (int64_t)blockIdx.z * p.d.z_split_stride;
+    float *const zout = p.z + (int64_t)split * p.d.z_split_stride;
     const int flags = d.flags;
     const __amdgpu_buffer_rsrc_t srd_x = make_srd(p.x, p.x_bytes);
     const __amdgpu_buffer_rsrc_t srd_w = make_srd(p.w, p.w_bytes);
 
-    switch (p.prio_mode ? ((blockIdx.x + blockIdx.y * gridDim.x + blockIdx.z * gridDim.x * gridDim.y) >> 8) & 3 : 0) {
+    switch (p.prio_mode ? (wg_seq >> 8) & 3 : 0) {
         case 1: __builtin_amdgcn_s_setprio(1); break;
         case 2: __builtin_amdgcn_s_setprio(2); break;
         case 3: __builtin_amdgcn_s_setprio(3); break;
@@ -337,6 +342,46 @@
             p.stats[(int64_t)(n0 + tid) * tid0.stride + tid0.row] = s;
             p.stats[((int64_t)d.Cout + n0 + tid) * tid0.stride + tid0.row] = q;
         }
+    }
+}
+
+template <int MT, int NT, bool BNMAJOR, bool FOLD, bool VEC, bool BNR = false>
+__global__ __launch_bounds__(256, (MT == 1 && NT == 1) ? 4 : (MT == 1 && NT == 2) ? 3 : 1) void conv_igemm_kernel(
+    const ConvParams p) {
+    __shared__ __attribute__((aligned(16))) float smem[igemm_smem_floats<MT, NT, BNMAJOR>()];
+    igemm_workgroup<MT, NT, BNMAJOR, FOLD, VEC, BNR>(
+        p, smem, tile_id(p), (int)blockIdx.z, (int)gridDim.z,
+        (int)(blockIdx.x + blockIdx.y * gridDim.x + blockIdx.z * gridDim.x * gridDim.y));
+}
+
+constexpr int kGemmGroupMax = 4;
+struct GemmGroupParams {
+    ConvParams p[kGemmGroupMax];
+    int wg_end[kGemmGroupMax];
+    int gx[kGemmGroupMax], gy[kGemmGroupMax], splits[kGemmGroupMax];
+    int variant[kGemmGroupMax];
+    int count;
+};
+
+__global__ __launch_bounds__(256, 4) void gemm_group_kernel(const GemmGroupParams g) {
+    constexpr int kSmem = igemm_smem_floats<1, 1, true>() > igemm_smem_floats<1, 1, false>() ? igemm_smem_floats<1, 1, true>()
+                                                                                              : igemm_smem_floats<1, 1, false>();
+    __shared__ __attribute__((aligned(16))) float smem[kSmem];
+    const int id = (int)blockIdx.x;
+    int q = 0;
+    while (q + 1 < g.count && id >= g.wg_end[q]) ++q;
+    const int local = id - (q ? g.wg_end[q - 1] : 0);
+    const int gx = g.gx[q], gxy = gx * g.gy[q];
+    const int split = local / gxy;
+    const int by = (local - split * gxy) / gx;
+    const int bx = local - split * gxy - by * gx;
+    const ConvParams &p = g.p[q];
+    const TileId t = tile_id(p, bx, by, gx);
+    switch (g.variant[q]) {
+        case 0: igemm_workgroup<1, 1, false, false, false>(p, smem, t, split, g.splits[q], local); break;
+        case 1: igemm_workgroup<1, 1, true, false, false>(p, smem, t, split, g.splits[q], local); break;
+        case 2: igemm_workgroup<1, 1, false, false, true>(p, smem, t, split, g.splits[q], local); break;
+        default: igemm_workgroup<1, 1, true, false, true>(p, smem, t, split, g.splits[q], local); break;
     }
 }
 
@@ -2217,6 +2262,15 @@
 }
 
 namespace {
+int xcd_remap_on() {
+    static int xcd_remap = -1;
+    if (xcd_remap < 0) {
+        const char *e = ds::tune_env("DS_CONV_XCD_REMAP");
+        xcd_remap = e ? atoi(e) : 1;
+    }
+    return xcd_remap;
+}
+
 int igemm_launch(const ds_conv_desc *d, const float *x, const float *w, float *z, const float *bias, const float *mask,
                  float *stats, const float *pivot, const float *scale, const float *shift, void *stream) {
     DS_REQUIRE(d && x && w && z, "ds_conv_igemm: null argument");
@@ -2280,11 +2334,7 @@
                "ds_conv_igemm: the launch would write %d statistics partials but the plan was made for %d "
                "(a ds_debug_conv_set_* switch changed after planning?)", c.direct ? gx * 4 : gx, d->partials);
     p.row_tiles = rt;
-    static int xcd_remap = -1;
-    if (xcd_remap < 0) {
-        const char *e = ds::tune_env("DS_CONV_XCD_REMAP");
-        xcd_remap = e ? atoi(e) : 1;
-    }
+    const int xcd_remap = xcd_remap_on();
     dim3 grid(gx, gy, splits);
     p.col_tiles = 0;
     if (one && (c.wide || (xcd_remap && gy > 1)) && !c.direct) {
@@ -2327,6 +2377,60 @@
     else hipLaunchKernelGGL(bnr ? bnr_kernel(c) : kernel_for(c, v), grid, dim3(256), 0, (hipStream_t)stream, p);
     return ds::check_launch("ds_conv_igemm");
 }
+}
+
+extern "C" int ds_gemm_group(const ds_conv_desc *const *descs, const float *const *x, const float *const *w, float *const *z,
+                             int32_t count, void *stream) {
+    DS_REQUIRE(descs && x && w && z && count >= 1 && count <= kGemmGroupMax, "ds_gemm_group: 1..%d problems", kGemmGroupMax);
+    GemmGroupParams g{};
+    g.count = count;
+    int wgs = 0;
+    for (int i = 0; i < count; ++i) {
+        const ds_conv_desc *d = descs[i];
+        DS_REQUIRE(d && x[i] && w[i] && z[i], "ds_gemm_group: null argument (problem %d)", i);
+        DS_REQUIRE(d->Cin > 0 && d->Cout > 0 && d->N > 0 && d->KH == 1 && d->KW == 1 && d->stride == 1 && d->H == 1 && d->W == 1 &&
+                       d->OH == 1 && d->OW == 1 && d->pad_t == 0 && d->pad_l == 0 && d->fold_cin == 0 && d->flip == 0,
+                   "ds_gemm_group: problem %d is not a plain GEMM", i);
+        DS_REQUIRE(d->dtype == DS_DTYPE_F32 && d->flags == 0 && !d->bnb && !d->fin && !d->norm_rstd && !d->norm_shift &&
+                       !d->mask_rstd && !d->mask_shift && !d->pool_argmax,
+                   "ds_gemm_group: problem %d: fp32 without epilogue flags or on-load operands (combine with ds_slab_epilogue_group)", i);
+        DS_REQUIRE(d->w_n_stride == 1 || d->w_k_stride == 1, "ds_gemm_group: one weight stride must be 1");
+        DS_REQUIRE(d->ldx >= d->Cin && d->ldz >= d->Cout, "ds_gemm_group: problem %d: row strides below the row lengths", i);
+        const int splits = d->splits > 1 ? d->splits : 1;
+        DS_REQUIRE(splits == 1 || d->z_split_stride >= (int64_t)(d->N - 1) * d->ldz + d->Cout,
+                   "ds_gemm_group: problem %d: overlapping output slabs", i);
+        const Variant v = variant_of(d, x[i], w[i]);
+        const TileCfg c = pick_cfg(d, v.vec);
+        DS_REQUIRE(c.mt == 1 && c.nt == 1 && !c.direct && !c.glds && !c.bf16 && !c.wide,
+                   "ds_gemm_group: problem %d's own launch is not the 128 x 32 tile (run it through ds_conv_igemm)", i);
+        ConvParams &p = g.p[i];
+        p.d = *d;
+        if (splits == 1) p.d.z_split_stride = 0;
+        p.x = x[i]; p.w = w[i]; p.z = z[i];
+        p.M = d->N;
+        p.taps = 1;
+        const int64_t x_elems = (int64_t)(d->N - 1) * d->ldx + d->Cin;
+        const int64_t w_elems = (int64_t)(d->Cout - 1) * d->w_n_stride + (int64_t)(d->Cin - 1) * d->w_k_stride + 1;
+        DS_REQUIRE(x_elems * 4 < (1ll << 31) && w_elems * 4 < (1ll << 31), "ds_gemm_group: operand larger than 2 GiB");
+        p.x_bytes = (unsigned)(x_elems * 4);
+        p.w_bytes = (unsigned)(w_elems * 4);
+        int gx, gy, rt;
+        bool one;
+        grid_for(d, c, v, &gx, &gy, &rt, &one);
+        p.row_tiles = rt;
+        if (one && xcd_remap_on() && gy > 1) {
+            p.col_tiles = gy;
+            gx = (rt * gy + 7) / 8 * 8;
+            gy = 1;
+        }
+        g.gx[i] = gx; g.gy[i] = gy; g.splits[i] = splits;
+        g.variant[i] = (v.bnmajor ? 1 : 0) | (v.vec ? 2 : 0);
+        DS_REQUIRE((int64_t)wgs + (int64_t)gx * gy * splits < (1 << 20), "ds_gemm_group: too many workgroups");
+        wgs += gx * gy * splits;
+        g.wg_end[i] = wgs;
+    }
+    hipLaunchKernelGGL(gemm_group_kernel, dim3(wgs), dim3(256), 0, (hipStream_t)stream, g);
+    return ds::check_launch("ds_gemm_group");
 }
 
 namespace {
diff --git a/tumblr_emotions_amd/csrc/text_misc.hip b/tumblr_emotions_amd/csrc/text_misc.hip
--- a/tumblr_emotions_amd/csrc/text_misc.hip
+++ b/tumblr_emotions_amd/csrc/text_misc.hip
@@ -199,10 +199,9 @@
     }
 }
 
-__global__ __launch_bounds__(256) void softmax_ce_kernel(const float *logits, const int64_t *labels, int B, int C,
-                                                         float grad_scale, const float *grad_scale_dev,
-                                                         float *loss, float *dlogits) {
-    __shared__ float red[256];
+__device__ __forceinline__ void softmax_ce_workgroup(const float *logits, const int64_t *labels, int B, int C,
+                                                     float grad_scale, const float *grad_scale_dev,
+                                                     float *loss, float *dlogits, float *red) {
     if (grad_scale_dev) grad_scale *= grad_scale_dev[0];
     float acc = 0.f;
     for (int b = threadIdx.x; b < B; b += 256) {
@@ -228,6 +227,13 @@
         __syncthreads();
     }
     if (threadIdx.x == 0 && loss) loss[0] = red[0] / (float)B;
+}
+
+__global__ __launch_bounds__(256) void softmax_ce_kernel(const float *logits, const int64_t *labels, int B, int C,
+                                                         float grad_scale, const float *grad_scale_dev,
+                                                         float *loss, float *dlogits) {
+    __shared__ float red[256];
+    softmax_ce_workgroup(logits, labels, B, C, grad_scale, grad_scale_dev, loss, dlogits, red);
 }
 
 __global__ __launch_bounds__(256) void adam_tf_kernel(float *theta, const float *g, float *m, float *v, int64_t n,
@@ -611,6 +617,95 @@
     return ds::check_launch("ds_slab_epilogue");
 }
 
+constexpr int kCombineMax = 4;
+struct SlabCombineParams {
+    ds_slab_combine op[kCombineMax];
+    int wg_end[kCombineMax];
+    int count;
+};
+
+__global__ __launch_bounds__(256) void slab_epilogue_group_kernel(const SlabCombineParams g) {
+    const int id = (int)blockIdx.x;
+    int q = 0;
+    while (q + 1 < g.count && id >= g.wg_end[q]) ++q;
+    const int wg0 = q ? g.wg_end[q - 1] : 0;
+    const ds_slab_combine &c = g.op[q];
+    const int64_t total = c.M * c.N, step = (int64_t)(g.wg_end[q] - wg0) * 256;
+    const int N = c.N, flags = c.flags;
+    for (int64_t i = (int64_t)(id - wg0) * 256 + threadIdx.x; i < total; i += step) {
+        const int64_t m = i / N;
+        const int n = (int)(i - m * N);
+        float v = 0.f;
+        for (int k = 0; k < c.splits; ++k) v += c.slabs[(int64_t)k * c.slab_stride + m * c.lds + n];
+        if (flags & DS_EPI_BIAS) v += c.bias[n];
+        float *const o = (c.out2 && n >= c.n_split) ? c.out2 + m * c.ldo2 + (n - c.n_split) : c.out + m * c.ldo + n;
+        if (flags & DS_EPI_ACCUM) {
+            if (c.pre_slabs) {
+                float u = 0.f;
+                for (int k = 0; k < c.pre_splits; ++k) u += c.pre_slabs[(int64_t)k * c.pre_slab_stride + m * c.pre_lds + n];
+                v += u;
+            } else {
+                v += *o;
+            }
+        }
+        if (flags & DS_EPI_MASK) v = c.mask[m * c.ldmask + n] > 0.f ? v : 0.f;
+        if (flags & DS_EPI_RELU) v = fmaxf(v, 0.f);
+        *o = v;
+    }
+}
+
+extern "C" int ds_slab_epilogue_group(const ds_slab_combine *ops, int32_t count, void *stream) {
+    DS_REQUIRE(ops && count >= 1 && count <= kCombineMax, "ds_slab_epilogue_group: 1..%d combines", kCombineMax);
+    SlabCombineParams g{};
+    g.count = count;
+    int wgs = 0;
+    for (int i = 0; i < count; ++i) {
+        const ds_slab_combine &c = ops[i];
+        DS_REQUIRE(c.slabs && c.out && c.splits >= 1 && c.M > 0 && c.N > 0 && c.lds >= c.N, "ds_slab_epilogue_group: bad argument (combine %d)", i);
+        DS_REQUIRE((c.flags & ~(DS_EPI_BIAS | DS_EPI_ACCUM | DS_EPI_MASK | DS_EPI_RELU)) == 0 && (!(c.flags & DS_EPI_BIAS) || c.bias) &&
+                       (!(c.flags & DS_EPI_MASK) || (c.mask && c.ldmask >= c.N)),
+                   "ds_slab_epilogue_group: flags are BIAS / ACCUM / MASK / RELU (with their operands)");
+        DS_REQUIRE(!c.pre_slabs || ((c.flags & DS_EPI_ACCUM) && c.pre_splits >= 1 && c.pre_lds >= c.N),
+                   "ds_slab_epilogue_group: pre_slabs is the DS_EPI_ACCUM operand (pre_splits >= 1, pre_lds >= N)");
+        if (c.out2)
+            DS_REQUIRE(c.n_split > 0 && c.n_split < c.N && c.ldo >= c.n_split && c.ldo2 >= c.N - c.n_split,
+                       "ds_slab_epilogue_group: out2 takes columns [n_split, N), 0 < n_split < N");
+        else
+            DS_REQUIRE(c.ldo >= c.N, "ds_slab_epilogue_group: ldo below N (combine %d)", i);
+        g.op[i] = c;
+        wgs += ds::stream_grid(c.M * c.N, 256);
+        g.wg_end[i] = wgs;
+    }
+    hipLaunchKernelGGL(slab_epilogue_group_kernel, dim3(wgs), dim3(256), 0, (hipStream_t)stream, g);
+    return ds::check_launch("ds_slab_epilogue_group");
+}
+
+__global__ __launch_bounds__(256) void slab_epilogue_ce_kernel(const float *slabs, int splits, int64_t slab_stride, int lds,
+                                                               int M, int N, float *logits, const float *bias,
+                                                               const int64_t *labels, float grad_scale,
+                                                               const float *grad_scale_dev, float *loss, float *dlogits) {
+    __shared__ float red[256];
+    for (int m = threadIdx.x; m < M; m += 256) {
+        for (int n = 0; n < N; ++n) {
+            float v = 0.f;
+            for (int k = 0; k < splits; ++k) v += slabs[(int64_t)k * slab_stride + (int64_t)m * lds + n];
+            if (bias) v += bias[n];
+            logits[(int64_t)m * N + n] = v;
+        }
+    }
+    softmax_ce_workgroup(logits, labels, M, N, grad_scale, grad_scale_dev, loss, dlogits, red);
+}
+
+extern "C" int ds_slab_epilogue_ce(const float *slabs, int32_t splits, int64_t slab_stride, int32_t lds, int32_t M, int32_t N,
+                                   float *logits, const float *bias, const int64_t *labels, float grad_scale,
+                                   const float *grad_scale_dev, float *loss, float *dlogits, void *stream) {
+    DS_REQUIRE(slabs && logits && labels && splits >= 1 && lds >= N, "ds_slab_epilogue_ce: bad argument");
+    DS_REQUIRE(M > 0 && M <= 512 && N > 0 && N <= 32, "ds_slab_epilogue_ce: M <= 512 rows of N <= 32 logits (packed, row stride N)");
+    hipLaunchKernelGGL(slab_epilogue_ce_kernel, dim3(1), dim3(256), 0, (hipStream_t)stream, slabs, splits, slab_stride, lds, M, N,
+                       logits, bias, labels, grad_scale, grad_scale_dev, loss, dlogits);
+    return ds::check_launch("ds_slab_epilogue_ce");
+}
+
 extern "C" int ds_copy2d(const float *src, int32_t lds, float *dst, int32_t ldd, int64_t rows, int32_t cols,
                          void *stream) {
     DS_REQUIRE(src && dst && rows > 0 && cols > 0, "ds_copy2d: bad argument");
diff --git a/tumblr_emotions_amd/engine_image.py b/tumblr_emotions_amd/engine_image.py
--- a/tumblr_emotions_amd/engine_image.py
+++ b/tumblr_emotions_amd/engine_image.py
@@ -1107,6 +1107,9 @@
         self.wgrad_side = True
         self.side_w = None
         self.wgrad_stream = None
+        self.head_group = _lib.tuning_env("DS_HEAD_GROUP", "1") != "0"
+        self.head_grads_pending = False
+        self.side_job = None
         self.bwd_sums = True
         self.stem_direct = True
         self.stem_pool = _lib.tuning_env("DS_STEM_POOL", "1") != "0"
@@ -1439,16 +1442,35 @@
         B, nc, F = self.B, self.num_classes, self.feat
         last = self.last
         dl = ops._p(dlogits)
-        self.fc_wgrad.run(ops._p(self.pooled), dl, self.gw_fc, ops._p(self.ws), self.ws_bytes)
-        ops.colsum(dlogits, B, nc, nc, self.colsum_scratch, self.gb_fc)
-        self.fc_dgrad.run(dl, self.w_fc, ops._p(self.dpooled))
-        ops.avgpool_dropout_bwd(self.dpooled, self.mask, B, last.H * last.W, F, self.keep, last.dout)
+        self.wgrad_stream = self.side_w if (self.wgrad_side and self.side_w is not None) else None
+        self.wgrad_pending = bool(self.head_grads_pending) and self.wgrad_stream is not None
+        self.head_grads_pending = False
+        job, self.side_job = self.side_job, None
+        if self.head_group and self.wgrad_stream is not None:
+            ev = torch.cuda.Event()
+            ev.record(torch.cuda.current_stream())
+            self.fc_dgrad.run(dl, self.w_fc, ops._p(self.dpooled))
+            ops.avgpool_dropout_bwd(self.dpooled, self.mask, B, last.H * last.W, F, self.keep, last.dout)
+            self.wgrad_stream.wait_event(ev)
+            if not torch.cuda.is_current_stream_capturing():
+                dlogits.record_stream(self.wgrad_stream)
+            with torch.cuda.stream(self.wgrad_stream):
+                self.fc_wgrad.run(ops._p(self.pooled), dl, self.gw_fc, ops._p(self.ws_set[3]), self.ws_bytes)
+                ops.colsum(dlogits, B, nc, nc, self.colsum_scratch, self.gb_fc)
+                if job is not None:
+                    job()
+            self.wgrad_pending = True
+        else:
+            self.fc_wgrad.run(ops._p(self.pooled), dl, self.gw_fc, ops._p(self.ws), self.ws_bytes)
+            ops.colsum(dlogits, B, nc, nc, self.colsum_scratch, self.gb_fc)
+            self.fc_dgrad.run(dl, self.w_fc, ops._p(self.dpooled))
+            ops.avgpool_dropout_bwd(self.dpooled, self.mask, B, last.H * last.W, F, self.keep, last.dout)
+            if job is not None:
+                job()
         n = len(self.stages)
         stop = 0
         if not self.trainable_bn_beta:
             stop = min(i for i, s in enumerate(self.stages) if any(l.trainable for l in s.layers))
-        self.wgrad_stream = self.side_w if (self.wgrad_side and self.side_w is not None) else None
-        self.wgrad_pending = False
         if self.frozen_step:
             self._backward_frozen(n, stop)
             return
diff --git a/tumblr_emotions_amd/engine_text.py b/tumblr_emotions_amd/engine_text.py
--- a/tumblr_emotions_amd/engine_text.py
+++ b/tumblr_emotions_amd/engine_text.py
@@ -1,3 +1,4 @@
+import contextlib
 import ctypes as C
 
 import torch
@@ -196,6 +197,11 @@
         store.declare("b_softmax", (nb_emotions,), True, bucket=1)
         self.B = None
         self.reducer = None
+        self.group = _lib.tuning_env("DS_HEAD_GROUP", "1") != "0"
+        self.image = None
+        self.async_grads = False
+        self.side_job = None
+        self.fwd_group = None
 
     def alloc(self, B):
         if self.B == B:
@@ -216,7 +222,7 @@
         self.b_fc, self.gb_fc = _vp(st.ptr("b_fc")), st.grad_view("b_fc")
         self.w_sm, self.gw_sm = _vp(st.ptr("W_softmax")), _vp(st.grad_ptr("W_softmax"))
         self.b_sm, self.gb_sm = _vp(st.ptr("b_softmax")), st.grad_view("b_softmax")
-        self.fc_im = None
+        self.fc_im = self.fwd_group = None
         self.ws_bytes = 0
         self.colsum_scratch = torch.empty(64 * max(fc, nc), device=dev)
 
@@ -234,22 +240,53 @@
         self.ws_bytes = max(p.ws_bytes for p in (self.sm_wgrad, self.im_wgrad, self.tx_wgrad))
         self.ws = torch.empty(max(self.ws_bytes // 4, 4), device=self.device)
         self._lds = (ld_im, ld_tx)
-
-    def forward(self, im_feat, tx_feat):
+        self.fwd_group = self.bwd_group = self.fc_dgrad = None
+        if all(isinstance(p, ops.SplitGemm) for p in (self.fc_im, self.fc_tx, self.im_dgrad, self.tx_dgrad)):
+            self.fwd_group = ops.GemmGroup([self.fc_im, self.fc_tx], [ops.slab_combine(
+                self.fc_tx, self.dense.data_ptr(), fc, flags=DS_EPI_ACCUM | DS_EPI_BIAS | DS_EPI_RELU, bias=self.b_fc.value,
+                pre=self.fc_im)])
+            self.fc_dgrad = head_gemm_plan(B, fc, im + tx, fc, im + tx, fc, transposed_w=True, device=self.device)
+            self.bwd_group = ops.GemmGroup([self.fc_dgrad], [ops.slab_combine(
+                self.fc_dgrad, self.d_im.data_ptr(), im, out2=self.d_tx.data_ptr(), ldo2=tx, n_split=im)])
+
+    def grouped(self):
+        return bool(self.group) and self.fwd_group is not None
+
+    def forward(self, im_feat, tx_feat, ce=None):
         B = im_feat.shape[0]
         self.alloc(B)
         lds = (im_feat.stride(0), tx_feat.stride(0))
         if self.fc_im is None or self._lds != lds:
             self._plans(*lds)
         self.im_feat, self.tx_feat = im_feat, tx_feat
-        self.fc_im.run(ops._p(im_feat), self.w_im, ops._p(self.dense))
-        self.fc_tx.run(ops._p(tx_feat), self.w_tx, ops._p(self.dense), bias=self.b_fc)
-        self.sm.run(ops._p(self.dense), self.w_sm, ops._p(self.logits), bias=self.b_sm)
+        if self.grouped():
+            self.fwd_group.run((ops._p(im_feat), ops._p(tx_feat)), (self.w_im, self.w_tx))
+        else:
+            self.fc_im.run(ops._p(im_feat), self.w_im, ops._p(self.dense))
+            self.fc_tx.run(ops._p(tx_feat), self.w_tx, ops._p(self.dense), bias=self.b_fc)
+        if ce is not None:
+            if not self.ce_fused():
+                raise ValueError("JointHeadEngine.forward(ce=...) needs the grouped chain (ce_fused())")
+            ops.split_gemm_ce(self.sm, ops._p(self.dense), self.w_sm, self.logits, self.b_sm, *ce)
+        else:
+            self.sm.run(ops._p(self.dense), self.w_sm, ops._p(self.logits), bias=self.b_sm)
         return self.logits
+
+    def ce_fused(self):
+        return self.grouped() and isinstance(self.sm, ops.SplitGemm) and self.B <= 512 and self.nc <= 32
+
+    def _grad_stream(self):
+        im = self.image
+        if not self.async_grads or im is None or not im.wgrad_side or im.side_w is None:
+            return None
+        return im.side_w
 
     def backward(self, dlogits):
         B, fc, nc = self.B, self.fc, self.nc
         dl, ws = ops._p(dlogits), ops._p(self.ws)
+        job, self.side_job = self.side_job, None
+        if self.grouped():
+            return self._backward_grouped(dlogits, job)
         self.sm_wgrad.run(ops._p(self.dense), dl, self.gw_sm, ws, self.ws_bytes)
         ops.colsum(dlogits, B, nc, nc, self.colsum_scratch, self.gb_sm)
         self.sm_dgrad.run(dl, self.w_sm, ops._p(self.ddense), mask=ops._p(self.dense))
@@ -259,8 +296,38 @@
         ops.colsum(self.ddense, B, fc, fc, self.colsum_scratch, self.gb_fc)
         self.im_dgrad.run(dd, self.w_im, ops._p(self.d_im))
         self.tx_dgrad.run(dd, self.w_tx, ops._p(self.d_tx))
+        if job is not None:
+            job()
         if self.reducer is not None:
             self.reducer.stage_done("head")
+        return self.d_im, self.d_tx
+
+    def _backward_grouped(self, dlogits, job):
+        B, fc, nc = self.B, self.fc, self.nc
+        dl, ws = ops._p(dlogits), ops._p(self.ws)
+        self.sm_dgrad.run(dl, self.w_sm, ops._p(self.ddense), mask=ops._p(self.dense))
+        dd = ops._p(self.ddense)
+        side = self._grad_stream()
+        if side is not None:
+            ev = torch.cuda.Event()
+            ev.record(torch.cuda.current_stream())
+        self.bwd_group.run((dd,), (self.w_im,))
+        if side is not None:
+            side.wait_event(ev)
+            if not torch.cuda.is_current_stream_capturing():
+                dlogits.record_stream(side)
+        with (torch.cuda.stream(side) if side is not None else contextlib.nullcontext()):
+            self.sm_wgrad.run(ops._p(self.dense), dl, self.gw_sm, ws, self.ws_bytes)
+            ops.colsum(dlogits, B, nc, nc, self.colsum_scratch, self.gb_sm)
+            self.im_wgrad.run(ops._p(self.im_feat), dd, self.gw_im, ws, self.ws_bytes)
+            self.tx_wgrad.run(ops._p(self.tx_feat), dd, self.gw_tx, ws, self.ws_bytes)
+            ops.colsum(self.ddense, B, fc, fc, self.colsum_scratch, self.gb_fc)
+            if job is not None:
+                job()
+            if self.reducer is not None:
+                self.reducer.stage_done("head")
+        if side is not None:
+            self.image.head_grads_pending = True
         return self.d_im, self.d_tx
 
     def input_backward(self, dlogits, with_text=False):
diff --git a/tumblr_emotions_amd/net.py b/tumblr_emotions_amd/net.py
--- a/tumblr_emotions_amd/net.py
+++ b/tumblr_emotions_amd/net.py
@@ -46,6 +46,7 @@
                                         trainable_embedding=trainable_embedding)
         if mode == "joint":
             self.head = JointHeadEngine(self.store, im_features_size, rnn_size, fc_size, nb_emotions, device)
+            self.head.image = self.image
         elif mode == "text":
             self.head = TextHeadEngine(self.store, rnn_size, nb_emotions, device)
         self.store.finalize()
@@ -399,19 +400,45 @@
         if self.frozen_bn:
             self.image.frozen_step = True
         try:
+            self._async_head_grads(True)
             logits = self.forward(batch, dropout_mask, seed)
             ce = self.cross_entropy(logits, batch["labels"])
-            if st.n_l2 > 0:
-                ops.sumsq(st.theta, st.n_l2, self.l2_scratch, self.l2_buf)
+            self._enqueue_l2_term()
             self.reducer.begin_step()
             ce.backward()
+            self._join_head_grads()
         finally:
+            self._async_head_grads(False)
             if self.frozen_bn:
                 self.image.frozen_step = False
         grad_scale = self.reducer.finish()
         ops.adam_tf(st.theta, st.grad, st.m, st.v, st.n_trainable_padded, st.n_l2, WEIGHT_DECAY, grad_scale, lr_t,
                     ADAM_B1, ADAM_B2, ADAM_EPS)
         return ce
+
+    def _l2_term(self):
+        st = self.store
+        ops.sumsq(st.theta, st.n_l2, self.l2_scratch, self.l2_buf)
+
+    def _enqueue_l2_term(self):
+        if self.store.n_l2 <= 0:
+            return
+        if self.mode == "joint" and self.head.grouped():
+            self.head.side_job = self._l2_term
+        elif self.mode == "image" and self.image.head_group:
+            self.image.side_job = self._l2_term
+        else:
+            self._l2_term()
+
+    def _async_head_grads(self, on):
+        if self.mode == "joint":
+            self.head.async_grads = bool(on)
+
+    def _join_head_grads(self):
+        im = self.image
+        if im is not None and im.head_grads_pending:
+            torch.cuda.current_stream().wait_stream(im.side_w)
+            im.head_grads_pending = False
 
     def check_clones(self, num_clones, batch_rows=None, seed=None):
         K = num_clones
@@ -503,7 +530,6 @@
             None if dropout_mask is None else dropout_mask.data_ptr(), gen, wv)
 
     def _step_kernels(self, batch, dropout_mask):
-        st = self.store
         main = torch.cuda.current_stream()
         side = self.text_stream if (self.image is not None and self.text is not None) else None
         im = tx = None
@@ -520,25 +546,35 @@
                 main.wait_stream(side)
             else:
                 tx = self.text.forward(batch["texts"], batch["seq_lens"])
+        if self.dlogits is None or self.dlogits.shape[0] != batch["labels"].shape[0]:
+            raise RuntimeError("capture_step: run one eager train_step with this batch size first")
+        ce_done = False
         if self.mode == "image":
             logits = im
         elif self.mode == "text":
             logits = self.head.forward(tx)
+        elif self.head.grouped() and self.head.ce_fused():
+            logits = self.head.forward(im, tx, ce=(batch["labels"], self.loss_buf, self.dlogits))
+            ce_done = True
         else:
             logits = self.head.forward(im, tx)
         self.logits = logits
-        if self.dlogits is None or self.dlogits.shape != logits.shape:
+        if self.dlogits.shape != logits.shape:
             raise RuntimeError("capture_step: run one eager train_step with this batch size first")
         B, C_ = logits.shape
-        ops.softmax_ce(logits, batch["labels"], B, C_, 1.0, None, self.loss_buf, self.dlogits)
-        if st.n_l2 > 0:
-            ops.sumsq(st.theta, st.n_l2, self.l2_scratch, self.l2_buf)
+        if not ce_done:
+            ops.softmax_ce(logits, batch["labels"], B, C_, 1.0, None, self.loss_buf, self.dlogits)
+        self._enqueue_l2_term()
         if self.mode == "image":
             self.image.backward(self.dlogits)
         elif self.mode == "text":
             self.text.backward(self.head.backward(self.dlogits))
         else:
-            d_im, d_tx = self.head.backward(self.dlogits)
+            self._async_head_grads(True)
+            try:
+                d_im, d_tx = self.head.backward(self.dlogits)
+            finally:
+                self._async_head_grads(False)
             if side is not None:
                 side.wait_stream(main)
                 with torch.cuda.stream(side):
@@ -548,6 +584,7 @@
             else:
                 self.text.backward(d_tx)
                 self.image.backward(d_im)
+        self._join_head_grads()
 
     def capture_step(self, batch, dropout_mask=None, num_clones=1):
         if type(num_clones) is not int or num_clones != 1:
diff --git a/tumblr_emotions_amd/ops.py b/tumblr_emotions_amd/ops.py
--- a/tumblr_emotions_amd/ops.py
+++ b/tumblr_emotions_amd/ops.py
@@ -159,6 +159,62 @@
                                         bias, mask, self.ldmask, self.flags, _stream()), "ds_slab_epilogue")
         if t is not None:
             t.end(self)
+
+
+def slab_combine(gemm, out, ldo, flags=0, bias=None, mask=None, ldmask=0, pre=None, out2=None, ldo2=0, n_split=0):
+    c = _lib.SlabCombine()
+    c.slabs, c.splits, c.slab_stride, c.lds = gemm.slabs.data_ptr(), gemm.splits, gemm.M * gemm.N, gemm.N
+    if pre is not None:
+        assert (pre.M, pre.N) == (gemm.M, gemm.N)
+        c.pre_slabs, c.pre_splits, c.pre_slab_stride, c.pre_lds = pre.slabs.data_ptr(), pre.splits, pre.M * pre.N, pre.N
+    c.M, c.N, c.flags = gemm.M, gemm.N, flags
+    c.out, c.ldo, c.out2, c.ldo2, c.n_split = out, ldo, out2, ldo2, n_split
+    c.bias, c.mask, c.ldmask = bias, mask, ldmask
+    return c
+
+
+def _addr(p):
+    return p.value if isinstance(p, C.c_void_p) else p
+
+
+class GemmGroup:
+
+    def __init__(self, gemms, combines):
+        n = len(gemms)
+        self.gemms, self.n = gemms, n
+        self._descs = (_lib._CD * n)(*[C.pointer(g.plan.d) for g in gemms])
+        self._z = (C.c_void_p * n)(*[g.slabs.data_ptr() for g in gemms])
+        self._combines = (_lib.SlabCombine * len(combines))(*combines)
+        self.alg_flops = sum(g.alg_flops for g in gemms)
+
+    def run(self, xs, ws):
+        t = CONV_TIMER
+        if t is not None:
+            t.begin()
+        lib = _lib.load()
+        n = self.n
+        if n == 1:
+            _lib.check(lib.ds_conv_igemm(C.byref(self.gemms[0].plan.d), xs[0], ws[0], _p(self.gemms[0].slabs), None, None, None,
+                                         None, _stream()), "ds_conv_igemm")
+        else:
+            x = (C.c_void_p * n)(*[_addr(p) for p in xs])
+            w = (C.c_void_p * n)(*[_addr(p) for p in ws])
+            _lib.check(lib.ds_gemm_group(self._descs, x, w, self._z, n, _stream()), "ds_gemm_group")
+        _lib.check(lib.ds_slab_epilogue_group(self._combines, len(self._combines), _stream()), "ds_slab_epilogue_group")
+        if t is not None:
+            t.end(self)
+
+
+def split_gemm_ce(gemm, x, w, logits, bias, labels, loss, dlogits):
+    t = CONV_TIMER
+    if t is not None:
+        t.begin()
+    lib = _lib.load()
+    _lib.check(lib.ds_conv_igemm(C.byref(gemm.plan.d), x, w, _p(gemm.slabs), None, None, None, None, _stream()), "ds_conv_igemm")
+    if t is not None:
+        t.end(gemm)
+    _lib.check(lib.ds_slab_epilogue_ce(_p(gemm.slabs), gemm.splits, gemm.M * gemm.N, gemm.N, gemm.M, gemm.N, _p(logits), bias,
+                                       _p(labels), 1.0, None, _p(loss), _p(dlogits), _stream()), "ds_slab_epilogue_ce")
 
 
 class WinoPlan:
```

After: 20010 samples/s, median of 6. 1.01x the previous value.
